# google/ffn

Measured on AMD Instinct MI355X. Metric: FoV-steps/sec (flood-filling inference loop, 250^3 volume), higher is better.
Workload: dtype f32 (fp16 hi + scaled-residual split products on the fp16 MFMA, f32 accumulate)

## Files before the change

### ffn_amd/csrc/ffn_canvas_kernels.h

```cpp
#pragma once

namespace ffn {

struct Box {
  int lo[3];
  int n[3];
  int cy, cx;
};

__device__ __forceinline__ size_t box_index(const Box& b, long e) {
  const int x = e % b.n[2];
  const long t = e / b.n[2];
  const int y = t % b.n[1];
  const int z = t / b.n[1];
  return ((size_t)(b.lo[0] + z) * b.cy + (b.lo[1] + y)) * b.cx + (b.lo[2] + x);
}

template <typename T>
__global__ void box_read_kernel(const T* __restrict__ vol, Box b, long total,
                                T* __restrict__ dst) {
  for (long e = blockIdx.x * (long)blockDim.x + threadIdx.x; e < total;
       e += (long)gridDim.x * blockDim.x)
    dst[e] = vol[box_index(b, e)];
}

template <typename T>
__global__ void box_write_kernel(T* __restrict__ vol, Box b, long total,
                                 const T* __restrict__ src) {
  for (long e = blockIdx.x * (long)blockDim.x + threadIdx.x; e < total;
       e += (long)gridDim.x * blockDim.x)
    vol[box_index(b, e)] = src[e];
}

template <typename T>
__global__ void box_fill_kernel(T* __restrict__ vol, Box b, long total, T value) {
  for (long e = blockIdx.x * (long)blockDim.x + threadIdx.x; e < total;
       e += (long)gridDim.x * blockDim.x)
    vol[box_index(b, e)] = value;
}

__global__ void fill_u32_kernel(uint32_t* __restrict__ p, uint32_t v, size_t n) {
  const size_t n4 = n / 4;
  uint4 vv = make_uint4(v, v, v, v);
  for (size_t e = blockIdx.x * (size_t)blockDim.x + threadIdx.x; e < n4;
       e += (size_t)gridDim.x * blockDim.x)
    reinterpret_cast<uint4*>(p)[e] = vv;
  if (blockIdx.x == 0 && threadIdx.x < (n & 3)) p[n4 * 4 + threadIdx.x] = v;
}

__global__ void points_read_kernel(const float* __restrict__ seed,
                                   const int32_t* __restrict__ seg, int cz,
                                   int cy, int cx, int n,
                                   const int32_t* __restrict__ pos,
                                   float* __restrict__ seed_out,
                                   int32_t* __restrict__ seg_out) {
  const int k = blockIdx.x * blockDim.x + threadIdx.x;
  if (k >= n) return;
  const int z = pos[3 * k], y = pos[3 * k + 1], x = pos[3 * k + 2];
  if (z < 0 || z >= cz || y < 0 || y >= cy || x < 0 || x >= cx) {
    seed_out[k] = __builtin_nanf("");
    seg_out[k] = 0;
    return;
  }
  const size_t ci = ((size_t)z * cy + y) * cx + x;
  seed_out[k] = seed[ci];
  seg_out[k] = seg[ci];
}

__global__ void points_write_seg_kernel(int32_t* __restrict__ seg, int cy, int cx,
                                        int n, const int32_t* __restrict__ pos,
                                        const int32_t* __restrict__ val) {
  const int k = blockIdx.x * blockDim.x + threadIdx.x;
  if (k >= n) return;
  seg[((size_t)pos[3 * k] * cy + pos[3 * k + 1]) * cx + pos[3 * k + 2]] = val[k];
}

__global__ void set_seg_point_kernel(int32_t* __restrict__ seg, size_t ci,
                                     int32_t value) {
  seg[ci] = value;
}

__global__ void set_seed_point_kernel(float* __restrict__ seed, size_t ci,
                                      float value) {
  seed[ci] = value;
}

__global__ void any_segmented_kernel(const int32_t* __restrict__ seg, Box b,
                                     long total, int32_t* __restrict__ out) {
  int hit = 0;
  for (long e = blockIdx.x * (long)blockDim.x + threadIdx.x; e < total;
       e += (long)gridDim.x * blockDim.x)
    hit |= seg[box_index(b, e)] > 0;
  if (__any(hit) && (threadIdx.x & 63) == 0) atomicOr(out, 1);
}

__global__ void commit_count_kernel(const float* __restrict__ seed,
                                    const int32_t* __restrict__ seg, Box b,
                                    long total, float thr, int32_t max_id,
                                    unsigned long long* __restrict__ counts,
                                    unsigned* __restrict__ hist) {
  unsigned raw = 0, act = 0;
  for (long e = blockIdx.x * (long)blockDim.x + threadIdx.x; e < total;
       e += (long)gridDim.x * blockDim.x) {
    const size_t ci = box_index(b, e);
    if (seed[ci] >= thr) {
      ++raw;
      const int32_t s = seg[ci];
      if (s <= 0) {
        ++act;
      } else if (s <= max_id) {
        atomicAdd(&hist[s], 1u);
      }
    }
  }
#pragma unroll
  for (int off = 32; off > 0; off >>= 1) {
    raw += __shfl_xor(raw, off);
    act += __shfl_xor(act, off);
  }
  if ((threadIdx.x & 63) == 0) {
    if (raw) atomicAdd(&counts[0], (unsigned long long)raw);
    if (act) atomicAdd(&counts[1], (unsigned long long)act);
  }
}

__global__ void commit_assign_kernel(const float* __restrict__ seed,
                                     int32_t* __restrict__ seg, Box b, long total,
                                     float thr, int32_t sid) {
  for (long e = blockIdx.x * (long)blockDim.x + threadIdx.x; e < total;
       e += (long)gridDim.x * blockDim.x) {
    const size_t ci = box_index(b, e);
    if (seed[ci] >= thr && seg[ci] <= 0) seg[ci] = sid;
  }
}

struct TurnRecord {
  unsigned long long counts[2];
  int committed;
  int chosen;
  int pad[2];
};
constexpr int kTurnOk = 0, kTurnSegmented = 1, kTurnTooClose = 2, kTurnNotReached = 3,
              kTurnRestricted = 4;

__global__ void turn_commit_kernel(const float* __restrict__ seed,
                                   int32_t* __restrict__ seg, Box b, long total,
                                   float thr, int32_t sid, long long min_size,
                                   TurnRecord* __restrict__ rec, long mark_ci,
                                   int mark_mode) {
  const bool ok = total > 0 && (long long)rec->counts[1] >= min_size;
  if (ok) {
    for (long e = blockIdx.x * (long)blockDim.x + threadIdx.x; e < total;
         e += (long)gridDim.x * blockDim.x) {
      const size_t ci = box_index(b, e);
      if (seed[ci] >= thr && seg[ci] <= 0) seg[ci] = sid;
    }
  }
  if (blockIdx.x == 0 && threadIdx.x == 0) {
    rec->committed = ok ? 1 : 0;
    if ((mark_mode == 1 || (mark_mode == 2 && !ok)) && seg[mark_ci] == 0)
      seg[mark_ci] = -1;
  }
}

__global__ __launch_bounds__(64) void turn_eval_kernel(
    const float* __restrict__ seed, const int32_t* __restrict__ seg, int cz, int cy,
    int cx, const int32_t* __restrict__ cand, int mz, int my, int mx,
    int* __restrict__ flags, float* __restrict__ cand_seed,
    int32_t* __restrict__ cand_seg, const unsigned long long* __restrict__ rplanes,
    size_t plane_words, int row_words) {
  const int j = blockIdx.x;
  const int z = cand[3 * j], y = cand[3 * j + 1], x = cand[3 * j + 2];
  const size_t ci = ((size_t)z * cy + y) * cx + x;
  const int32_t s = seg[ci];
  int flag = kTurnOk;
  bool restricted = false;
  if (rplanes) {
    const size_t wi = ((size_t)z * cy + y) * row_words + (x >> 6);
    restricted = ((rplanes[wi] | rplanes[plane_words + wi]) >> (x & 63)) & 1ull;
  }
  if (s > 0) {
    flag = kTurnSegmented;
  } else if (restricted) {
    flag = kTurnRestricted;
  } else {
    const int z0 = max(z - mz, 0), z1 = min(z + mz + 1, cz);
    const int y0 = max(y - my, 0), y1 = min(y + my + 1, cy);
    const int x0 = max(x - mx, 0), x1 = min(x + mx + 1, cx);
    const int ny = y1 - y0, nx = x1 - x0;
    const int total = (z1 - z0) * ny * nx;
    int hit = 0;
    for (int e = threadIdx.x; e < total; e += 64) {
      const int ex = e % nx, t = e / nx;
      hit |= seg[((size_t)(z0 + t / ny) * cy + (y0 + t % ny)) * cx + (x0 + ex)] > 0;
    }
    if (__any(hit)) flag = kTurnTooClose;
  }
  if (threadIdx.x == 0) {
    flags[j] = flag;
    cand_seed[j] = seed[ci];
    cand_seg[j] = s;
  }
}

__global__ __launch_bounds__(64) void turn_pick_kernel(
    int32_t* __restrict__ seg, int cy, int cx, const int32_t* __restrict__ cand,
    int n, int* __restrict__ flags, TurnRecord* __restrict__ rec) {
  int chosen = -1;
  for (int base = 0; base < n && chosen < 0; base += 64) {
    const int j = base + threadIdx.x;
    const unsigned long long m = __ballot(j < n && flags[j] == kTurnOk);
    if (m) chosen = base + __ffsll((long long)m) - 1;
  }
  const int upto = chosen < 0 ? n : chosen;
  for (int j = threadIdx.x; j < n; j += 64) {
    if (j < upto) {
      if (flags[j] == kTurnTooClose)
        seg[((size_t)cand[3 * j] * cy + cand[3 * j + 1]) * cx + cand[3 * j + 2]] = -1;
    } else if (j > upto) {
      flags[j] = kTurnNotReached;
    }
  }
  if (threadIdx.x == 0) rec->chosen = chosen;
}

__global__ void turn_clear_kernel(uint32_t* __restrict__ seed, Box b, long total,
                                  int linear, size_t nvox,
                                  const TurnRecord* __restrict__ rec) {
  if (rec->chosen < 0) return;
  if (linear) {
    const size_t n4 = nvox / 4;
    const uint4 vv = make_uint4(0x7fc00000u, 0x7fc00000u, 0x7fc00000u, 0x7fc00000u);
    for (size_t e = blockIdx.x * (size_t)blockDim.x + threadIdx.x; e < n4;
         e += (size_t)gridDim.x * blockDim.x)
      reinterpret_cast<uint4*>(seed)[e] = vv;
    if (blockIdx.x == 0 && threadIdx.x < (nvox & 3))
      seed[n4 * 4 + threadIdx.x] = 0x7fc00000u;
    return;
  }
  for (long e = blockIdx.x * (long)blockDim.x + threadIdx.x; e < total;
       e += (long)gridDim.x * blockDim.x)
    seed[box_index(b, e)] = 0x7fc00000u;
}

__global__ void turn_seed_kernel(float* __restrict__ seed, int cy, int cx,
                                 const int32_t* __restrict__ cand, float value,
                                 const TurnRecord* __restrict__ rec) {
  const int j = rec->chosen;
  if (j < 0) return;
  seed[((size_t)cand[3 * j] * cy + cand[3 * j + 1]) * cx + cand[3 * j + 2]] = value;
}

}
```

### ffn_amd/csrc/ffn_hip.hip

```cpp

#include <hip/hip_runtime.h>
#include <hip/hip_ext.h>

#include <algorithm>
#include <cmath>
#include <cstdarg>
#include <cstdio>
#include <cstdlib>
#include <chrono>
#include <cstring>
#include <map>
#include <mutex>
#include <string>
#include <vector>

#include "ffn_internal.h"
#include "ffn_kernels.h"
#include "ffn_restrict_kernels.h"
#include "ffn_host_loop.h"

using namespace ffn;

namespace {

constexpr int kHeadBlocks = 281;

thread_local std::string g_error;

int fail(int code, const char* fmt, ...) {
  char buf[512];
  va_list ap;
  va_start(ap, fmt);
  vsnprintf(buf, sizeof(buf), fmt, ap);
  va_end(ap);
  g_error = buf;
  return code;
}

}

int ffn_set_error(int code, const char* fmt, ...) {
  char buf[512];
  va_list ap;
  va_start(ap, fmt);
  vsnprintf(buf, sizeof(buf), fmt, ap);
  va_end(ap);
  g_error = buf;
  return code;
}

namespace {

#define HIP_TRY(expr)                                                        \
  do {                                                                       \
    hipError_t _e = (expr);                                                  \
    if (_e != hipSuccess)                                                    \
      return fail(FFN_ERR_HIP, "%s failed: %s (%s:%d)", #expr,               \
                  hipGetErrorString(_e), __FILE__, __LINE__);                \
  } while (0)

}

struct ffn_engine {
  std::recursive_mutex mu;
  std::mutex util_mu;
  hipStream_t ustream = nullptr;
  hipEvent_t main_ev = nullptr;
  std::mutex many_mu;
  ffn_host::ManyCarry many_carry;
  uint32_t many_ticket = 0;
  std::vector<ffn_canvas*> many_canvases;
  int device = 0;
  hipStream_t stream = nullptr;
  Geom g{};
  Geom gp{};
  bool permuted = false;
  int depth = 0;
  int max_batch = 0;
  bool weights_set = false;

  float* act_base = nullptr;
  float* bufT = nullptr;
  float* bufX = nullptr;
  uint32_t* validbits = nullptr;
  int32_t* pidx = nullptr;
  int nchunks_c = 0, Rc = 0;
  int fuse_head = 1;
  int count_blocks = kHeadBlocks;
  int store_policy = 1;
  long long* d_dbg = nullptr;
  int dbg_clock = 0;
  int dbg_layer = 3;
  size_t lds_bytes_c = 0;
  int nchunks_k = 0, Rc_k = 0;
  bool k_ok = false;
  float* rawT = nullptr;
  float* rawX = nullptr;
  float* rawS = nullptr;
  bool d_ok = false;
  bool e_ok = false;
  int batch_chunks = 1;
  bool small_now = false;
  bool m_ok = false;
  bool m_now = false;
  bool t_ok = false;
  bool t_now = false;
  int tail_batched = 0;
  int flow = 0;
  unsigned* flow_flags = nullptr;
  unsigned* flow_err = nullptr;
  unsigned flow_epoch = 0;
  int flow_debug = 0;
  bool flow_fits = false;
  int flow_strikes = 0;
  int flow_skip = 0;
  int flow_auto_off = 0;
  long stat_flow_voids = 0;
  bool last_stack_resident = false;
  bool slot_resident[2] = {false, false};
  long long* flow_trace = nullptr;
  int flow_trace_slots = 0;
  int n_main = 0, n_tail = 0, n_tail3 = 0;
  int tsched_aoff[4 * 8] = {};
  int t3sched_aoff[4 * 8] = {};
  int nchunks_m = 0;
  int nchunks_e = 0;
  size_t lds_bytes_e = 0;
  int esched_aoff[4 * 8] = {};
  bool d_weights_ok = true;
  uint16_t* wpackd = nullptr;
  size_t wpackd_layer = 0;
  uint16_t* wpackh = nullptr;
  bool h_ok = false;
  bool h_now = false;
  int n_half = 0;
  int flow_pace = -1;
  int flow_pace_tail = 0;
  int flow_pace_spread = -1;
  int pace_auto = 0;
  float pace_auto_us[2] = {0.f, 0.f};
  int cus = 0;
  size_t lds_bytes_d = 0;
  int dsched_aoff[4 * 8] = {};
  int dsched_btap[4 * 8] = {};
  unsigned* range_flag = nullptr;
  struct Spec {
    bool valid = false;
    const ffn_canvas* canvas = nullptr;
    int n = 0;
    int pos[kSpecMax][3] = {};
    float pad_value = 0.f, move_thr = 0.f;
    int variant = 0;
  } spec;
  int speculate = 1;
  int spec_force_mismatch = 0;
  long stat_spec_mismatch = 0;
  long stat_many_carried = 0;
  int fuse_paste = 1;
  int fuse_conv0a = 1;
  int* d_spec_choice = nullptr;
  long stat_spec_launched = 0, stat_spec_hits = 0;
  long stat_spec_miss_full = 0, stat_spec_miss_short = 0;
  long long stat_segturn_queue_ns = 0, stat_segturn_wait_ns = 0;
  long stat_segturn_calls = 0;
  int stack_ahead = 1;
  int paste_blocks = 0;
  int debug_submit_delay_ns = 0;
  int debug_fused_twice = 0;
  bool trace_now = false;
  bool ahead_valid = false;
  long stat_ahead_used = 0, stat_ahead_wasted = 0;
  unsigned range_tag = 0;
  bool fp16_ok = true;
  int conv_variant = 0;
  int exact_variant = 0;
  float* h_io = nullptr;
  float* up_image = nullptr;
  float* up_seed = nullptr;
  float* seed_raw = nullptr;
  float* seed_raw_alt = nullptr;
  unsigned* range_flag_alt = nullptr;
  int* d_spec_choice_alt = nullptr;
  float* logits = nullptr;
  unsigned* count = nullptr;
  uint8_t* valid = nullptr;
  float* weights = nullptr;
  size_t w0a_off = 0, b0a_off = 0, wl_off = 0;
  size_t w0ap_off = 0;
  std::vector<size_t> wpack_off, bias_off;

  StepItem* d_items = nullptr;
  StepItem* h_items = nullptr;
  unsigned long long* h_pub = nullptr;
  unsigned step_id = 0;
  int next_slot = 0;
  int slot_n[2] = {0, 0};
  bool slot_waited[2] = {false, false};
  unsigned slot_ticket[2] = {0, 0};
  std::vector<ffn_canvas*> slot_canvas[2];
  int sync_mode = 1;
  long stat_calls = 0, stat_items = 0;
  long stat_hist[65] = {};
  long long* d_stamps = nullptr;
  long long t_arrived_ns = 0;
  int fused_trace_in = 0;
  long long stat_turn_host_ns = 0, stat_launch_host_ns = 0;
  long stat_turn_host_count = 0;

  void* d_scratch = nullptr;
  void* h_scratch = nullptr;
  size_t scratch_bytes = 0;

  int prof_mode = 0;
  std::vector<hipEvent_t> events;
  int events_used = 0;
  hipEvent_t ahead_ev[2] = {nullptr, nullptr};
  bool ahead_ev_pending = false;
  double conv_ms = 0.0;
  int64_t conv_launches = 0;
  size_t lds_bytes = 0;
  std::vector<ffn_canvas*> canvases;
  int prof_every = 1;
  long stack_calls = 0;
  bool prof_now = false;
  int ablate = 0;
  std::vector<int> chain_launches_pending;
  std::vector<float> prof_samples;
};

struct ffn_canvas {
  ffn_engine* engine = nullptr;
  float* image = nullptr;
  uint8_t* image_u8 = nullptr;
  float* image_lut = nullptr;
  float* seed = nullptr;
  int32_t* seg = nullptr;
  int cz = 0, cy = 0, cx = 0;
  size_t nvox = 0;
  int dirty_lo[3] = {0, 0, 0};
  int dirty_hi[3] = {0, 0, 0};
  ffn_host::SegmentState loop;
  hipEvent_t ev_util = nullptr;
  bool util_pending = false;
  bool paste_after_flag = false;
  int hint_n = 0;
  int hint_pos[kSpecMax][3] = {};
  bool hint_from_loop = false;
  unsigned long long* restrict_planes = nullptr;
  size_t restrict_plane_words = 0;
  int restrict_row_words = 0;
  std::vector<uint64_t> restrict_host;

  void mark_dirty(const int lo[3], const int hi[3]) {
    const int dims[3] = {cz, cy, cx};
    const bool empty = dirty_lo[0] >= dirty_hi[0];
    for (int k = 0; k < 3; ++k) {
      const int l = std::max(lo[k], 0), h = std::min(hi[k], dims[k]);
      dirty_lo[k] = empty ? l : std::min(dirty_lo[k], l);
      dirty_hi[k] = empty ? h : std::max(dirty_hi[k], h);
    }
  }
};

namespace {
inline long long steady_ns() {
  return std::chrono::duration_cast<std::chrono::nanoseconds>(
             std::chrono::steady_clock::now().time_since_epoch()).count();
}
inline unsigned next_tag(unsigned t) { return t + 1 ? t + 1 : 1; }
inline void drop_spec(ffn_engine* e) {
  if (e->spec.valid && !e->ahead_valid) e->range_tag = next_tag(e->range_tag);
  if (e->ahead_valid) e->stat_ahead_wasted += 1;
  e->spec.valid = false;
  e->ahead_valid = false;
}
struct EngineLock {
  std::unique_lock<std::recursive_mutex> lk;
  explicit EngineLock(ffn_engine* e) {
    if (e) lk = std::unique_lock<std::recursive_mutex>(e->mu);
  }
};
constexpr int kFlowStrikes = 3;

int flow_voided(ffn_engine* e, bool timed_out) {
  if (!timed_out) return 0;
  EngineLock lock_(e);
  e->stat_flow_voids += 1;
  e->flow_strikes += 1;
  e->flow_skip = 1;
  if (e->flow_strikes >= kFlowStrikes && e->flow == 2) {
    e->flow = 0;
    e->flow_auto_off = 1;
    e->flow_skip = 0;
    return fail(FFN_ERR_FLOW,
                "the resident conv launch timed out waiting for one of its own "
                "workgroups %d steps in a row (is the GPU shared or partitioned?): "
                "the step changed nothing; this engine now runs one launch per conv "
                "(option flow = 0; set flow = 2 to try again) -- repeat the step",
                kFlowStrikes);
  }
  return fail(FFN_ERR_FLOW,
              "the resident conv launch timed out waiting for one of its own "
              "workgroups: the step changed nothing; repeat it (the repeat runs one "
              "launch per conv, same arithmetic)");
}

struct UtilLock {
  std::unique_lock<std::mutex> ul;
  std::unique_lock<std::recursive_mutex> lk;
  explicit UtilLock(ffn_engine* e) {
    if (e) {
      ul = std::unique_lock<std::mutex>(e->util_mu);
      lk = std::unique_lock<std::recursive_mutex>(e->mu);
    }
  }
  hipError_t begin(ffn_engine* e, ffn_canvas* c, bool reads_only = false) {
    if (!reads_only) drop_spec(e);
    if (!c->paste_after_flag) return hipSuccess;
    hipError_t err = hipEventRecord(e->main_ev, e->stream);
    if (err == hipSuccess) err = hipStreamWaitEvent(e->ustream, e->main_ev, 0);
    if (err == hipSuccess) c->paste_after_flag = false;
    return err;
  }
  hipError_t end(ffn_engine* e, ffn_canvas* c) {
    c->util_pending = true;
    return hipEventRecord(c->ev_util, e->ustream);
  }
  hipError_t wait(ffn_engine* e, ffn_canvas* c) {
    hipError_t err = end(e, c);
    if (err != hipSuccess) return err;
    lk.unlock();
    err = hipEventSynchronize(c->ev_util);
    lk.lock();
    if (err == hipSuccess) c->util_pending = false;
    return err;
  }
};
hipError_t canvas_quiesce(ffn_engine* e, ffn_canvas* c) {
  drop_spec(e);
  hipError_t err = hipSuccess;
  if (c->paste_after_flag) {
    err = hipStreamSynchronize(e->stream);
    if (err == hipSuccess) c->paste_after_flag = false;
  }
  if (err == hipSuccess && c->util_pending) {
    err = hipEventSynchronize(c->ev_util);
    if (err == hipSuccess) c->util_pending = false;
  }
  return err;
}
}

int ffn_canvas_view(ffn_canvas* c, FfnCanvasView* out) {
  if (!c || !out) return ffn_set_error(FFN_ERR_ARG, "NULL canvas");
  if (!c->engine)
    return ffn_set_error(FFN_ERR_STATE, "canvas outlived its engine");
  {
    EngineLock lock_(c->engine);
    if (canvas_quiesce(c->engine, c) != hipSuccess)
      return ffn_set_error(FFN_ERR_HIP, "canvas_quiesce failed");
  }
  out->device_id = c->engine->device;
  out->engine_stream = c->engine->stream;
  out->image = c->image;
  out->image_u8 = c->image_u8;
  out->image_lut = c->image_lut;
  out->segmentation = c->seg;
  out->shape_zyx[0] = c->cz;
  out->shape_zyx[1] = c->cy;
  out->shape_zyx[2] = c->cx;
  return FFN_OK;
}

namespace {

int ensure_scratch(ffn_engine* e, size_t bytes) {
  if (bytes <= e->scratch_bytes) return FFN_OK;
  HIP_TRY(hipStreamSynchronize(e->ustream));
  if (e->d_scratch) HIP_TRY(hipFree(e->d_scratch));
  if (e->h_scratch) HIP_TRY(hipHostFree(e->h_scratch));
  e->d_scratch = e->h_scratch = nullptr;
  e->scratch_bytes = 0;
  size_t want = std::max<size_t>(bytes, 1 << 20);
  HIP_TRY(hipMalloc(&e->d_scratch, want));
  HIP_TRY(hipHostMalloc(&e->h_scratch, want, hipHostMallocDefault));
  e->scratch_bytes = want;
  return FFN_OK;
}

template <bool RI, bool RO, bool SK>
int set_lds_attr(size_t bytes) {
  HIP_TRY(hipFuncSetAttribute(
      reinterpret_cast<const void*>(&conv32_kernel<RI, RO, SK>),
      hipFuncAttributeMaxDynamicSharedMemorySize, (int)bytes));
  return FFN_OK;
}

inline void split_fp16x2(float x, uint16_t part[2]) {
  const float xh = std::fabs(x) < 6.103515625e-05f ? 0.0f : x;
  const _Float16 hi = (_Float16)xh;
  const _Float16 res = (_Float16)((x - (float)hi) * 2048.0f);
  std::memcpy(&part[0], &hi, 2);
  std::memcpy(&part[1], &res, 2);
}

int set_lds_attr_d(size_t bytes) {
#define FFN_D_ATTR(KIND, SK, KSV, HEADV)                                          \
  HIP_TRY(hipFuncSetAttribute(                                                    \
      reinterpret_cast<const void*>(&conv32d_kernel<KIND, SK, KSV, HEADV>),       \
      hipFuncAttributeMaxDynamicSharedMemorySize, (int)bytes))
#define FFN_D_ATTRS(KSV)            \
  FFN_D_ATTR(0, false, KSV, false); \
  FFN_D_ATTR(1, false, KSV, false); \
  FFN_D_ATTR(1, true, KSV, false);  \
  FFN_D_ATTR(1, false, KSV, true);  \
  FFN_D_ATTR(1, true, KSV, true)
  FFN_D_ATTRS(8);
  FFN_D_ATTRS(9);
  FFN_D_ATTRS(10);
#undef FFN_D_ATTRS
#undef FFN_D_ATTR
  return FFN_OK;
}

constexpr int kERows = 208, kETiles = 3, kEPieces = 7;

// ... 389 lines not shown
  nx.tiles_x = qx;
  nx.so.out_sp = reinterpret_cast<char*>(e->rawT) + (size_t)q.guard * 16;
  nx.so.sp_plane_bytes = (q.act_stride / kFeatures) * 16;
  nx.so.item_bytes = q.act_stride * (long)sizeof(float);
  nx.so.range_flag = next ? e->range_flag_alt : e->range_flag;
  nx.so.range_tag = tag;
  nx.sp = sp;
  if (sp.n > 0) nx.sp.choice = next ? e->d_spec_choice_alt : e->d_spec_choice;
  return qz * qy * qx;
}

void launch_conv0a(ffn_engine* e, int n, const StepItems& si, float pad_value,
                   unsigned tag, const SpecArgs& sp, bool next = false) {
  const Geom& g = e->g;
  const float* W = e->weights;
  const int tz = (g.fz + kC0Z - 1) / kC0Z, ty = (g.fy + kC0Y - 1) / kC0Y,
            tx = (g.fx + kC0X - 1) / kC0X;
  if (e->conv_variant >= 6) {
    Conv0Next nx;
    const int tiles = conv0a_split_args(e, pad_value, tag, sp, next, nx);
    hipLaunchKernelGGL(conv0a_mfma_kernel<true>, dim3(tiles, n),
                       dim3(kC0Threads), 0, e->stream, si, pad_value, nx.w, nx.bias,
                       nx.out, nx.seed_raw, nx.q, nx.tiles_y, nx.tiles_x, nx.so, nx.sp);
  } else {
    SpecArgs sp2 = sp;
    if (sp.n > 0) sp2.choice = next ? e->d_spec_choice_alt : e->d_spec_choice;
    hipLaunchKernelGGL(conv0a_mfma_kernel<false>, dim3(tz * ty * tx, n),
                       dim3(kC0Threads), 0, e->stream, si, pad_value,
                       W + e->w0a_off, W + e->b0a_off, e->bufT,
                       next ? e->seed_raw_alt : e->seed_raw, g, ty, tx,
                       Conv0SplitOut(), sp2);
  }
}

int launch_conv32ps(ffn_engine* e, float pad_value, float move_thr,
                    const int* ahead_choice = nullptr, hipEvent_t ev0 = nullptr,
                    hipEvent_t ev1 = nullptr) {
  HeadFusion hf;
  hf.on = true;
  hf.pad_value = pad_value;
  hf.move_thr = move_thr;
  ConvDArgs a;
  conv32d_args(e, 1, e->rawT, e->rawS, 0, hf, a);
  a.L.dbg = e->dbg_clock ? e->d_dbg : nullptr;
  ConvTailMap mp;
  tail_map(e, 1, mp);
  const Geom& g = e->gp;
  ConvStackTab tb;
  tb.nlayers = 2 * e->depth - 1;
  tb.dbg_layer = e->dbg_layer;
  tb.sp_t = reinterpret_cast<const char*>(e->rawT) + (size_t)g.guard * 16;
  tb.sp_s = reinterpret_cast<char*>(e->rawS) + (size_t)g.guard * 16;
  tb.wpack0 = reinterpret_cast<const char*>(e->wpackd);
  tb.wpack_stride = (long)(e->wpackd_layer * sizeof(uint16_t));
  tb.bias0 = e->weights + e->bias_off[0];
  tb.bias_stride = e->depth > 1 ? (long)(e->bias_off[1] - e->bias_off[0]) : 0;
  tb.epoch0 = e->flow_epoch;
  tb.pace = e->flow_pace < 0 ? e->pace_auto : e->flow_pace;
  tb.pace_tail = e->flow_pace_tail;
  tb.pace_spread = e->flow_pace_spread < 0 ? tb.pace : e->flow_pace_spread;
  e->flow_epoch += (unsigned)tb.nlayers;
  const dim3 grid(8 * (mp.mains_per_xcd + mp.tails_per_xcd)), block(kDThreads);
  tb.l_begin = 0;
  tb.l_end = tb.nlayers;
  tb.stamps = e->d_stamps;
  tb.ahead_choice = ahead_choice;
  tb.trace = e->trace_now ? 1 : (ahead_choice && e->fused_trace_in == 1) ? 2 : 0;
  const long long t_l0 = e->t_arrived_ns ? steady_ns() : 0;
  if (ev0)
    hipExtLaunchKernelGGL(conv32ps_kernel, grid, block, kMLdsBytes, e->stream, ev0, ev1, 0, a,
                          mp, tb);
  else
    hipLaunchKernelGGL(conv32ps_kernel, grid, block, kMLdsBytes, e->stream, a, mp, tb);
  if (e->t_arrived_ns) {
    const long long t_l1 = steady_ns();
    if (t_l1 - e->t_arrived_ns < 100000) {
      e->stat_turn_host_ns += t_l1 - e->t_arrived_ns;
      e->stat_launch_host_ns += t_l1 - t_l0;
      e->stat_turn_host_count += 1;
    }
    e->t_arrived_ns = 0;
  }
  return FFN_OK;
}

void half_map(const ffn_engine* e, ConvHalfMap& mp) {
  mp.n_chunks = e->n_half;
  mp.per_first = std::max(1, e->cus / 8);
  mp.n_first = std::min(e->n_half, 8 * mp.per_first);
  mp.per_second = (e->n_half - mp.n_first + 7) / 8;
}

template <int KIND, bool SK>
int launch_conv32h(ffn_engine* e, const float* raw_in, float* raw_out, int layer,
                   const HeadFusion& head = HeadFusion()) {
  ConvDArgs a;
  conv32d_args(e, 1, raw_in, raw_out, layer, head, a);
  a.L.wpack = reinterpret_cast<const char*>(e->wpackh + (size_t)layer * e->wpackd_layer);
  a.flow_n_main = -1;
  ConvHalfMap mp;
  half_map(e, mp);
  const dim3 grid(8 * (mp.per_first + mp.per_second)), block(kDThreads);
  if (head.on) {
    if constexpr (KIND == 1)
      hipLaunchKernelGGL((conv32h_kernel<KIND, SK, true>), grid, block, kHLdsBytes, e->stream,
                         a, mp);
  } else {
    hipLaunchKernelGGL((conv32h_kernel<KIND, SK, false>), grid, block, kHLdsBytes, e->stream,
                       a, mp);
  }
  return FFN_OK;
}

int launch_conv32hs(ffn_engine* e, float pad_value, float move_thr) {
  HeadFusion hf;
  hf.on = true;
  hf.pad_value = pad_value;
  hf.move_thr = move_thr;
  ConvDArgs a;
  conv32d_args(e, 1, e->rawT, e->rawS, 0, hf, a);
  a.flow_n_main = -1;
  ConvHalfMap mp;
  half_map(e, mp);
  const Geom& g = e->gp;
  ConvStackTab tb;
  tb.nlayers = 2 * e->depth - 1;
  tb.dbg_layer = e->dbg_layer;
  tb.sp_t = reinterpret_cast<const char*>(e->rawT) + (size_t)g.guard * 16;
  tb.sp_s = reinterpret_cast<char*>(e->rawS) + (size_t)g.guard * 16;
  tb.wpack0 = reinterpret_cast<const char*>(e->wpackh);
  tb.wpack_stride = (long)(e->wpackd_layer * sizeof(uint16_t));
  tb.bias0 = e->weights + e->bias_off[0];
  tb.bias_stride = e->depth > 1 ? (long)(e->bias_off[1] - e->bias_off[0]) : 0;
  tb.epoch0 = e->flow_epoch;
  e->flow_epoch += (unsigned)tb.nlayers;
  tb.l_begin = 0;
  tb.l_end = tb.nlayers;
  tb.pace = e->flow_pace < 0 ? 0 : e->flow_pace;
  tb.pace_tail = 0;
  tb.pace_spread = e->flow_pace_spread < 0 ? tb.pace : e->flow_pace_spread;
  tb.stamps = nullptr;
  tb.ahead_choice = nullptr;
  tb.trace = 0;
  const dim3 grid(8 * (mp.per_first + mp.per_second)), block(kDThreads);
  hipLaunchKernelGGL(conv32hs_kernel, grid, block, kHLdsBytes, e->stream, a, mp, tb);
  return FFN_OK;
}

int run_stack(ffn_engine* e, int n, const StepItems& si, float pad_value,
              float move_thr, bool conv0a_done = false, bool ahead = false) {
  const Geom& g = e->g;
  const float* W = e->weights;
  if (!conv0a_done) drop_spec(e);
  if (e->ahead_valid) e->stat_ahead_wasted += 1;
  e->spec.valid = false;
  e->ahead_valid = false;
  e->last_stack_resident = false;
  e->range_tag = next_tag(e->range_tag);
  std::swap(e->seed_raw, e->seed_raw_alt);
  std::swap(e->range_flag, e->range_flag_alt);
  std::swap(e->d_spec_choice, e->d_spec_choice_alt);
  const bool sampled = (e->stack_calls % e->prof_every) == 0;
  e->stack_calls++;
  e->prof_now = e->prof_mode == 1 && sampled;
  const bool prof_chain = e->prof_mode == 2 && sampled;
  if (!conv0a_done) launch_conv0a(e, n, si, pad_value, e->range_tag, SpecArgs());
  int rc;
  const float* head_in;
  bool head_fused = false;
  e->ahead_ev_pending = false;
  const bool one_launch = e->conv_variant == 9 && n == 1 && e->flow == 2 &&
                          e->flow_skip == 0 && e->tail_batched == 0;
  hipEvent_t k_ev0 = nullptr, k_ev1 = nullptr;
  if (prof_chain && ahead) {
    if (one_launch) k_ev0 = e->ahead_ev[0], k_ev1 = e->ahead_ev[1];
    else HIP_TRY(hipEventRecord(e->ahead_ev[0], e->stream));
  } else if (prof_chain) {
    if (e->events_used + 2 > (int)e->events.size()) {
      rc = flush_events(e);
      if (rc) return rc;
    }
    e->chain_launches_pending.push_back(2 * e->depth - 1);
    if (one_launch) {
      k_ev0 = e->events[e->events_used], k_ev1 = e->events[e->events_used + 1];
      e->events_used += 2;
    } else {
      HIP_TRY(hipEventRecord(e->events[e->events_used++], e->stream));
    }
  }
  e->small_now = e->conv_variant == 7 ||
                 (e->conv_variant == 6 && e->batch_chunks == 1 && n >= 2 && e->e_ok);
  e->m_now = e->conv_variant >= 8 ||
             (e->conv_variant == 6 && e->batch_chunks == 2 && n >= 2 && e->m_ok);
  e->t_now = e->conv_variant == 9 && (n == 1 || e->tail_batched != 0);
  e->h_now = e->conv_variant == 10 && n == 1;
  if (e->conv_variant >= 6) {
    if (e->depth == 1)
      return fail(FFN_ERR_ARG, "conv_variant 6 needs depth >= 2 (fused head)");
    auto chain = [&]() -> int {
      if (e->h_now) {
        if (e->flow == 2 && e->flow_skip > 0) {
          e->flow_skip -= 1;
        } else if (e->flow == 2) {
          e->last_stack_resident = true;
          return launch_conv32hs(e, pad_value, move_thr);
        }
        int r = launch_conv32h<1, false>(e, e->rawT, e->rawS, 0);
        for (int i = 1; i < e->depth && !r; ++i) {
          r = launch_conv32h<0, false>(e, e->rawS, e->rawT, 2 * i - 1);
          if (r) break;
          HeadFusion hf;
          hf.on = i == e->depth - 1;
          hf.pad_value = pad_value;
          hf.move_thr = move_thr;
          r = launch_conv32h<1, true>(e, e->rawT, e->rawS, 2 * i, hf);
        }
        return r;
      }
      if (e->t_now && n == 1 && e->flow == 2) {
        if (e->flow_skip > 0) {
          e->flow_skip -= 1;
        } else {
          e->last_stack_resident = true;
          return launch_conv32ps(e, pad_value, move_thr, ahead ? e->d_spec_choice : nullptr,
                                 k_ev0, k_ev1);
        }
      }
      if (ahead) return fail(FFN_ERR_STATE, "stack_ahead without the resident launch");
      int r = launch_conv32d<1, false>(e, n, e->rawT, e->rawS, 0);
      for (int i = 1; i < e->depth && !r; ++i) {
        r = launch_conv32d<0, false>(e, n, e->rawS, e->rawT, 2 * i - 1);
        if (r) break;
        HeadFusion hf;
        hf.on = i == e->depth - 1;
        hf.pad_value = pad_value;
        hf.move_thr = move_thr;
        r = launch_conv32d<1, true>(e, n, e->rawT, e->rawS, 2 * i, hf);
      }
      return r;
    };
    rc = chain();
    if (rc) return rc;
    head_fused = true;
    head_in = e->bufX;
  } else if (e->conv_variant == 0) {
    rc = launch_conv32<false, false, false>(e, n, e->bufT, e->bufX, nullptr, 0);
    if (rc) return rc;
    for (int i = 1; i < e->depth; ++i) {
      rc = launch_conv32<true, true, false>(e, n, e->bufX, e->bufT, nullptr,
                                            2 * i - 1);
      if (rc) return rc;
      rc = launch_conv32<false, false, true>(e, n, e->bufT, e->bufX, e->bufX,
                                             2 * i);
      if (rc) return rc;
    }
    head_in = e->bufX;
  } else {
    rc = launch_conv32c<false, false, false>(e, n, e->bufT, e->bufX, nullptr, 0);
    if (rc) return rc;
    for (int i = 1; i < e->depth; ++i) {
      rc = launch_conv32c<true, true, false>(e, n, e->bufX, e->bufT, nullptr,
                                             2 * i - 1);
      if (rc) return rc;
      HeadFusion hf;
      hf.on = e->fuse_head && i == e->depth - 1 && e->ablate == 0;
      hf.pad_value = pad_value;
      hf.move_thr = move_thr;
      rc = launch_conv32c<false, false, true>(e, n, e->bufT, e->bufX, e->bufX,
                                              2 * i, hf);
      if (rc) return rc;
      head_fused = hf.on;
    }
    head_in = e->bufX;
  }
  if (prof_chain && ahead) {
    if (!k_ev0) HIP_TRY(hipEventRecord(e->ahead_ev[1], e->stream));
    e->ahead_ev_pending = true;
  } else if (prof_chain && !k_ev0) {
    HIP_TRY(hipEventRecord(e->events[e->events_used++], e->stream));
  }
  if (head_fused) {
    e->count_blocks = e->h_now ? e->n_half
                      : e->t_now ? e->n_main + (n == 1 ? e->n_tail : e->n_tail3)
                      : e->m_now ? e->nchunks_m : e->small_now ? e->nchunks_e
                      : e->conv_variant >= 6 ? e->nchunks_k : e->nchunks_c;
  } else {
    e->count_blocks = kHeadBlocks;
    hipLaunchKernelGGL(head_kernel, dim3(kHeadBlocks, n), dim3(256), 0, e->stream,
                       head_in, e->seed_raw, pad_value, W + e->wl_off, move_thr,
                       e->logits, e->count, g);
  }
  HIP_TRY(hipGetLastError());
  return FFN_OK;
}

int dense_items(ffn_engine* e, int n, StepItems* si) {
  const Geom& g = e->g;
  for (int k = 0; k < n; ++k) {
    StepItem& it = e->h_items[k];
    std::memset(&it, 0, sizeof(it));
    it.image = e->up_image + (size_t)k * g.V;
    it.image_u8 = nullptr;
    it.image_lut = nullptr;
    it.seed = e->up_seed + (size_t)k * g.V;
    it.seg = nullptr;
    it.cz = g.fz;
    it.cy = g.fy;
    it.cx = g.fx;
// ... 26 lines not shown
int check_canvas(const ffn_canvas* c) {
  if (!c) return fail(FFN_ERR_ARG, "null canvas");
  if (!c->engine) return fail(FFN_ERR_STATE, "canvas outlived its engine");
  return FFN_OK;
}

int check_box(const ffn_canvas* c, const int32_t lo[3], const int32_t hi[3]) {
  const int dims[3] = {c->cz, c->cy, c->cx};
  for (int k = 0; k < 3; ++k)
    if (lo[k] < 0 || hi[k] > dims[k] || hi[k] < lo[k])
      return fail(FFN_ERR_ARG, "box [%d,%d) out of canvas axis %d (size %d)",
                  lo[k], hi[k], k, dims[k]);
  return FFN_OK;
}

int grid_for(long total, int block = 256) {
  long g = (total + block - 1) / block;
  return (int)std::max<long>(1, std::min<long>(g, 2048));
}

}

extern "C" {

int ffn_abi_version(void) { return 10; }

const char* ffn_last_error(void) { return g_error.c_str(); }

size_t ffn_engine_weight_count(int depth, int features) {
  const size_t F = (size_t)features;
  return 27 * 2 * F + F + (size_t)(2 * depth - 1) * (27 * F * F + F) + F + 1;
}

int ffn_engine_create(int device_id, const int32_t fov_zyx[3],
                      const int32_t deltas_zyx[3], int depth, int features,
                      int max_batch, ffn_engine** out) {
  if (!out || !fov_zyx || !deltas_zyx) return fail(FFN_ERR_ARG, "null argument");
  *out = nullptr;
  if (features != kFeatures)
    return fail(FFN_ERR_ARG, "features must be %d (got %d)", kFeatures, features);
  if (depth < 1 || max_batch < 1)
    return fail(FFN_ERR_ARG, "depth and max_batch must be >= 1");
  for (int k = 0; k < 3; ++k) {
    if (fov_zyx[k] < 3 || fov_zyx[k] % 2 == 0)
      return fail(FFN_ERR_ARG, "fov must be odd and >= 3 per axis");
    if (deltas_zyx[k] < 0 || 2 * deltas_zyx[k] + 1 > fov_zyx[k])
      return fail(FFN_ERR_ARG, "deltas do not fit inside the fov");
  }
  int ndev = 0;
  HIP_TRY(hipGetDeviceCount(&ndev));
  if (device_id < 0 || device_id >= ndev)
    return fail(FFN_ERR_ARG, "device %d not present (%d visible)", device_id, ndev);
  HIP_TRY(hipSetDevice(device_id));

  ffn_engine* e = new ffn_engine();
  e->device = device_id;
  e->depth = depth;
  e->max_batch = max_batch;
  Geom& g = e->g;
  g.fz = fov_zyx[0];
  g.fy = fov_zyx[1];
  g.fx = fov_zyx[2];
  g.dz = deltas_zyx[0];
  g.dy = deltas_zyx[1];
  g.dx = deltas_zyx[2];
  g.XS = g.fx + 1;
  g.plane = (g.fy + 1) * g.XS;
  g.npos = g.fz * g.plane;
  g.guard = g.plane + g.XS + 1;
  g.nchunks = (g.npos + kChunk - 1) / kChunk;
  g.V = g.fz * g.fy * g.fx;
  g.R = kChunk + 2 * (g.XS + 1);
  g.oa[0] = 0, g.oa[1] = 1, g.oa[2] = 2;
  g.dstr[0] = g.fy * g.fx, g.dstr[1] = g.fx, g.dstr[2] = 1;
  g.crop = 0;
  g.c0[0] = g.c0[1] = g.c0[2] = 0;
  g.c1[0] = g.fz, g.c1[1] = g.fy, g.c1[2] = g.fx;
  g.Vp = g.V;
  auto permute = [&](const int oa[3]) {
    const int f[3] = {g.fz, g.fy, g.fx}, d[3] = {g.dz, g.dy, g.dx};
    const int ds[3] = {g.fy * g.fx, g.fx, 1};
    Geom q = g;
    q.fz = f[oa[0]], q.fy = f[oa[1]], q.fx = f[oa[2]];
    q.dz = d[oa[0]], q.dy = d[oa[1]], q.dx = d[oa[2]];
    q.XS = q.fx + 1;
    q.plane = (q.fy + 1) * q.XS;
    q.npos = q.fz * q.plane;
    q.guard = q.plane + q.XS + 1;
    q.nchunks = (q.npos + kChunk - 1) / kChunk;
    q.R = kChunk + 2 * (q.XS + 1);
    for (int a = 0; a < 3; ++a) q.oa[a] = oa[a], q.dstr[a] = ds[oa[a]];
    return q;
  };
  auto chunk_span = [](const Geom& q, int start, int chunk, int count) {
    auto pad = [&](int v) {
      const int x = v % q.fx, y = (v / q.fx) % q.fy, z = v / (q.fx * q.fy);
      return z * q.plane + y * q.XS + x;
    };
    int span = 0;
    for (int c = 0; c < count; ++c) {
      const int lo = start + c * chunk, hi = std::min(q.V, lo + chunk) - 1;
      if (lo <= hi) span = std::max(span, pad(hi) - pad(lo) + 1);
    }
    return span;
  };
  auto m_fits = [&](const Geom& q) {
    return chunk_span(q, 0, kMChunk, (q.V + kMChunk - 1) / kMChunk) +
               2 * (q.XS + 1) <= kMRows;
  };
  e->gp = g;
  if (!m_fits(g)) {
    static const int kPerms[5][3] = {{0, 2, 1}, {1, 0, 2}, {1, 2, 0}, {2, 0, 1},
                                     {2, 1, 0}};
    int best = -1;
    for (int k = 0; k < 5; ++k) {
      const Geom q = permute(kPerms[k]);
      if (m_fits(q) && (best < 0 || q.fx < permute(kPerms[best]).fx)) best = k;
    }
    if (best >= 0) {
      e->gp = permute(kPerms[best]);
      e->permuted = true;
    }
  }
  const long positions = std::max(
      (long)g.guard + (long)g.nchunks * kChunk + g.guard + 320,
      (long)e->gp.guard + (long)e->gp.nchunks * kChunk + e->gp.guard + 320);
  g.act_stride = positions * kFeatures;
  e->gp.act_stride = g.act_stride;
  e->lds_bytes = (size_t)3 * g.R * kFeatures * sizeof(float);
  if (e->lds_bytes > 160 * 1024) {
    delete e;
    return fail(FFN_ERR_ARG, "fov too wide for the LDS-staged conv (%zu B)",
                e->lds_bytes);
  }

#define E_TRY(expr)                                                          \
  do {                                                                       \
    hipError_t _e = (expr);                                                  \
    if (_e != hipSuccess) {                                                  \
      int _rc = fail(FFN_ERR_HIP, "%s failed: %s (%s:%d)", #expr,            \
                     hipGetErrorString(_e), __FILE__, __LINE__);             \
      ffn_engine_destroy(e);                                                 \
      return _rc;                                                            \
    }                                                                        \
  } while (0)

  E_TRY(hipStreamCreateWithFlags(&e->stream, hipStreamNonBlocking));
  {
    int lo = 0, hi = 0;
    E_TRY(hipDeviceGetStreamPriorityRange(&lo, &hi));
    E_TRY(hipStreamCreateWithPriority(&e->ustream, hipStreamNonBlocking, hi));
  }
  E_TRY(hipEventCreateWithFlags(&e->main_ev, hipEventDisableTiming));
  const size_t act_bytes = (size_t)3 * max_batch * g.act_stride * sizeof(float);
  E_TRY(hipMalloc(&e->act_base, act_bytes));
  E_TRY(hipMemset(e->act_base, 0, act_bytes));
  e->rawT = e->act_base;
  e->rawX = e->rawT + (size_t)max_batch * g.act_stride;
  e->rawS = e->rawX + (size_t)max_batch * g.act_stride;
  e->bufT = e->rawT + (size_t)g.guard * kFeatures;
  e->bufX = e->rawX + (size_t)g.guard * kFeatures;
  const size_t vbytes = (size_t)max_batch * g.V * sizeof(float);
  E_TRY(hipMalloc(&e->up_image, vbytes));
  E_TRY(hipMalloc(&e->up_seed, vbytes));
  E_TRY(hipMalloc(&e->seed_raw, vbytes));
  E_TRY(hipMalloc(&e->seed_raw_alt, vbytes));
  E_TRY(hipMalloc(&e->logits, vbytes));
  E_TRY(hipHostMalloc(&e->h_io, 3 * vbytes, hipHostMallocDefault));
  E_TRY(hipMemset(e->up_image, 0, vbytes));
  E_TRY(hipMemset(e->up_seed, 0, vbytes));
  E_TRY(hipMalloc(&e->count, sizeof(unsigned) * max_batch *
                                  std::max<size_t>(kHeadBlocks, (g.V + 31) / 32)));
  E_TRY(hipMalloc(&e->d_items, sizeof(StepItem) * 2 * max_batch));
  E_TRY(hipHostMalloc(&e->h_items, sizeof(StepItem) * 2 * max_batch,
                      hipHostMallocDefault));
  E_TRY(hipHostMalloc(&e->h_pub,
                      sizeof(unsigned long long) * kPubWords * 2 * max_batch,
                      hipHostMallocDefault));
  std::memset(e->h_pub, 0, sizeof(unsigned long long) * kPubWords * 2 * max_batch);

  {
    std::vector<uint8_t> v((size_t)g.nchunks * kChunk, 0);
    for (int p = 0; p < g.npos; ++p) {
      const int rem = p % g.plane;
      v[p] = (rem / g.XS < g.fy && rem % g.XS < g.fx) ? 1 : 0;
    }
    E_TRY(hipMalloc(&e->valid, v.size()));
    E_TRY(hipMemcpy(e->valid, v.data(), v.size(), hipMemcpyHostToDevice));
    std::vector<uint32_t> bits((size_t)g.nchunks * 5, 0u);
    for (size_t p = 0; p < v.size(); ++p)
      if (v[p]) bits[(p / kChunk) * 5 + ((p % kChunk) >> 5)] |= 1u << (p & 31);
    static_assert(kChunk == 160, "validbits layout assumes 5 words per chunk");
    E_TRY(hipMalloc(&e->validbits, bits.size() * sizeof(uint32_t)));
    E_TRY(hipMemcpy(e->validbits, bits.data(), bits.size() * sizeof(uint32_t),
                    hipMemcpyHostToDevice));
  }

  {
    e->nchunks_c = (g.V + kCChunk - 1) / kCChunk;
    e->nchunks_k = (g.V + kDChunk - 1) / kDChunk;
    std::vector<int32_t> pidx(std::max((size_t)e->nchunks_c * kCChunk,
                                       (size_t)e->nchunks_k * kDChunk));
    for (size_t v = 0; v < pidx.size(); ++v) {
      const int vv = (int)std::min<size_t>(v, (size_t)g.V - 1);
      const int x = vv % g.fx, y = (vv / g.fx) % g.fy, z = vv / (g.fx * g.fy);
      pidx[v] = z * g.plane + y * g.XS + x;
    }
    int span = 0;
    for (int c = 0; c < e->nchunks_c; ++c)
      span = std::max(span, pidx[(size_t)c * kCChunk + kCChunk - 1] -
                                pidx[(size_t)c * kCChunk] + 1);
    e->Rc = ((span + 2 * (g.XS + 1)) + 31) / 32 * 32;
    if (e->Rc < 256) e->Rc = 256;
    e->lds_bytes_c = (size_t)2 * e->Rc * kCLdsStride * sizeof(float);
    {
      const Geom& q = e->gp;
      const int span_k = chunk_span(q, 0, kDChunk, e->nchunks_k);
      e->Rc_k = ((span_k + 2 * (q.XS + 1)) + 31) / 32 * 32;
      if (e->Rc_k < 256) e->Rc_k = 256;
      e->k_ok = e->Rc_k <= 320 && e->nchunks_k >= 2;
      static const int kSched[4][7] = {{0, 1, 8, 9, 16, 18, 19},
                                       {2, 3, 10, 11, 17, 20, 21},
                                       {4, 5, 12, 13, 22, 23, 24},
                                       {6, 7, 14, 15, 25, 26, -1}};
      e->lds_bytes_d = std::max((size_t)3 * 128 * e->Rc_k,
                                (size_t)4 * kDChunk * kDRowB + 64);
      for (int w = 0; w < 4; ++w)
        for (int j = 0; j < 7; ++j) {
          int s = kSched[w][j];
          const bool dummy = s < 0;
          if (dummy) s = kSched[w][j - 1];
          const int kz = s / 9, ky = (s / 3) % 3, kx = s % 3;
          e->dsched_aoff[w * 8 + j] =
              kz * 128 * e->Rc_k + ((ky - 1) * q.XS + (kx - 1)) * 16;
          e->dsched_btap[w * 8 + j] = dummy ? 27 : s;
        }
      e->d_ok = e->k_ok && e->lds_bytes_d <= 160 * 1024 && depth >= 2;
      {
        const int ce = 32 * kETiles;
        e->nchunks_e = (q.V + ce - 1) / ce;
        const int span_e = chunk_span(q, 0, ce, e->nchunks_e);
        e->lds_bytes_e = std::max((size_t)3 * 128 * kERows,
                                  (size_t)4 * ce * kDRowB + 64);
        e->e_ok = e->d_ok && span_e + 2 * (q.XS + 1) <= kERows &&
                  e->nchunks_e >= 2 && e->lds_bytes_e <= 80 * 1024;
        e->nchunks_m = (q.V + kMChunk - 1) / kMChunk;
        const int span_m = chunk_span(q, 0, kMChunk, e->nchunks_m);
        e->m_ok = e->d_ok && span_m + 2 * (q.XS + 1) <= kMRows && e->nchunks_m >= 2;
        if (e->m_ok && e->nchunks_m > 256) {
          e->n_main = 256;
          e->n_tail = (q.V - 256 * kMChunk + 31) / 32;
          e->n_tail3 = (q.V - 256 * kMChunk + 95) / 96;
          const int span_t = chunk_span(q, 256 * kMChunk, 32, e->n_tail);
          const int span_t3 = chunk_span(q, 256 * kMChunk, 96, e->n_tail3);
          static_assert((size_t)3 * 128 * kTRows <= kMLdsBytes &&
                            (size_t)4 * 32 * kDRowB + 64 <= kMLdsBytes &&
                            (size_t)3 * 128 * kT3Rows <= kMLdsBytes &&
                            (size_t)4 * 96 * kDRowB + 64 <= kMLdsBytes,
                        "a tail workgroup fits conv32m's LDS");
          e->t_ok = span_t + 2 * (q.XS + 1) <= kTRows &&
                    span_t3 + 2 * (q.XS + 1) <= kT3Rows && e->n_tail <= 256;
          for (int w = 0; w < 4; ++w)
            for (int j = 0; j < 7; ++j) {
              int s = kSched[w][j];
              if (s < 0) s = kSched[w][j - 1];
              const int kz = s / 9, ky = (s / 3) % 3, kx = s % 3;
              e->tsched_aoff[w * 8 + j] =
                  kz * 128 * kTRows + ((ky - 1) * q.XS + (kx - 1)) * 16;
              e->t3sched_aoff[w * 8 + j] =
                  kz * 128 * kT3Rows + ((ky - 1) * q.XS + (kx - 1)) * 16;
            }
        }
        for (int w = 0; w < 4; ++w)
          for (int j = 0; j < 7; ++j) {
            int s = kSched[w][j];
            if (s < 0) s = kSched[w][j - 1];
            const int kz = s / 9, ky = (s / 3) % 3, kx = s % 3;
            e->esched_aoff[w * 8 + j] =
                kz * 128 * kERows + ((ky - 1) * q.XS + (kx - 1)) * 16;
          }
      }
    }
    E_TRY(hipMalloc(&e->d_dbg, (24 + 4 * kDbgMaxWgs) * sizeof(long long)));
    E_TRY(hipMemset(e->d_dbg, 0, (24 + 4 * kDbgMaxWgs) * sizeof(long long)));
    E_TRY(hipMalloc(&e->pidx, pidx.size() * sizeof(int32_t)));
    E_TRY(hipMemcpy(e->pidx, pidx.data(), pidx.size() * sizeof(int32_t),
                    hipMemcpyHostToDevice));
    const bool c_ok = e->Rc == 256 || e->Rc == 288;
    e->exact_variant = c_ok ? 2 : 0;
    e->conv_variant = e->t_ok ? 9 : e->m_ok ? 8 : e->d_ok ? 6 : e->exact_variant;
    if (e->t_ok && depth >= 2) {
      int cus = 0, per_cu = 0;
      E_TRY(hipDeviceGetAttribute(&cus, hipDeviceAttributeMultiprocessorCount, device_id));
      E_TRY(hipFuncSetAttribute(reinterpret_cast<const void*>(conv32ps_kernel),
                                hipFuncAttributeMaxDynamicSharedMemorySize, kMLdsBytes));
      E_TRY(hipOccupancyMaxActiveBlocksPerMultiprocessor(&per_cu, conv32ps_kernel,
                                                         kDThreads, kMLdsBytes));
      ConvTailMap mp;
      tail_map(e, 1, mp);
      const int grid = 8 * (mp.mains_per_xcd + mp.tails_per_xcd);
      e->flow_fits = cus >= e->n_main && (long)cus * per_cu >= grid;
    }
    e->flow = e->flow_fits ? 2 : 0;
    if (e->t_ok && depth >= 2) {
      const Geom& q = e->gp;
      e->n_half = FFN_H_VCLIP ? FFN_H_VCLIP / kHChunk : (q.V + kHChunk - 1) / kHChunk;
      const int span_h = chunk_span(q, 0, kHChunk, e->n_half);
      int cus = 0, per_cu = 0;
      E_TRY(hipDeviceGetAttribute(&cus, hipDeviceAttributeMultiprocessorCount, device_id));
      e->cus = cus;
      E_TRY(hipFuncSetAttribute(reinterpret_cast<const void*>(conv32hs_kernel),
                                hipFuncAttributeMaxDynamicSharedMemorySize, kHLdsBytes));
      E_TRY(hipOccupancyMaxActiveBlocksPerMultiprocessor(&per_cu, conv32hs_kernel, kDThreads,
                                                         kHLdsBytes));
      ConvHalfMap mp;
      half_map(e, mp);
      e->h_ok = e->n_half >= 2 && span_h + 2 * (q.XS + 1) <= kHRows &&
                (long)cus * per_cu >= 8 * (mp.per_first + mp.per_second);
    }
  }

  {
    size_t off = 0;
    e->w0a_off = off;
    off += 27 * 2 * kFeatures;
    e->b0a_off = off;
    off += kFeatures;
    e->w0ap_off = off;
    off += 27 * 2 * kFeatures;
    for (int l = 0; l < 2 * depth - 1; ++l) {
      e->wpack_off.push_back(off);
      off += 27 * kFeatures * kFeatures;
      e->bias_off.push_back(off);
      off += kFeatures;
    }
    e->wl_off = off;
    off += kFeatures + 1;
    off = (off + 3) & ~(size_t)3;
    E_TRY(hipMalloc(&e->weights, off * sizeof(float)));
    e->wpackd_layer = (size_t)kDTaps * 2 * 2 * 64 * 8;
    E_TRY(hipMalloc(&e->wpackd, e->wpackd_layer * (2 * depth - 1) *
                                    sizeof(uint16_t)));
    E_TRY(hipMalloc(&e->wpackh, e->wpackd_layer * (2 * depth - 1) * sizeof(uint16_t)));
    E_TRY(hipMalloc(&e->range_flag, 2 * sizeof(unsigned)));
    E_TRY(hipMemset(e->range_flag, 0, 2 * sizeof(unsigned)));
    E_TRY(hipMalloc(&e->range_flag_alt, 2 * sizeof(unsigned)));
    E_TRY(hipMemset(e->range_flag_alt, 0, 2 * sizeof(unsigned)));
    {
      const size_t words = ((size_t)(e->gp.V + 31) / 32 + 64) * kFlowStride;
      E_TRY(hipMalloc(&e->flow_flags, words * sizeof(unsigned)));
      E_TRY(hipMemset(e->flow_flags, 0, words * sizeof(unsigned)));
      E_TRY(hipMalloc(&e->flow_err, sizeof(unsigned)));
      E_TRY(hipMemset(e->flow_err, 0, sizeof(unsigned)));
      if (e->t_ok) {
        e->flow_trace_slots = std::max(e->n_main + e->n_tail, (e->gp.V + kHChunk - 1) / kHChunk);
        const size_t bytes = (size_t)e->flow_trace_slots * kFlowTraceLayers * 8 * sizeof(long long);
        E_TRY(hipMalloc(&e->flow_trace, bytes));
        E_TRY(hipMemset(e->flow_trace, 0, bytes));
      }
    }
    E_TRY(hipMalloc(&e->d_stamps, (32 + 1024) * sizeof(long long)));
    E_TRY(hipMemset(e->d_stamps, 0, (32 + 1024) * sizeof(long long)));
    E_TRY(hipMalloc(&e->d_spec_choice, sizeof(int)));
    E_TRY(hipMemset(e->d_spec_choice, 0xff, sizeof(int)));
    E_TRY(hipMalloc(&e->d_spec_choice_alt, sizeof(int)));
    E_TRY(hipMemset(e->d_spec_choice_alt, 0xff, sizeof(int)));
  }

  e->events.resize(2 * 64);
  for (auto& ev : e->events) E_TRY(hipEventCreate(&ev));
  for (auto& ev : e->ahead_ev) E_TRY(hipEventCreate(&ev));

  {
    int rc = set_lds_attr<false, false, false>(e->lds_bytes);
    if (!rc) rc = set_lds_attr<true, true, false>(e->lds_bytes);
    if (!rc) rc = set_lds_attr<false, false, true>(e->lds_bytes);
    if (!rc) rc = set_lds_attr_c<false, false, false>(e->lds_bytes_c);
    if (!rc) rc = set_lds_attr_c<true, true, false>(e->lds_bytes_c);
    if (!rc) rc = set_lds_attr_c<false, false, true>(e->lds_bytes_c);
    if (!rc) rc = set_lds_attr_c<false, false, true, 8>(e->lds_bytes_c);
    if (!rc) rc = set_lds_attr_c<false, false, true, 16>(e->lds_bytes_c);
    if (!rc) rc = set_lds_attr_c<false, false, true, 24>(e->lds_bytes_c);
    if (!rc && e->d_ok) rc = set_lds_attr_d(e->lds_bytes_d);
    if (!rc && e->e_ok) rc = set_lds_attr_e(e->lds_bytes_e);
    if (!rc && e->m_ok) rc = set_lds_attr_m();
    if (rc) {
      ffn_engine_destroy(e);
      return rc;
    }
  }
#undef E_TRY
  *out = e;
  return FFN_OK;
}

void ffn_engine_destroy(ffn_engine* e) {
  if (!e) return;
  (void)hipSetDevice(e->device);
  if (e->stream) (void)hipStreamSynchronize(e->stream);
  for (ffn_canvas* c : e->canvases) {
    (void)hipFree(c->image);
    (void)hipFree(c->image_u8);
    (void)hipFree(c->image_lut);
    (void)hipFree(c->seed);
    (void)hipFree(c->seg);
    (void)hipFree(c->restrict_planes);
    c->restrict_planes = nullptr;
    if (c->ev_util) (void)hipEventDestroy(c->ev_util);
    c->ev_util = nullptr;
    c->image = c->seed = nullptr;
    c->image_u8 = nullptr;
    c->image_lut = nullptr;
    c->seg = nullptr;
    c->engine = nullptr;
  }
  e->canvases.clear();
  if (e->ustream) (void)hipStreamSynchronize(e->ustream);
  if (e->main_ev) (void)hipEventDestroy(e->main_ev);
  if (e->ustream) (void)hipStreamDestroy(e->ustream);
  for (auto& ev : e->events)
    if (ev) (void)hipEventDestroy(ev);
  for (auto& ev : e->ahead_ev)
    if (ev) (void)hipEventDestroy(ev);
  (void)hipFree(e->act_base);
  (void)hipFree(e->up_image);
  (void)hipFree(e->up_seed);
  (void)hipFree(e->seed_raw);
  (void)hipFree(e->seed_raw_alt);
  (void)hipFree(e->range_flag_alt);
  (void)hipFree(e->d_spec_choice_alt);
  (void)hipFree(e->logits);
  (void)hipFree(e->count);
  (void)hipFree(e->wpackd);
  (void)hipFree(e->wpackh);
  (void)hipFree(e->range_flag);
  (void)hipFree(e->flow_flags);
  (void)hipFree(e->flow_err);
  (void)hipFree(e->flow_trace);
  (void)hipFree(e->d_spec_choice);
  (void)hipFree(e->d_stamps);
  (void)hipFree(e->valid);
  (void)hipFree(e->validbits);
  (void)hipFree(e->pidx);
  (void)hipFree(e->d_dbg);
  (void)hipFree(e->weights);
  (void)hipFree(e->d_items);
  (void)hipFree(e->d_scratch);
  if (e->h_io) (void)hipHostFree(e->h_io);
  if (e->h_items) (void)hipHostFree(e->h_items);
  if (e->h_pub) (void)hipHostFree(e->h_pub);
  if (e->h_scratch) (void)hipHostFree(e->h_scratch);
  if (e->stream) (void)hipStreamDestroy(e->stream);
  delete e;
}

struct PaceKey {
  int device, depth, V;
  bool operator<(const PaceKey& o) const {
    return device != o.device ? device < o.device : depth != o.depth ? depth < o.depth : V < o.V;
  }
};
struct PaceVal { int beat; float free_us, best_us; };
std::mutex g_pace_mu;
std::map<PaceKey, PaceVal> g_pace_cache;

int tune_pace(ffn_engine* e) {
  e->pace_auto = 0;
  e->pace_auto_us[0] = e->pace_auto_us[1] = 0.f;
  if (!(e->t_ok && e->flow_fits && e->flow == 2 && e->conv_variant == 9 && e->depth >= 2))
    return FFN_OK;
  const PaceKey key{e->device, e->depth, e->g.V};
  {
    std::lock_guard<std::mutex> lk(g_pace_mu);
    auto it = g_pace_cache.find(key);
    if (it != g_pace_cache.end()) {
      e->pace_auto = it->second.beat;
      e->pace_auto_us[0] = it->second.free_us;
      e->pace_auto_us[1] = it->second.best_us;
      return FFN_OK;
    }
  }
  const size_t V = (size_t)e->g.V;
  {
    std::vector<float> noise(2 * V);
    unsigned x = 12345u;
    for (auto& v : noise) {
      x = x * 1664525u + 1013904223u;
      v = ((int)(x >> 8) % 2001 - 1000) * 1e-3f;
    }
    HIP_TRY(hipMemcpy(e->up_image, noise.data(), V * sizeof(float), hipMemcpyHostToDevice));
    HIP_TRY(hipMemcpy(e->up_seed, noise.data() + V, V * sizeof(float), hipMemcpyHostToDevice));
  }
  unsigned errs0 = 0;
  HIP_TRY(hipMemcpy(&errs0, e->flow_err, sizeof(errs0), hipMemcpyDeviceToHost));
  StepItems si;
  int rc = dense_items(e, 1, &si);
  if (rc) return rc;
  hipEvent_t ev0, ev1;
  HIP_TRY(hipEventCreate(&ev0));
  HIP_TRY(hipEventCreate(&ev1));
  const int user_pace = e->flow_pace;
  auto stacks_us = [&](int pace, int reps, float* us) -> int {
    e->flow_pace = pace;
    int r = FFN_OK;
    for (int k = 0; k < 6 && !r; ++k) r = run_stack(e, 1, si, std::nanf(""), INFINITY);
    if (!r && hipEventRecord(ev0, e->stream) != hipSuccess) r = FFN_ERR_HIP;
    for (int k = 0; k < reps && !r; ++k) r = run_stack(e, 1, si, std::nanf(""), INFINITY);
    if (!r && (hipEventRecord(ev1, e->stream) != hipSuccess ||
               hipEventSynchronize(ev1) != hipSuccess))
      r = FFN_ERR_HIP;
    float ms = 0.f;
    if (!r && hipEventElapsedTime(&ms, ev0, ev1) != hipSuccess) r = FFN_ERR_HIP;
    *us = ms * 1e3f / (float)reps;
    return r;
  };
  float us = 0.f, free_us = 0.f, best_us = 0.f;
  int best = 0;
  {
    const long long t_end = steady_ns() + 150000000LL;
    while (!rc && steady_ns() < t_end) rc = stacks_us(0, 60, &us);
  }
  if (!rc) rc = stacks_us(0, 40, &free_us);
  best_us = 1e30f;
  for (int pace = 560; pace <= 800 && !rc; pace += 20) {
    rc = stacks_us(pace, 24, &us);
    if (!rc && us < best_us) {
      best_us = us;
      best = pace;
    }
  }
  if (!rc) {
    rc = stacks_us(0, 40, &us);
    free_us = std::min(free_us, us);
  }
  bool keep = !rc && best > 0 && best_us < 0.985f * free_us;
  float conf_free = free_us, conf_paced = best_us;
  for (int round = 0; round < 2 && keep && !rc; ++round) {
    float f = 0.f, p = 0.f;
    rc = stacks_us(0, 40, &f);
    if (!rc) rc = stacks_us(best + 10, 40, &p);
    keep = !rc && p < 0.985f * f;
    conf_free = f;
    conf_paced = p;
  }
  e->flow_pace = user_pace;
  (void)hipEventDestroy(ev0);
  (void)hipEventDestroy(ev1);
  if (rc) return rc;
  unsigned errs = 0;
  HIP_TRY(hipMemcpy(&errs, e->flow_err, sizeof(errs), hipMemcpyDeviceToHost));
  const bool timed_out = errs != errs0;
  e->pace_auto_us[0] = conf_free;
  e->pace_auto_us[1] = keep ? conf_paced : best_us;
  if (!timed_out && keep) e->pace_auto = best + 10;
  if (!timed_out) {
    std::lock_guard<std::mutex> lk(g_pace_mu);
    g_pace_cache[key] = PaceVal{e->pace_auto, e->pace_auto_us[0], e->pace_auto_us[1]};
  }
  return FFN_OK;
}

int ffn_engine_set_weights(ffn_engine* e, const float* blob, size_t count) {
  EngineLock lock_(e);
  if (!e || !blob) return fail(FFN_ERR_ARG, "null argument");
  const size_t want = ffn_engine_weight_count(e->depth, kFeatures);
  if (count != want)
    return fail(FFN_ERR_ARG, "weight blob has %zu floats, expected %zu", count,
                want);
  drop_spec(e);
  HIP_TRY(hipSetDevice(e->device));
  const int F = kFeatures;
  std::vector<float> host(e->wl_off + F + 1 + 3, 0.0f);
  const float* src = blob;
  std::vector<uint16_t> hostd(e->wpackd_layer * (2 * e->depth - 1));
  std::vector<uint16_t> hosth(hostd.size());
  bool d_weights_ok = true;
  bool weights_in_fp16_range = true;
  int tap_of[27];
  for (int t = 0; t < 27; ++t) {
    const int kp[3] = {t / 9, (t / 3) % 3, t % 3};
    int ko[3];
    for (int a = 0; a < 3; ++a) ko[e->gp.oa[a]] = kp[a];
    tap_of[t] = ko[0] * 9 + ko[1] * 3 + ko[2];
  }
  std::memcpy(&host[e->w0a_off], src, sizeof(float) * 27 * 2 * F);
  for (int t = 0; t < 27; ++t)
    std::memcpy(&host[e->w0ap_off + (size_t)t * 2 * F], src + (size_t)tap_of[t] * 2 * F,
                sizeof(float) * 2 * F);
  src += 27 * 2 * F;
  std::memcpy(&host[e->b0a_off], src, sizeof(float) * F);
  src += F;
  for (int l = 0; l < 2 * e->depth - 1; ++l) {
    float* wp = &host[e->wpack_off[l]];
    for (int tap = 0; tap < 27; ++tap)
      for (int nh = 0; nh < 2; ++nh)
        for (int h = 0; h < 2; ++h)
          for (int lane = 0; lane < 64; ++lane)
            for (int s = 0; s < 4; ++s) {
              const int gq = lane >> 4, j = lane & 15;
              const int ci = 16 * h + 4 * gq + s, co = 16 * nh + j;
// ... 89 lines not shown
    if (!is_void) {
      if (e->last_stack_resident) e->flow_strikes = 0;
      break;
    }
    if (attempt == 2) return fail(FFN_ERR_HIP, "ffn_predict: the step stayed void");
    if (flow_voided(e, flag[1] == e->range_tag) == 0) {
      rc = switch_variant(e, e->exact_variant);
      if (rc) return rc;
    }
    rc = run_stack(e, n, si, std::nanf(""), INFINITY);
    if (rc) return rc;
    HIP_TRY(hipMemcpyAsync(h_logits, e->logits, bytes, hipMemcpyDeviceToHost, e->stream));
  }
  std::memcpy(logits_out, h_logits, bytes);
  return FFN_OK;
}

int ffn_forward_resident(ffn_engine* e, int n, int repeats) {
  EngineLock lock_(e);
  if (!e) return fail(FFN_ERR_ARG, "null argument");
  if (n < 1 || n > e->max_batch)
    return fail(FFN_ERR_ARG, "batch %d outside [1, %d]", n, e->max_batch);
  if (!e->weights_set) return fail(FFN_ERR_STATE, "weights not set");
  HIP_TRY(hipSetDevice(e->device));
  StepItems si;
  int rc = dense_items(e, n, &si);
  if (rc) return rc;
  for (int r = 0; r < repeats; ++r) {
    rc = run_stack(e, n, si, std::nanf(""), INFINITY);
    if (rc) return rc;
  }
  return FFN_OK;
}

int ffn_engine_set_option(ffn_engine* e, const char* name, int value) {
  EngineLock lock_(e);
  if (!e || !name) return fail(FFN_ERR_ARG, "null argument");

  if (std::strcmp(name, "conv_variant") == 0) {
    if (value == -1) value = e->exact_variant;
    if (value != 0 && value != 2 && !(value >= 6 && value <= 10))
      return fail(FFN_ERR_ARG, "conv_variant must be 0, 2, 6, 7, 8, 9 or 10 (1, 3, 4, 5 "
                               "were removed in ABI 7)");
    if (value == 10 && !e->h_ok)
      return fail(FFN_ERR_ARG, "conv_variant 10 unsupported for this fov / depth / device "
                               "(80-voxel workgroups, two per CU, all resident)");
    if (value >= 6 && e->weights_set && !e->fp16_ok)
      return fail(FFN_ERR_ARG, "conv_variant %d: a weight is outside the fp16 range",
                  value);
    if (value == 6 && !e->d_ok)
      return fail(FFN_ERR_ARG, "conv_variant 6 unsupported for this fov / depth");
    if (value == 7 && !e->e_ok)
      return fail(FFN_ERR_ARG, "conv_variant 7 unsupported for this fov / depth");
    if (value == 8 && !e->m_ok)
      return fail(FFN_ERR_ARG, "conv_variant 8 unsupported for this fov / depth");
    if (value == 9 && !e->t_ok)
      return fail(FFN_ERR_ARG, "conv_variant 9 unsupported for this fov / depth "
                               "(257 .. 512 chunks of 128 voxels)");
    if (value >= 6 && e->weights_set && !e->d_weights_ok)
      return fail(FFN_ERR_ARG, "conv_variant 6: a weight x 2^11 is outside the fp16 range");
    if (value == 2 && !(e->Rc == 256 || e->Rc == 288))
      return fail(FFN_ERR_ARG, "conv_variant %d unsupported for this fov", value);
    return switch_variant(e, value);
  }
  if (std::strcmp(name, "profile_every") == 0) {
    if (value < 1) return fail(FFN_ERR_ARG, "profile_every must be >= 1");
    e->prof_every = value;
    return FFN_OK;
  }
  if (std::strcmp(name, "sync_mode") == 0) {
    if (value != 0 && value != 1) return fail(FFN_ERR_ARG, "sync_mode must be 0 or 1");
    e->sync_mode = value;
    return FFN_OK;
  }
  if (std::strcmp(name, "debug_clock") == 0) {
    e->dbg_clock = value;
    return FFN_OK;
  }
  if (std::strcmp(name, "batch_chunks") == 0) {
    if (value < 0 || value > 2) return fail(FFN_ERR_ARG, "batch_chunks 0..2");
    e->batch_chunks = value;
    return FFN_OK;
  }
  if (std::strcmp(name, "tail_batched") == 0) {
    e->tail_batched = value != 0;
    return FFN_OK;
  }
  if (std::strcmp(name, "flow_debug") == 0) {
    e->flow_debug = value;
    return FFN_OK;
  }
  if (std::strcmp(name, "flow_pace") == 0) {
    if (value < -1 || value > 5000)
      return fail(FFN_ERR_ARG, "flow_pace: -1 (measured), 0 (off) .. 5000 (10-ns ticks)");
    e->flow_pace = value;
    return FFN_OK;
  }
  if (std::strcmp(name, "flow_pace_spread") == 0) {
    if (value < -1 || value > 5000) return fail(FFN_ERR_ARG, "flow_pace_spread: -1 .. 5000");
    e->flow_pace_spread = value;
    return FFN_OK;
  }
  if (std::strcmp(name, "flow_pace_tail") == 0) {
    if (value < 0 || value > 5000) return fail(FFN_ERR_ARG, "flow_pace_tail: 0 .. 5000");
    e->flow_pace_tail = value;
    return FFN_OK;
  }
  if (std::strcmp(name, "flow") == 0) {
    if (value < 0 || value > 2) return fail(FFN_ERR_ARG, "flow: 0, 1 or 2");
    if (value && !e->t_ok)
      return fail(FFN_ERR_ARG, "flow needs conv32mt's geometry (conv_variant 9)");
    if (value && e->depth < 2) return fail(FFN_ERR_ARG, "flow needs depth >= 2");
    if (value == 2 && !e->flow_fits)
      return fail(FFN_ERR_ARG, "flow 2: this device cannot hold the resident launch's "
                  "workgroups all at once (compute units x occupancy)");
    drop_spec(e);
    e->flow = value;
    e->flow_auto_off = 0;
    e->flow_strikes = 0;
    e->flow_skip = 0;
    return FFN_OK;
  }
  if (std::strcmp(name, "spec_force_mismatch") == 0) {
    e->spec_force_mismatch = value;
    return FFN_OK;
  }
  if (std::strcmp(name, "fuse_paste") == 0) {
    e->fuse_paste = value != 0;
    return FFN_OK;
  }
  if (std::strcmp(name, "fuse_conv0a") == 0) {
    drop_spec(e);
    e->fuse_conv0a = value != 0;
    return FFN_OK;
  }
  if (std::strcmp(name, "paste_blocks") == 0) {
    if (value < 0 || value > 1024) return fail(FFN_ERR_ARG, "paste_blocks out of range");
    e->paste_blocks = value;
    return FFN_OK;
  }
  if (std::strcmp(name, "debug_fused_twice") == 0) {
    e->debug_fused_twice = value;
    return FFN_OK;
  }
  if (std::strcmp(name, "debug_submit_delay_ns") == 0) {
    e->debug_submit_delay_ns = value;
    return FFN_OK;
  }
  if (std::strcmp(name, "stack_ahead") == 0) {
    drop_spec(e);
    e->stack_ahead = value != 0;
    return FFN_OK;
  }
  if (std::strcmp(name, "speculate") == 0) {
    drop_spec(e);
    e->speculate = value != 0;
    return FFN_OK;
  }
  if (std::strcmp(name, "stat_reset") == 0) {
    e->stat_spec_launched = e->stat_spec_hits = e->stat_spec_mismatch = 0;
    e->stat_ahead_used = e->stat_ahead_wasted = 0;
    e->stat_spec_miss_full = e->stat_spec_miss_short = 0;
    e->stat_segturn_queue_ns = e->stat_segturn_wait_ns = 0;
    e->stat_segturn_calls = 0;
    e->stat_calls = e->stat_items = 0;
    std::memset(e->stat_hist, 0, sizeof(e->stat_hist));
    e->stat_turn_host_ns = e->stat_launch_host_ns = 0;
    e->stat_turn_host_count = 0;
    e->t_arrived_ns = 0;
    HIP_TRY(hipSetDevice(e->device));
    HIP_TRY(hipStreamSynchronize(e->stream));
    HIP_TRY(hipMemset(e->d_stamps, 0, 32 * sizeof(long long)));
    return FFN_OK;
  }
  if (std::strcmp(name, "debug_fused_trace") == 0) {
    HIP_TRY(hipSetDevice(e->device));
    HIP_TRY(hipStreamSynchronize(e->stream));
    HIP_TRY(hipMemset(e->d_stamps + 4, 0x7f, 4 * sizeof(long long)));
    HIP_TRY(hipMemset(e->d_stamps + 8, 0, 4 * sizeof(long long)));
    HIP_TRY(hipMemset(e->d_stamps + 12, 0, 20 * sizeof(long long)));
    HIP_TRY(hipMemset(e->d_stamps + 32, 0, 1024 * sizeof(long long)));
    e->fused_trace_in = value;
    return FFN_OK;
  }
  if (std::strcmp(name, "debug_layer") == 0) {
    e->dbg_layer = value;
    return FFN_OK;
  }
  if (std::strcmp(name, "ablate") == 0) {
    e->ablate = value;
    return FFN_OK;
  }
  if (std::strcmp(name, "fuse_head") == 0) {
    e->fuse_head = value != 0;
    return FFN_OK;
  }
  if (std::strcmp(name, "store_policy") == 0) {
    if (value < 0 || value > 2) return fail(FFN_ERR_ARG, "store_policy 0..2");
    e->store_policy = value;
    return FFN_OK;
  }
  return fail(FFN_ERR_ARG, "unknown option '%s'", name);
}

int ffn_engine_get_option(ffn_engine* e, const char* name, int* value) {
  EngineLock lock_(e);
  if (!e || !name || !value) return fail(FFN_ERR_ARG, "null argument");
  if (std::strcmp(name, "conv_variant") == 0) *value = e->conv_variant;
  else if (std::strcmp(name, "fuse_head") == 0) *value = e->fuse_head;
  else if (std::strcmp(name, "exact_variant") == 0) *value = e->exact_variant;
  else if (std::strcmp(name, "stat_step_calls") == 0) *value = (int)e->stat_calls;
  else if (std::strcmp(name, "stat_step_items") == 0) *value = (int)e->stat_items;
  else if (std::strcmp(name, "speculate") == 0) *value = e->speculate;
  else if (std::strcmp(name, "stack_ahead") == 0) *value = e->stack_ahead;
  else if (std::strcmp(name, "paste_blocks") == 0) *value = e->paste_blocks;
  else if (std::strcmp(name, "stat_segturn_queue_ns") == 0)
    *value = e->stat_segturn_calls ? (int)(e->stat_segturn_queue_ns / e->stat_segturn_calls) : 0;
  else if (std::strcmp(name, "stat_segturn_wait_ns") == 0)
    *value = e->stat_segturn_calls ? (int)(e->stat_segturn_wait_ns / e->stat_segturn_calls) : 0;
  else if (std::strcmp(name, "stat_segturn_calls") == 0) *value = (int)e->stat_segturn_calls;
  else if (std::strcmp(name, "stat_spec_miss_full") == 0) *value = (int)e->stat_spec_miss_full;
  else if (std::strcmp(name, "stat_spec_miss_short") == 0) *value = (int)e->stat_spec_miss_short;
  else if (std::strcmp(name, "stat_ahead_used") == 0) *value = (int)e->stat_ahead_used;
  else if (std::strcmp(name, "stat_ahead_wasted") == 0) *value = (int)e->stat_ahead_wasted;
  else if (std::strcmp(name, "fuse_paste") == 0) *value = e->fuse_paste;
  else if (std::strcmp(name, "fuse_conv0a") == 0) *value = e->fuse_conv0a;
  else if (std::strcmp(name, "stat_spec_launched") == 0)
    *value = (int)e->stat_spec_launched;
  else if (std::strcmp(name, "stat_spec_hits") == 0) *value = (int)e->stat_spec_hits;
  else if (std::strcmp(name, "stat_spec_mismatch") == 0)
    *value = (int)e->stat_spec_mismatch;
  else if (std::strcmp(name, "stat_many_carried") == 0)
    *value = (int)e->stat_many_carried;
  else if (std::strcmp(name, "flow") == 0) *value = e->flow;
  else if (std::strcmp(name, "flow_auto_off") == 0) *value = e->flow_auto_off;
  else if (std::strcmp(name, "stat_flow_voids") == 0) *value = (int)e->stat_flow_voids;
  else if (std::strcmp(name, "stat_turn_host_ns") == 0)
    *value = e->stat_turn_host_count
                 ? (int)(e->stat_turn_host_ns / e->stat_turn_host_count) : 0;
  else if (std::strcmp(name, "stat_launch_host_ns") == 0)
    *value = e->stat_turn_host_count
                 ? (int)(e->stat_launch_host_ns / e->stat_turn_host_count) : 0;
  else if (std::strcmp(name, "stat_turn_count") == 0) *value = (int)e->stat_turn_host_count;
  else if (std::strcmp(name, "stat_ahead_aborted") == 0) {
    long long st[4] = {0, 0, 0, 0};
    HIP_TRY(hipSetDevice(e->device));
    HIP_TRY(hipStreamSynchronize(e->stream));
    HIP_TRY(hipMemcpy(st, e->d_stamps, sizeof(st), hipMemcpyDeviceToHost));
    *value = (int)st[3];
  }
  else if (std::strcmp(name, "stat_turn_gpu_ns") == 0) {
    long long st[4] = {0, 0, 0, 0};
    HIP_TRY(hipSetDevice(e->device));
    HIP_TRY(hipStreamSynchronize(e->stream));
    HIP_TRY(hipMemcpy(st, e->d_stamps, sizeof(st), hipMemcpyDeviceToHost));
    *value = st[2] ? (int)(st[1] * 10 / st[2]) : 0;
  }
  else if (std::strncmp(name, "debug_fused_stamp_", 18) == 0) {
    const int k = std::atoi(name + 18);
    long long st[32 + 1024];
    HIP_TRY(hipSetDevice(e->device));
    HIP_TRY(hipStreamSynchronize(e->stream));
    HIP_TRY(hipMemcpy(st, e->d_stamps, sizeof(st), hipMemcpyDeviceToHost));
    for (int w = 0; w < 512; ++w) st[25] = std::max(st[25], st[32 + w]);
    {
      std::map<unsigned, int> per_cu;
      for (int w = 0; w < 512; ++w) {
        const unsigned v = (unsigned)st[32 + 512 + w];
        if (st[32 + 512 + w] != 0 && ((v - 1) >> 31)) per_cu[(v - 1) & 0x7fffffffu] += 1;
      }
      long long shared = 0;
      for (const auto& kv : per_cu) if (kv.second > 1) shared += kv.second;
      st[27] = st[4] + shared;
      if (!e->stack_ahead) st[27] = st[7] + shared;
    }
    if (k < 4 || k > 27 || k == 15) return fail(FFN_ERR_ARG, "debug_fused_stamp_4 .. 27");
    *value = (int)(st[k] - (e->stack_ahead ? st[4] : st[7]));
  }
  else if (std::strcmp(name, "flow_pace") == 0) *value = e->flow_pace;
  else if (std::strcmp(name, "flow_pace_now") == 0)
    *value = e->flow_pace < 0 ? e->pace_auto : e->flow_pace;
  else if (std::strcmp(name, "flow_pace_free_ns") == 0) *value = (int)(e->pace_auto_us[0] * 1e3f);
  else if (std::strcmp(name, "flow_pace_best_ns") == 0) *value = (int)(e->pace_auto_us[1] * 1e3f);
  else if (std::strcmp(name, "stat_flow_timeouts") == 0) {
    unsigned v = 0;
    HIP_TRY(hipSetDevice(e->device));
    HIP_TRY(hipStreamSynchronize(e->stream));
    HIP_TRY(hipMemcpy(&v, e->flow_err, sizeof(v), hipMemcpyDeviceToHost));
    *value = (int)v;
  }
  else if (std::strncmp(name, "stat_hist_", 10) == 0) {
    const int k = std::atoi(name + 10);
    if (k < 0 || k > 64) return fail(FFN_ERR_ARG, "stat_hist_<0..64>");
    *value = (int)e->stat_hist[k];
  }
  else if (std::strcmp(name, "store_policy") == 0) *value = e->store_policy;
  else if (std::strcmp(name, "sync_mode") == 0) *value = e->sync_mode;
  else if (std::strcmp(name, "profile_every") == 0) *value = e->prof_every;
  else return fail(FFN_ERR_ARG, "unknown option '%s'", name);
  return FFN_OK;
}

int ffn_engine_set_pred_size(ffn_engine* e, const int32_t pred_zyx[3]) {
  EngineLock lock_(e);
  if (!e || !pred_zyx) return fail(FFN_ERR_ARG, "null argument");
  Geom& g = e->g;
  const int f[3] = {g.fz, g.fy, g.fx}, d[3] = {g.dz, g.dy, g.dx};
  for (int a = 0; a < 3; ++a) {
    if (pred_zyx[a] < 1 || pred_zyx[a] > f[a])
      return fail(FFN_ERR_ARG, "pred size %d outside 1..%d (axis %d)", pred_zyx[a],
                  f[a], a);
    if (d[a] > pred_zyx[a] / 2)
      return fail(FFN_ERR_ARG, "delta %d beyond the prediction's half size %d (axis %d)",
                  d[a], pred_zyx[a] / 2, a);
    if ((f[a] - pred_zyx[a]) % 2 != 0)
      return fail(FFN_ERR_ARG, "seed size %d - pred size %d is odd (axis %d): the "
                  "prediction cannot be centred in the seed FoV", f[a], pred_zyx[a], a);
  }
  HIP_TRY(hipSetDevice(e->device));
  HIP_TRY(hipStreamSynchronize(e->stream));
  drop_spec(e);
  g.Vp = 1;
  g.crop = 0;
  for (int a = 0; a < 3; ++a) {
    g.c0[a] = (f[a] - pred_zyx[a]) / 2;
    g.c1[a] = g.c0[a] + pred_zyx[a];
    g.Vp *= pred_zyx[a];
    g.crop |= pred_zyx[a] != f[a];
  }
  return FFN_OK;
}

int ffn_engine_debug_flow_trace(ffn_engine* e, long long* out, int max_slots) {
  EngineLock lock_(e);
  if (!e || !out) return fail(FFN_ERR_ARG, "null argument");
  if (!e->flow_trace) return fail(FFN_ERR_ARG, "no flow trace on this engine (conv_variant 9)");
  if (max_slots < 0 || max_slots > e->flow_trace_slots)
    return fail(FFN_ERR_ARG, "max_slots must be 0..%d", e->flow_trace_slots);
  HIP_TRY(hipSetDevice(e->device));
  HIP_TRY(hipStreamSynchronize(e->stream));
  const size_t row = (size_t)kFlowTraceLayers * 8 * sizeof(long long);
  HIP_TRY(hipMemcpy(out, e->flow_trace, row * max_slots, hipMemcpyDeviceToHost));
  HIP_TRY(hipMemset(e->flow_trace, 0, row * e->flow_trace_slots));
  return FFN_OK;
}

int ffn_engine_debug_workgroups(ffn_engine* e, long long* out, int max_wgs) {
  EngineLock lock_(e);
  if (!e || !out) return fail(FFN_ERR_ARG, "null argument");
  if (max_wgs < 0 || max_wgs > kDbgMaxWgs)
    return fail(FFN_ERR_ARG, "max_wgs must be 0..%d", kDbgMaxWgs);
  HIP_TRY(hipSetDevice(e->device));
  HIP_TRY(hipStreamSynchronize(e->stream));
  HIP_TRY(hipMemcpy(out, e->d_dbg + 24, (size_t)4 * max_wgs * sizeof(long long),
                    hipMemcpyDeviceToHost));
  HIP_TRY(hipMemset(e->d_dbg + 24, 0, (size_t)4 * kDbgMaxWgs * sizeof(long long)));
  return FFN_OK;
}

int ffn_engine_debug_clocks(ffn_engine* e, long long* out24) {
  EngineLock lock_(e);
  if (!e || !out24) return fail(FFN_ERR_ARG, "null argument");
  HIP_TRY(hipSetDevice(e->device));
  HIP_TRY(hipStreamSynchronize(e->stream));
  HIP_TRY(hipMemcpy(out24, e->d_dbg, 24 * sizeof(long long), hipMemcpyDeviceToHost));
  return FFN_OK;
}

// ... 131 lines not shown
namespace {
int resolve_many_carry(ffn_engine* e, const ffn_canvas* only = nullptr);
}

void ffn_canvas_destroy(ffn_canvas* c) {
  if (c && c->engine) (void)resolve_many_carry(c->engine, c);
  EngineLock lock_(c ? c->engine : nullptr);
  if (!c) return;
  if (c->engine) {
    ffn_engine* e = c->engine;
    drop_spec(e);
    (void)hipSetDevice(e->device);
    (void)hipStreamSynchronize(e->stream);
    (void)hipStreamSynchronize(e->ustream);
    if (c->ev_util) (void)hipEventDestroy(c->ev_util);
    e->canvases.erase(std::remove(e->canvases.begin(), e->canvases.end(), c),
                      e->canvases.end());
    (void)hipFree(c->image);
    (void)hipFree(c->image_u8);
    (void)hipFree(c->image_lut);
    (void)hipFree(c->seed);
    (void)hipFree(c->seg);
    (void)hipFree(c->restrict_planes);
  }
  delete c;
}

int ffn_canvas_init_seed(ffn_canvas* c, const int32_t pos[3], float value) {
  UtilLock lock_(c ? c->engine : nullptr);
  if (!c || !pos) return fail(FFN_ERR_ARG, "null argument");
  if (pos[0] < 0 || pos[0] >= c->cz || pos[1] < 0 || pos[1] >= c->cy ||
      pos[2] < 0 || pos[2] >= c->cx)
    return fail(FFN_ERR_ARG, "seed position outside the canvas");
  ffn_engine* e = c->engine;
  if (!e) return fail(FFN_ERR_STATE, "canvas outlived its engine");
  HIP_TRY(hipSetDevice(e->device));
  HIP_TRY(lock_.begin(e, c));
  if (c->dirty_lo[0] < c->dirty_hi[0]) {
    long total = 0;
    Box b = make_box(c, c->dirty_lo, c->dirty_hi, &total);
    if ((size_t)total * 2 >= c->nvox) {
      hipLaunchKernelGGL(fill_u32_kernel, dim3(2048), dim3(256), 0, e->ustream,
                         reinterpret_cast<uint32_t*>(c->seed), 0x7fc00000u,
                         c->nvox);
    } else if (total > 0) {
      hipLaunchKernelGGL((box_fill_kernel<uint32_t>), dim3(grid_for(total)),
                         dim3(256), 0, e->ustream,
                         reinterpret_cast<uint32_t*>(c->seed), b, total,
                         0x7fc00000u);
    }
  }
  {
    const int lo[3] = {pos[0], pos[1], pos[2]};
    const int hi[3] = {pos[0] + 1, pos[1] + 1, pos[2] + 1};
    c->dirty_lo[0] = c->dirty_hi[0] = 0;
    c->mark_dirty(lo, hi);
  }
  const size_t ci = ((size_t)pos[0] * c->cy + pos[1]) * c->cx + pos[2];
  hipLaunchKernelGGL(set_seed_point_kernel, dim3(1), dim3(1), 0, e->ustream,
                     c->seed, ci, value);
  HIP_TRY(hipGetLastError());
  HIP_TRY(lock_.end(e, c));
  return FFN_OK;
}

int ffn_canvas_step_submit(ffn_engine* e, int n, ffn_canvas* const* canvases,
                           const ffn_step_request* requests,
                           const ffn_step_params* params, uint32_t* ticket) {
  EngineLock lock_(e);
  if (!e || !canvases || !requests || !params || !ticket)
    return fail(FFN_ERR_ARG, "null argument");
  if (n < 1 || n > e->max_batch)
    return fail(FFN_ERR_ARG, "batch %d outside [1, %d]", n, e->max_batch);
  if (!e->weights_set) return fail(FFN_ERR_STATE, "weights not set");
  const int slot = e->slot_n[e->next_slot] == 0 ? e->next_slot : e->next_slot ^ 1;
  if (e->slot_n[slot] != 0)
    return fail(FFN_ERR_STATE,
                "two steps already in flight: call ffn_canvas_step_wait first");
  HIP_TRY(hipSetDevice(e->device));
  const Geom& g = e->g;
  int hint_n = 0;
  int hint_pos[kSpecMax][3];
  bool from_loop = false;
  for (int k = 0; k < n; ++k)
    if (canvases[k]) {
      if (n == 1) {
        hint_n = canvases[k]->hint_n;
        std::memcpy(hint_pos, canvases[k]->hint_pos, sizeof(hint_pos));
        from_loop = canvases[k]->hint_from_loop;
      }
      canvases[k]->hint_n = 0;
      canvases[k]->hint_from_loop = false;
    }
  StepItem* h_items = e->h_items + (size_t)slot * e->max_batch;
  StepItem* d_items = e->d_items + (size_t)slot * e->max_batch;
  unsigned long long* h_pub = e->h_pub + (size_t)slot * e->max_batch * kPubWords;
  const int other = slot ^ 1;
  for (int k = 0; k < n; ++k) {
    const ffn_canvas* c = canvases[k];
    if (!c || c->engine != e) return fail(FFN_ERR_ARG, "canvas %d not of this engine", k);
    const ffn_step_request& r = requests[k];
    const int half[3] = {g.fz / 2, g.fy / 2, g.fx / 2};
    const int dims[3] = {c->cz, c->cy, c->cx};
    for (int a = 0; a < 3; ++a)
      if (r.pos[a] - half[a] < 0 || r.pos[a] + half[a] >= dims[a])
        return fail(FFN_ERR_ARG, "FoV at (%d,%d,%d) leaves the canvas", r.pos[0],
                    r.pos[1], r.pos[2]);
    if (r.num_candidates < 0 || r.num_candidates > FFN_MAX_CANDIDATES)
      return fail(FFN_ERR_ARG, "num_candidates out of range");
    for (int k2 = 0; k2 < k; ++k2)
      if (canvases[k2] == c)
        return fail(FFN_ERR_ARG, "canvas appears twice in one batch");
    for (int k2 = 0; k2 < e->slot_n[other]; ++k2)
      if (e->slot_canvas[other][k2] == c)
        return fail(FFN_ERR_STATE, "canvas %d already has a step in flight", k);
    {
      const int lo[3] = {r.pos[0] - half[0], r.pos[1] - half[1], r.pos[2] - half[2]};
      const int hi[3] = {r.pos[0] + half[0] + 1, r.pos[1] + half[1] + 1,
                         r.pos[2] + half[2] + 1};
      const_cast<ffn_canvas*>(c)->mark_dirty(lo, hi);
    }
    if (c->util_pending) {
      HIP_TRY(hipStreamWaitEvent(e->stream, c->ev_util, 0));
      const_cast<ffn_canvas*>(c)->util_pending = false;
    }
    const_cast<ffn_canvas*>(c)->paste_after_flag = n == 1;
    StepItem& it = h_items[k];
    it.image = c->image;
    it.image_u8 = c->image_u8;
    it.image_lut = c->image_lut;
    it.seed = c->seed;
    it.seg = c->seg;
    it.cz = c->cz;
    it.cy = c->cy;
    it.cx = c->cx;
    it.req = r;
  }
  HIP_TRY(hipSetDevice(e->device));
  StepItems si;
  si.items = d_items;
  si.use_inline = n == 1;
  si.inline_item = h_items[0];
  if (n > 1)
    HIP_TRY(hipMemcpyAsync(d_items, h_items, sizeof(StepItem) * n,
                           hipMemcpyHostToDevice, e->stream));
  int spec_expected = -1;
  if (e->spec.valid && n == 1 && from_loop && e->spec.canvas == canvases[0] &&
      e->spec.variant == e->conv_variant &&
      std::memcmp(&e->spec.pad_value, &params->pad_value, sizeof(float)) == 0 &&
      std::memcmp(&e->spec.move_thr, &params->move_threshold, sizeof(float)) == 0)
    for (int j = 0; j < e->spec.n && spec_expected < 0; ++j)
      if (std::memcmp(e->spec.pos[j], requests[0].pos, sizeof(int) * 3) == 0)
        spec_expected = j;
  if (spec_expected >= 0) e->stat_spec_hits += 1;
  else if (e->spec.valid && n == 1 && from_loop && e->spec.canvas == canvases[0]) {
    if (e->spec.n >= kSpecMax) e->stat_spec_miss_full += 1;
    else e->stat_spec_miss_short += 1;
  }
  if (spec_expected >= 0 && e->spec_force_mismatch > 0) {
    e->spec_force_mismatch -= 1;
    spec_expected = kSpecMax;
  }
  const bool traced = n == 1 && e->fused_trace_in > 0 && --e->fused_trace_in == 0;
  e->trace_now = traced;
  if (e->debug_submit_delay_ns > 0) {
    const long long t_d = steady_ns();
    while (steady_ns() - t_d < e->debug_submit_delay_ns) {}
  }
  int rc = FFN_OK;
  if (e->ahead_valid && spec_expected >= 0) {
    e->ahead_valid = false;
    e->spec.valid = false;
    e->stat_ahead_used += 1;
    if (e->ahead_ev_pending) {
      e->ahead_ev_pending = false;
      if (e->events_used + 2 > (int)e->events.size()) {
        rc = flush_events(e);
        if (rc) return rc;
      }
      e->chain_launches_pending.push_back(2 * e->depth - 1);
      std::swap(e->events[e->events_used++], e->ahead_ev[0]);
      std::swap(e->events[e->events_used++], e->ahead_ev[1]);
    }
  } else {
    rc = run_stack(e, n, si, params->pad_value, params->move_threshold,
                   spec_expected >= 0);
  }
  if (rc) return rc;
  const bool this_stack_resident = e->last_stack_resident;
  const unsigned step_id = ++e->step_id ? e->step_id : ++e->step_id;
  auto paste = [&]() {
    hipLaunchKernelGGL(paste_kernel, dim3(71, n), dim3(512), 0, e->stream, si, g,
                       e->logits, e->seed_raw, e->count, e->count_blocks,
                       params->move_threshold, params->disco_seed_threshold,
                       e->range_flag, e->range_tag,
                       e->d_spec_choice, spec_expected);
  };
  SpecArgs sp;
  sp.n = 0;
  sp.move_thr = params->move_threshold;
  sp.choice = nullptr;
  if (n == 1) {
    const ffn_canvas* c = canvases[0];
    const int half[3] = {g.fz / 2, g.fy / 2, g.fx / 2};
    const int dims[3] = {c->cz, c->cy, c->cx};
    for (int j = 0; j < hint_n && e->speculate; ++j) {
      bool inside = true;
      for (int a = 0; a < 3; ++a)
        if (hint_pos[j][a] - half[a] < 0 || hint_pos[j][a] + half[a] >= dims[a])
          inside = false;
      if (!inside) continue;
      for (int a = 0; a < 3; ++a) sp.pos[sp.n][a] = hint_pos[j][a];
      ++sp.n;
    }
    for (int j = sp.n; j < kSpecMax && sp.n > 0; ++j)
      for (int a = 0; a < 3; ++a) sp.pos[j][a] = sp.pos[0][a];
  }
  const bool fused_next = n == 1 && sp.n > 0 && e->fuse_paste && e->fuse_conv0a &&
                          e->conv_variant >= 6;
  if (n > 1) paste();
  if (fused_next) {
    Conv0Next nx;
    const int tiles = conv0a_split_args(e, params->pad_value, next_tag(e->range_tag), sp,
                                        true, nx);
    const int paste_blocks = e->paste_blocks > 0
        ? e->paste_blocks
        : std::max(kPasteBlocksMin, std::min(kPasteBlocks, e->cus - 1 - tiles));
    if (e->debug_fused_twice)
      hipLaunchKernelGGL(faces_paste_conv0a_kernel, dim3(1 + paste_blocks + tiles),
                         dim3(512), 0, e->stream, si, g, e->logits, e->seed_raw, e->count,
                         e->count_blocks, params->move_threshold,
                         params->disco_seed_threshold, params->deleted_threshold,
                         e->range_flag, e->range_tag, h_pub, step_id, e->d_spec_choice,
                         spec_expected, nx, e->d_stamps, 0, paste_blocks);
    hipLaunchKernelGGL(faces_paste_conv0a_kernel, dim3(1 + paste_blocks + tiles),
                       dim3(512), 0, e->stream, si, g, e->logits, e->seed_raw, e->count,
                       e->count_blocks, params->move_threshold,
                       params->disco_seed_threshold, params->deleted_threshold,
                       e->range_flag, e->range_tag, h_pub, step_id, e->d_spec_choice,
                       spec_expected, nx, e->d_stamps, e->trace_now ? 1 : 0, paste_blocks);
  } else if (n == 1 && e->fuse_paste) {
    hipLaunchKernelGGL(faces_paste_kernel, dim3(1 + 71), dim3(512), 0, e->stream, si,
                       g, e->logits, e->seed_raw, e->count, e->count_blocks,
                       params->move_threshold, params->disco_seed_threshold,
                       params->deleted_threshold, e->range_flag, e->range_tag,
                       h_pub, step_id, e->d_spec_choice, spec_expected);
  } else {
    hipLaunchKernelGGL(faces_kernel, dim3(n), dim3(512), 0, e->stream, si, g,
                       e->logits, e->seed_raw, e->count, e->count_blocks,
                       params->move_threshold, params->disco_seed_threshold,
                       params->deleted_threshold, e->range_flag, e->range_tag,
                       h_pub, step_id, e->d_spec_choice, spec_expected);
    if (n == 1) paste();
  }
  if (n == 1) {
    ffn_canvas* c = canvases[0];
    if (sp.n > 0) {
      if (!fused_next)
        launch_conv0a(e, 1, si, params->pad_value, next_tag(e->range_tag), sp, true);
      bool ahead = false;
      if (fused_next && e->stack_ahead && from_loop && this_stack_resident &&
          e->flow == 2 && e->flow_skip == 0 && e->conv_variant == 9) {
        rc = run_stack(e, 1, si, params->pad_value, params->move_threshold, true, true);
        if (rc) return rc;
        ahead = true;
      }
      e->ahead_valid = ahead;
      e->spec.valid = true;
      e->spec.canvas = c;
      e->spec.n = sp.n;
      std::memcpy(e->spec.pos, sp.pos, sizeof(sp.pos));
      e->spec.pad_value = params->pad_value;
      e->spec.move_thr = params->move_threshold;
      e->spec.variant = e->conv_variant;
      e->stat_spec_launched += 1;
    }
  }
  e->trace_now = false;
  HIP_TRY(hipGetLastError());
  e->stat_calls += 1;
  e->stat_items += n;
  e->stat_hist[n < 64 ? n : 64] += 1;
  e->slot_n[slot] = n;
  e->slot_resident[slot] = this_stack_resident;
  e->slot_ticket[slot] = step_id;
  e->slot_canvas[slot].assign(canvases, canvases + n);
  e->next_slot = other;
  *ticket = step_id;
  return FFN_OK;
}

namespace {
int step_wait_impl(ffn_engine* e, uint32_t ticket, ffn_step_result* results,
                   bool* spec_mismatch);
}

int ffn_canvas_step_wait(ffn_engine* e, uint32_t ticket,
                         ffn_step_result* results) {
  return step_wait_impl(e, ticket, results, nullptr);
}

namespace {
int step_wait_impl(ffn_engine* e, uint32_t ticket, ffn_step_result* results,
                   bool* spec_mismatch) {
  if (spec_mismatch) *spec_mismatch = false;
  if (!e || !results) return fail(FFN_ERR_ARG, "null argument");
  int slot = -1;
  int n = 0;
  {
    EngineLock lock_(e);
    for (int s = 0; s < 2; ++s)
      if (e->slot_n[s] != 0 && e->slot_ticket[s] == ticket && !e->slot_waited[s])
        slot = s;
    if (slot < 0)
      return fail(FFN_ERR_STATE, "no step with ticket %u in flight", ticket);
    n = e->slot_n[slot];
    e->slot_waited[slot] = true;
  }
  const unsigned step_id = ticket;
  unsigned long long* h_pub = e->h_pub + (size_t)slot * e->max_batch * kPubWords;
  struct SlotRelease {
    ffn_engine* e;
    int slot;
    ~SlotRelease() {
      EngineLock lock_(e);
      e->slot_n[slot] = 0;
      e->slot_waited[slot] = false;
      e->slot_canvas[slot].clear();
    }
  } release_{e, slot};
  HIP_TRY(hipSetDevice(e->device));
  auto arrived = [&]() {
    for (int k = 0; k < n * kPubWords; ++k)
      if ((unsigned)(__atomic_load_n(&h_pub[k], __ATOMIC_ACQUIRE) >> 32) != step_id)
        return false;
    return true;
  };
  if (e->sync_mode == 1) {
    bool done = false;
    long long t_first = 0, t_query = 0;
    for (long spin = 0; !done; ++spin) {
      done = arrived();
      if (!done && (spin & 0xfff) == 0xfff) {
        const long long now = steady_ns();
        if (t_first == 0) t_first = t_query = now;
        if (now - t_first > 10000000000LL) break;
        if (now - t_query > 2000000) {
          t_query = now;
          if (hipStreamQuery(e->stream) == hipSuccess)
            done = true;
        }
      }
    }
    if (!done) HIP_TRY(hipStreamSynchronize(e->stream));
  } else {
    HIP_TRY(hipStreamSynchronize(e->stream));
  }
  if (!arrived()) {
    HIP_TRY(hipStreamSynchronize(e->stream));
    if (!arrived()) return fail(FFN_ERR_HIP, "step %u did not complete", step_id);
  }
  if (n == 1) e->t_arrived_ns = steady_ns();
  {
    uint32_t* out = reinterpret_cast<uint32_t*>(results);
    for (int k = 0; k < n * kPubWords; ++k)
      out[k] = (uint32_t)__atomic_load_n(&h_pub[k], __ATOMIC_RELAXED);
  }
  for (int k = 0; k < n; ++k)
    if (results[k].range_error == 2) {
      if (spec_mismatch) {
        *spec_mismatch = true;
        return FFN_OK;
      }
      return fail(FFN_ERR_STATE,
                  "the speculative conv0_a launch of step %u chose another position "
                  "than the segment loop; the step changed nothing (speculate 0 "
                  "turns the launches off)", step_id);
    }
  bool any_void = false;
  for (int k = 0; k < n; ++k) any_void = any_void || results[k].range_error != 0;
  if (any_void) {
    bool timed_out = false;
    for (int k = 0; k < n; ++k) timed_out = timed_out || results[k].range_error == 3;
    const int frc = flow_voided(e, timed_out);
    if (frc) return frc;
  } else {
    EngineLock lock_(e);
    if (e->slot_resident[slot]) e->flow_strikes = 0;
  }
  for (int k = 0; k < n; ++k)
    if (results[k].range_error)
      return fail(FFN_ERR_RANGE,
                  "an activation left the fp16 range (conv_variant >= 6): the "
                  "step changed nothing; set conv_variant -1 and repeat it");
  return FFN_OK;
}
}

int ffn_canvas_step(ffn_engine* e, int n, ffn_canvas* const* canvases,
                    const ffn_step_request* requests,
                    const ffn_step_params* params, ffn_step_result* results) {
  if (!results) return fail(FFN_ERR_ARG, "null argument");
  uint32_t ticket = 0;
  int rc = ffn_canvas_step_submit(e, n, canvases, requests, params, &ticket);
  if (rc) return rc;
  bool mismatch = false;
  rc = step_wait_impl(e, ticket, results, &mismatch);
  if (rc || !mismatch) return rc;
  {
    EngineLock lock_(e);
    e->stat_spec_mismatch += 1;
    drop_spec(e);
  }
  rc = ffn_canvas_step_submit(e, n, canvases, requests, params, &ticket);
  if (rc) return rc;
  return step_wait_impl(e, ticket, results, nullptr);
}

namespace {
struct HipLoopDevice {
  ffn_canvas* c;
  int step(const ffn_step_request& req, const ffn_step_params& params,
           ffn_step_result* res) {
    ffn_canvas* one = c;
    return ffn_canvas_step(c->engine, 1, &one, &req, &params, res);
  }
  int read_point(const int32_t pos[3], float* seed, int32_t* seg) {
    return ffn_canvas_read_points(c, 1, pos, seed, seg);
  }
  void hint_next(int n, const int32_t (*pos)[3]) {
    EngineLock lock_(c->engine);
    c->hint_from_loop = true;
    c->hint_n = n < kSpecMax ? n : kSpecMax;
    for (int j = 0; j < c->hint_n; ++j)
      for (int a = 0; a < 3; ++a) c->hint_pos[j][a] = pos[j][a];
  }
};
}

namespace {
int resolve_many_carry_locked(ffn_engine* e) {
  if (!e->many_carry.active) return FFN_OK;
  HipLoopDevice dev{e->many_canvases.empty() ? nullptr : e->many_canvases[0]};
  auto wait = [&](ffn_step_result* res) {
    return step_wait_impl(e, e->many_ticket, res, nullptr);
  };
  const int rc = ffn_host::resolve_carry(&e->many_carry, dev, wait);
  e->many_canvases.clear();
  return rc;
}
int resolve_many_carry(ffn_engine* e, const ffn_canvas* only) {
  std::lock_guard<std::mutex> guard(e->many_mu);
  if (only && std::find(e->many_canvases.begin(), e->many_canvases.end(), only) ==
                  e->many_canvases.end())
    return FFN_OK;
  return resolve_many_carry_locked(e);
}
}

int ffn_canvas_segment_at(ffn_canvas* c, const int32_t start[3],
                          const ffn_segment_params* p, int resume,
                          ffn_segment_result* out) {
  if (!c || !start || !p || !out) return fail(FFN_ERR_ARG, "null argument");
  if (!c->engine) return fail(FFN_ERR_STATE, "canvas outlived its engine");
  if (int rc = resolve_many_carry(c->engine, c)) return rc;
  if (p->prefetch < 0 || p->prefetch > FFN_MAX_CANDIDATES)
    return fail(FFN_ERR_ARG, "prefetch must be 0..%d", FFN_MAX_CANDIDATES);
  if (p->shape_zyx[0] != c->cz || p->shape_zyx[1] != c->cy ||
      p->shape_zyx[2] != c->cx)
    return fail(FFN_ERR_ARG, "shape_zyx does not match the canvas");
  for (int a = 0; a < 3; ++a)
    if (p->deltas_zyx[a] < 0 || p->margin_zyx[a] < 0)
      return fail(FFN_ERR_ARG, "negative deltas / margin");
  if (resume && !c->loop.active)
    return fail(FFN_ERR_STATE, "no segment to resume");
  HipLoopDevice dev{c};
  ffn_host::SegmentLoop<HipLoopDevice> loop(dev, c->loop, *p);
  return loop.run(start, resume, out);
}

int ffn_canvas_segment_many(ffn_engine* e, int n, ffn_canvas* const* canvases,
                            const int32_t (*starts)[3],
                            const ffn_segment_params* params, const int32_t* resume,
                            ffn_segment_result* results, int32_t* finished) {
  return ffn_canvas_segment_many_carry(e, n, canvases, starts, params, resume, results,
                                       finished, 0);
}

int ffn_canvas_segment_many_carry(ffn_engine* e, int n, ffn_canvas* const* canvases,
                                  const int32_t (*starts)[3],
                                  const ffn_segment_params* params,
                                  const int32_t* resume, ffn_segment_result* results,
                                  int32_t* finished, int32_t carry) {
  if (!e || !canvases || !starts || !params || !resume || !results || !finished)
    return fail(FFN_ERR_ARG, "null argument");
  if (n < 1 || n > e->max_batch)
    return fail(FFN_ERR_ARG, "batch %d outside [1, %d]", n, e->max_batch);
  std::vector<HipLoopDevice> devs(n);
  std::vector<ffn_host::SegmentState*> states(n);
  for (int k = 0; k < n; ++k) {
    ffn_canvas* c = canvases[k];
    if (!c) return fail(FFN_ERR_ARG, "null canvas");
    if (c->engine != e) return fail(FFN_ERR_ARG, "canvas %d is not of this engine", k);
    for (int k2 = 0; k2 < k; ++k2)
      if (canvases[k2] == c) return fail(FFN_ERR_ARG, "canvas appears twice");
    const ffn_segment_params& p = params[k];
    if (p.prefetch < 0 || p.prefetch > FFN_MAX_CANDIDATES)
      return fail(FFN_ERR_ARG, "prefetch must be 0..%d", FFN_MAX_CANDIDATES);
    if (p.shape_zyx[0] != c->cz || p.shape_zyx[1] != c->cy || p.shape_zyx[2] != c->cx)
      return fail(FFN_ERR_ARG, "shape_zyx does not match canvas %d", k);
    for (int a = 0; a < 3; ++a)
      if (p.deltas_zyx[a] < 0 || p.margin_zyx[a] < 0)
        return fail(FFN_ERR_ARG, "negative deltas / margin");
    if (resume[k] && !c->loop.active)
      return fail(FFN_ERR_STATE, "canvas %d: no segment to resume", k);
    if (std::memcmp(&p.step, &params[0].step, sizeof(ffn_step_params)) != 0)
      return fail(FFN_ERR_ARG, "canvas %d: step parameters differ from canvas 0's", k);
    devs[k].c = c;
    states[k] = &c->loop;
  }
  std::vector<ffn_canvas*> batch(n);
  auto batch_step = [&](int nb, const int* idx, const ffn_step_request* reqs,
                        const ffn_step_params& sp, ffn_step_result* res) {
    for (int b = 0; b < nb; ++b) batch[b] = canvases[idx[b]];
    return ffn_canvas_step(e, nb, batch.data(), reqs, &sp, res);
  };
  std::unique_lock<std::mutex> many_guard(e->many_mu);
  if (!carry) {
    const int rc = resolve_many_carry_locked(e);
    many_guard.unlock();
    if (rc) return rc;
    return ffn_host::segment_many(n, devs.data(), states.data(), starts, params,
                                  resume, results, finished, batch_step);
  }
  auto submit = [&](int nb, const int* idx, const ffn_step_request* reqs,
                    const ffn_step_params& sp) {
    for (int b = 0; b < nb; ++b) batch[b] = canvases[idx[b]];
    const int rc = ffn_canvas_step_submit(e, nb, batch.data(), reqs, &sp,
                                          &e->many_ticket);
    if (rc == FFN_OK) {
      e->many_canvases.assign(batch.begin(), batch.begin() + nb);
      e->stat_many_carried += 1;
    }
    return rc;
  };
  auto wait = [&](ffn_step_result* res) {
    const int rc = step_wait_impl(e, e->many_ticket, res, nullptr);
    e->many_canvases.clear();
    return rc;
  };
  return ffn_host::segment_many(n, devs.data(), states.data(), starts, params, resume,
                                results, finished, batch_step, &e->many_carry, submit,
                                wait);
}

int ffn_canvas_segment_history(ffn_canvas* c, size_t first, size_t n,
                               int32_t* pos, uint32_t* deleted, size_t* total) {
  if (!c) return fail(FFN_ERR_ARG, "null canvas");
  if (c->engine)
    if (int rc = resolve_many_carry(c->engine, c)) return rc;
  const size_t have = c->loop.history_deleted.size();
  if (total) *total = have;
  if (n == 0) return FFN_OK;
  if (first > have || n > have - first)
    return fail(FFN_ERR_ARG, "history range [%zu, +%zu) of %zu", first, n, have);
  if (pos) std::memcpy(pos, c->loop.history.data() + 3 * first, 12 * n);
  if (deleted) std::memcpy(deleted, c->loop.history_deleted.data() + first, 4 * n);
  return FFN_OK;
}

int ffn_canvas_set_restrictor(ffn_canvas* c, const uint8_t* mask,
                              const uint8_t* seed_mask, const uint8_t* shift_mask,
                              const int32_t shift_shape[3], const int32_t pre[3],
                              const int32_t post[3], int32_t scale) {
  if (!c) return fail(FFN_ERR_ARG, "null canvas");
  ffn_engine* e = c->engine;
  if (!e) return fail(FFN_ERR_STATE, "canvas outlived its engine");
  if (shift_mask) {
    if (!shift_shape || !pre || !post)
      return fail(FFN_ERR_ARG, "shift mask without its shape / FoV offsets");
    for (int k = 0; k < 3; ++k) {
      if (shift_shape[k] < 1) return fail(FFN_ERR_ARG, "bad shift mask shape");
      if (post[k] < -1) return fail(FFN_ERR_ARG, "shift mask FoV ends before 0");
    }
    if (scale < 1) return fail(FFN_ERR_ARG, "shift mask scale must be >= 1");
  }
// ... 151 lines not shown
                     e->ustream, c->seed, c->seg, c->cz, c->cy, c->cx, n,
                     reinterpret_cast<const int32_t*>(ds), d_seed, d_seg);
  HIP_TRY(hipMemcpyAsync(hs + pbr, ds + pbr, 8 * (size_t)n, hipMemcpyDeviceToHost,
                         e->ustream));
  HIP_TRY(lock_.wait(e, c));
  std::memcpy(seed_out, hs + pbr, 4 * (size_t)n);
  std::memcpy(seg_out, hs + pbr + 4 * (size_t)n, 4 * (size_t)n);
  return FFN_OK;
}

int ffn_canvas_write_seg_points(ffn_canvas* c, int n, const int32_t* pos,
                                const int32_t* values) {
  UtilLock lock_(c ? c->engine : nullptr);
  if (!c || !pos || !values) return fail(FFN_ERR_ARG, "null argument");
  if (n < 1) return FFN_OK;
  for (int k = 0; k < n; ++k)
    if (pos[3 * k] < 0 || pos[3 * k] >= c->cz || pos[3 * k + 1] < 0 ||
        pos[3 * k + 1] >= c->cy || pos[3 * k + 2] < 0 || pos[3 * k + 2] >= c->cx)
      return fail(FFN_ERR_ARG, "point %d outside the canvas", k);
  ffn_engine* e = c->engine;
  if (!e) return fail(FFN_ERR_STATE, "canvas outlived its engine");
  HIP_TRY(hipSetDevice(e->device));
  HIP_TRY(lock_.begin(e, c));
  if (n == 1) {
    const size_t ci = ((size_t)pos[0] * c->cy + pos[1]) * c->cx + pos[2];
    hipLaunchKernelGGL(set_seg_point_kernel, dim3(1), dim3(1), 0, e->ustream, c->seg,
                       ci, values[0]);
    HIP_TRY(hipGetLastError());
    HIP_TRY(lock_.end(e, c));
    return FFN_OK;
  }
  const size_t pb = sizeof(int32_t) * 3 * n;
  const size_t pbr = (pb + 15) & ~(size_t)15;
  int rc = ensure_scratch(e, pbr + 4 * (size_t)n);
  if (rc) return rc;
  char* hs = static_cast<char*>(e->h_scratch);
  char* ds = static_cast<char*>(e->d_scratch);
  std::memcpy(hs, pos, pb);
  std::memcpy(hs + pbr, values, 4 * (size_t)n);
  HIP_TRY(hipMemcpyAsync(ds, hs, pbr + 4 * (size_t)n, hipMemcpyHostToDevice,
                         e->ustream));
  hipLaunchKernelGGL(points_write_seg_kernel, dim3((n + 63) / 64), dim3(64), 0,
                     e->ustream, c->seg, c->cy, c->cx, n,
                     reinterpret_cast<const int32_t*>(ds),
                     reinterpret_cast<const int32_t*>(ds + pbr));
  HIP_TRY(lock_.wait(e, c));
  return FFN_OK;
}

int ffn_canvas_any_segmented(ffn_canvas* c, const int32_t lo[3],
                             const int32_t hi[3], int32_t* out) {
  UtilLock lock_(c ? c->engine : nullptr);
  if (!c || !lo || !hi || !out) return fail(FFN_ERR_ARG, "null argument");
  int32_t l[3], h[3];
  const int dims[3] = {c->cz, c->cy, c->cx};
  for (int k = 0; k < 3; ++k) {
    l[k] = std::max(lo[k], 0);
    h[k] = std::min(hi[k], dims[k]);
    if (h[k] <= l[k]) {
      *out = 0;
      return FFN_OK;
    }
  }
  ffn_engine* e = c->engine;
  if (!e) return fail(FFN_ERR_STATE, "canvas outlived its engine");
  HIP_TRY(hipSetDevice(e->device));
  HIP_TRY(lock_.begin(e, c));
  int rc = ensure_scratch(e, 16);
  if (rc) return rc;
  long total;
  Box b = make_box(c, l, h, &total);
  HIP_TRY(hipMemsetAsync(e->d_scratch, 0, 4, e->ustream));
  hipLaunchKernelGGL(any_segmented_kernel, dim3(grid_for(total)), dim3(256), 0,
                     e->ustream, c->seg, b, total,
                     static_cast<int32_t*>(e->d_scratch));
  HIP_TRY(hipMemcpyAsync(e->h_scratch, e->d_scratch, 4, hipMemcpyDeviceToHost,
                         e->ustream));
  HIP_TRY(lock_.wait(e, c));
  *out = *static_cast<int32_t*>(e->h_scratch);
  return FFN_OK;
}

int ffn_canvas_commit_count(ffn_canvas* c, const int32_t lo[3],
                            const int32_t hi[3], float segment_threshold,
                            int32_t max_existing_id, ffn_commit_counts* counts,
                            int32_t max_overlaps, int32_t* overlap_ids,
                            int64_t* overlap_counts) {
  UtilLock lock_(c ? c->engine : nullptr);
  if (!c || !lo || !hi || !counts) return fail(FFN_ERR_ARG, "null argument");
  int rc = check_box(c, lo, hi);
  if (rc) return rc;
  if (max_existing_id < 0) max_existing_id = 0;
  ffn_engine* e = c->engine;
  if (!e) return fail(FFN_ERR_STATE, "canvas outlived its engine");
  HIP_TRY(hipSetDevice(e->device));
  HIP_TRY(lock_.begin(e, c));
  const size_t hist_n = (size_t)max_existing_id + 1;
  const size_t bytes = 16 + hist_n * sizeof(unsigned);
  rc = ensure_scratch(e, bytes);
  if (rc) return rc;
  long total;
  Box b = make_box(c, lo, hi, &total);
  HIP_TRY(hipMemsetAsync(e->d_scratch, 0, bytes, e->ustream));
  auto* d_counts = static_cast<unsigned long long*>(e->d_scratch);
  auto* d_hist = reinterpret_cast<unsigned*>(static_cast<char*>(e->d_scratch) + 16);
  if (total > 0)
    hipLaunchKernelGGL(commit_count_kernel, dim3(grid_for(total)), dim3(256), 0,
                       e->ustream, c->seed, c->seg, b, total, segment_threshold,
                       max_existing_id, d_counts, d_hist);
  HIP_TRY(hipMemcpyAsync(e->h_scratch, e->d_scratch, bytes, hipMemcpyDeviceToHost,
                         e->ustream));
  HIP_TRY(lock_.wait(e, c));
  const auto* hc = static_cast<const unsigned long long*>(e->h_scratch);
  const auto* hh = reinterpret_cast<const unsigned*>(
      static_cast<const char*>(e->h_scratch) + 16);
  counts->raw_segmented_voxels = (int64_t)hc[0];
  counts->actual_segmented_voxels = (int64_t)hc[1];
  int nover = 0;
  for (size_t id = 1; id < hist_n; ++id) {
    if (hh[id]) {
      if (nover < max_overlaps && overlap_ids && overlap_counts) {
        overlap_ids[nover] = (int32_t)id;
        overlap_counts[nover] = (int64_t)hh[id];
      }
      ++nover;
    }
  }
  counts->num_overlapped_ids = nover;
  return FFN_OK;
}

int ffn_canvas_commit_assign(ffn_canvas* c, const int32_t lo[3],
                             const int32_t hi[3], float segment_threshold,
                             int32_t segment_id) {
  UtilLock lock_(c ? c->engine : nullptr);
  if (!c || !lo || !hi) return fail(FFN_ERR_ARG, "null argument");
  int rc = check_box(c, lo, hi);
  if (rc) return rc;
  ffn_engine* e = c->engine;
  if (!e) return fail(FFN_ERR_STATE, "canvas outlived its engine");
  HIP_TRY(hipSetDevice(e->device));
  HIP_TRY(lock_.begin(e, c));
  long total;
  Box b = make_box(c, lo, hi, &total);
  if (total > 0)
    hipLaunchKernelGGL(commit_assign_kernel, dim3(grid_for(total)), dim3(256), 0,
                       e->ustream, c->seed, c->seg, b, total, segment_threshold,
                       segment_id);
  HIP_TRY(hipGetLastError());
  HIP_TRY(lock_.end(e, c));
  return FFN_OK;
}

int ffn_canvas_segment_turn(ffn_canvas* c, const ffn_turn_request* rq,
                            const int32_t* cand, ffn_turn_result* out,
                            int32_t max_overlaps, int32_t* overlap_ids,
                            int64_t* overlap_counts, int32_t* cand_flags,
                            float* cand_seed, int32_t* cand_seg) {
  UtilLock lock_(c ? c->engine : nullptr);
  if (!c || !rq || !out) return fail(FFN_ERR_ARG, "null argument");
  const int n = rq->num_candidates;
  if (n < 0 || (n > 0 && (!cand || !cand_flags || !cand_seed || !cand_seg)))
    return fail(FFN_ERR_ARG, "candidate arrays");
  int rc = FFN_OK;
  if (rq->do_commit && (rc = check_box(c, rq->lo, rq->hi))) return rc;
  auto inside = [&](const int32_t* p) {
    return p[0] >= 0 && p[0] < c->cz && p[1] >= 0 && p[1] < c->cy && p[2] >= 0 &&
           p[2] < c->cx;
  };
  if (rq->mark_mode && !inside(rq->mark_pos))
    return fail(FFN_ERR_ARG, "marker outside the canvas");
  for (int k = 0; k < n; ++k)
    if (!inside(cand + 3 * k)) return fail(FFN_ERR_ARG, "candidate %d outside the canvas", k);
  for (int a = 0; a < 3; ++a)
    if (rq->min_boundary_dist[a] < 0) return fail(FFN_ERR_ARG, "min_boundary_dist");
  ffn_engine* e = c->engine;
  if (!e) return fail(FFN_ERR_STATE, "canvas outlived its engine");
  HIP_TRY(hipSetDevice(e->device));
  const long long t_turn0 = steady_ns();
  HIP_TRY(lock_.begin(e, c));
  const int32_t max_id = rq->do_commit ? std::max(rq->max_existing_id, 0) : 0;
  const size_t hist_n = rq->do_commit ? (size_t)max_id + 1 : 0;
  const size_t o_hist = sizeof(TurnRecord);
  const size_t o_flag = (o_hist + hist_n * 4 + 15) & ~(size_t)15;
  const size_t o_cand = o_flag + 12 * (size_t)n;
  const size_t bytes = o_cand + 12 * (size_t)n;
  rc = ensure_scratch(e, bytes);
  if (rc) return rc;
  char* ds = static_cast<char*>(e->d_scratch);
  char* hs = static_cast<char*>(e->h_scratch);
  auto* d_rec = reinterpret_cast<TurnRecord*>(ds);
  auto* d_hist = reinterpret_cast<unsigned*>(ds + o_hist);
  auto* d_flag = reinterpret_cast<int*>(ds + o_flag);
  auto* d_cseed = reinterpret_cast<float*>(ds + o_flag + 4 * (size_t)n);
  auto* d_cseg = reinterpret_cast<int32_t*>(ds + o_flag + 8 * (size_t)n);
  auto* d_cand = reinterpret_cast<int32_t*>(ds + o_cand);
  HIP_TRY(hipMemsetAsync(ds, 0, o_flag, e->ustream));
  HIP_TRY(hipMemsetAsync(&d_rec->chosen, 0xff, 4, e->ustream));
  if (n > 0) {
    std::memcpy(hs + o_cand, cand, 12 * (size_t)n);
    HIP_TRY(hipMemcpyAsync(d_cand, hs + o_cand, 12 * (size_t)n, hipMemcpyHostToDevice,
                           e->ustream));
  }
  long total = 0;
  Box b{};
  if (rq->do_commit) {
    b = make_box(c, rq->lo, rq->hi, &total);
    if (total > 0)
      hipLaunchKernelGGL(commit_count_kernel, dim3(grid_for(total)), dim3(256), 0,
                         e->ustream, c->seed, c->seg, b, total, rq->segment_threshold,
                         max_id, d_rec->counts, d_hist);
  }
  if (rq->do_commit || rq->mark_mode) {
    const long mark_ci =
        rq->mark_mode ? ((long)rq->mark_pos[0] * c->cy + rq->mark_pos[1]) * c->cx +
                            rq->mark_pos[2]
                      : 0;
    hipLaunchKernelGGL(turn_commit_kernel, dim3(total > 0 ? grid_for(total) : 1),
                       dim3(256), 0, e->ustream, c->seed, c->seg, b, total,
                       rq->segment_threshold, rq->segment_id,
                       (long long)rq->min_segment_size, d_rec, mark_ci, rq->mark_mode);
  }
  long dirty_total = 0;
  if (n > 0) {
    hipLaunchKernelGGL(turn_eval_kernel, dim3(n), dim3(64), 0, e->ustream, c->seed,
                       c->seg, c->cz, c->cy, c->cx, d_cand, rq->min_boundary_dist[0],
                       rq->min_boundary_dist[1], rq->min_boundary_dist[2], d_flag,
                       d_cseed, d_cseg, c->restrict_planes, c->restrict_plane_words,
                       c->restrict_row_words);
    hipLaunchKernelGGL(turn_pick_kernel, dim3(1), dim3(64), 0, e->ustream, c->seg,
                       c->cy, c->cx, d_cand, n, d_flag, d_rec);
    if (rq->do_init) {
      if (c->dirty_lo[0] < c->dirty_hi[0]) {
        Box db = make_box(c, c->dirty_lo, c->dirty_hi, &dirty_total);
        const int linear = (size_t)dirty_total * 2 >= c->nvox;
        if (dirty_total > 0)
          hipLaunchKernelGGL(turn_clear_kernel,
                             dim3(linear ? 2048 : grid_for(dirty_total)), dim3(256), 0,
                             e->ustream, reinterpret_cast<uint32_t*>(c->seed), db,
                             dirty_total, linear, c->nvox, d_rec);
      }
      hipLaunchKernelGGL(turn_seed_kernel, dim3(1), dim3(1), 0, e->ustream, c->seed,
                         c->cy, c->cx, d_cand, rq->init_value, d_rec);
    }
  }
  HIP_TRY(hipGetLastError());
  HIP_TRY(hipMemcpyAsync(hs, ds, o_cand, hipMemcpyDeviceToHost, e->ustream));
  const long long t_turn1 = steady_ns();
  HIP_TRY(lock_.wait(e, c));
  e->stat_segturn_queue_ns += t_turn1 - t_turn0;
  e->stat_segturn_wait_ns += steady_ns() - t_turn1;
  e->stat_segturn_calls += 1;
  const auto* hr = reinterpret_cast<const TurnRecord*>(hs);
  std::memset(out, 0, sizeof(*out));
  out->counts.raw_segmented_voxels = (int64_t)hr->counts[0];
  out->counts.actual_segmented_voxels = (int64_t)hr->counts[1];
  out->committed = hr->committed;
  out->chosen = n > 0 ? hr->chosen : -1;
  const auto* hh = reinterpret_cast<const unsigned*>(hs + o_hist);
  int nover = 0;
  for (size_t id = 1; id < hist_n; ++id) {
    if (hh[id]) {
      if (nover < max_overlaps && overlap_ids && overlap_counts) {
        overlap_ids[nover] = (int32_t)id;
        overlap_counts[nover] = (int64_t)hh[id];
      }
      ++nover;
    }
  }
  out->counts.num_overlapped_ids = nover;
  if (n > 0) {
    std::memcpy(cand_flags, hs + o_flag, 4 * (size_t)n);
    std::memcpy(cand_seed, hs + o_flag + 4 * (size_t)n, 4 * (size_t)n);
    std::memcpy(cand_seg, hs + o_flag + 8 * (size_t)n, 4 * (size_t)n);
    if (rq->do_init && out->chosen >= 0) {
      const int32_t* p = cand + 3 * out->chosen;
      const int lo[3] = {p[0], p[1], p[2]};
      const int hi[3] = {p[0] + 1, p[1] + 1, p[2] + 1};
      c->dirty_lo[0] = c->dirty_hi[0] = 0;
      c->mark_dirty(lo, hi);
    }
  }
  return FFN_OK;
}

}

namespace {

template <typename T>
int box_read(ffn_canvas* c, const T* vol, const int32_t lo[3], const int32_t hi[3],
             T* dst) {
  UtilLock lock_(c ? c->engine : nullptr);
  if (!c || !lo || !hi || !dst) return fail(FFN_ERR_ARG, "null argument");
  int rc = check_box(c, lo, hi);
  if (rc) return rc;
  ffn_engine* e = c->engine;
  if (!e) return fail(FFN_ERR_STATE, "canvas outlived its engine");
  HIP_TRY(hipSetDevice(e->device));
  long total;
  Box b = make_box(c, lo, hi, &total);
  if (total == 0) return FFN_OK;
  if (total == (long)c->nvox) {
    HIP_TRY(canvas_quiesce(e, c));
    HIP_TRY(hipMemcpy(dst, vol, sizeof(T) * total, hipMemcpyDeviceToHost));
    return FFN_OK;
  }
  HIP_TRY(lock_.begin(e, c));
  rc = ensure_scratch(e, sizeof(T) * total);
  if (rc) return rc;
  hipLaunchKernelGGL((box_read_kernel<T>), dim3(grid_for(total)), dim3(256), 0,
                     e->ustream, vol, b, total, static_cast<T*>(e->d_scratch));
  HIP_TRY(hipMemcpyAsync(e->h_scratch, e->d_scratch, sizeof(T) * total,
                         hipMemcpyDeviceToHost, e->ustream));
  HIP_TRY(lock_.wait(e, c));
  std::memcpy(dst, e->h_scratch, sizeof(T) * total);
  return FFN_OK;
}

template <typename T>
int box_write(ffn_canvas* c, T* vol, const int32_t lo[3], const int32_t hi[3],
              const T* src) {
  UtilLock lock_(c ? c->engine : nullptr);
  if (!c || !lo || !hi || !src) return fail(FFN_ERR_ARG, "null argument");
  int rc = check_box(c, lo, hi);
  if (rc) return rc;
  ffn_engine* e = c->engine;
  if (!e) return fail(FFN_ERR_STATE, "canvas outlived its engine");
  HIP_TRY(hipSetDevice(e->device));
  long total;
  Box b = make_box(c, lo, hi, &total);
  if (total == 0) return FFN_OK;
  if (total == (long)c->nvox) {
    HIP_TRY(canvas_quiesce(e, c));
    HIP_TRY(hipMemcpy(vol, src, sizeof(T) * total, hipMemcpyHostToDevice));
    return FFN_OK;
  }
  HIP_TRY(lock_.begin(e, c));
  rc = ensure_scratch(e, sizeof(T) * total);
  if (rc) return rc;
  std::memcpy(e->h_scratch, src, sizeof(T) * total);
  HIP_TRY(hipMemcpyAsync(e->d_scratch, e->h_scratch, sizeof(T) * total,
                         hipMemcpyHostToDevice, e->ustream));
  hipLaunchKernelGGL((box_write_kernel<T>), dim3(grid_for(total)), dim3(256), 0,
                     e->ustream, vol, b, total,
                     static_cast<const T*>(e->d_scratch));
  HIP_TRY(lock_.wait(e, c));
  return FFN_OK;
}

}

extern "C" {

int ffn_canvas_read_seed(ffn_canvas* c, const int32_t lo[3], const int32_t hi[3],
                         float* dst) {
  return box_read<float>(c, c ? c->seed : nullptr, lo, hi, dst);
}

int ffn_canvas_read_segmentation(ffn_canvas* c, const int32_t lo[3],
                                 const int32_t hi[3], int32_t* dst) {
  return box_read<int32_t>(c, c ? c->seg : nullptr, lo, hi, dst);
}

int ffn_canvas_write_seed(ffn_canvas* c, const int32_t lo[3], const int32_t hi[3],
                          const float* src) {
  if (c && lo && hi) c->mark_dirty(lo, hi);
  return box_write<float>(c, c ? c->seed : nullptr, lo, hi, src);
}

int ffn_canvas_write_segmentation(ffn_canvas* c, const int32_t lo[3],
                                  const int32_t hi[3], const int32_t* src) {
  return box_write<int32_t>(c, c ? c->seg : nullptr, lo, hi, src);
}

}
```

### ffn_amd/csrc/ffn_host_loop.h

```cpp
#pragma once

#include <cstdlib>
#include <algorithm>
#include <cstdint>
#include <cstring>
#include <deque>
#include <unordered_map>
#include <unordered_set>
#include <vector>

#include "../../include/ffn_hip.h"

namespace ffn_host {

struct Coord {
  int32_t z, y, x;
  bool operator==(const Coord& o) const { return z == o.z && y == o.y && x == o.x; }
};

struct CoordHash {
  size_t operator()(const Coord& c) const {
    uint64_t h = (uint64_t)(uint32_t)c.z * 0x9E3779B97F4A7C15ull;
    h ^= (uint64_t)(uint32_t)c.y * 0xC2B2AE3D27D4EB4Full + (h << 6) + (h >> 2);
    h ^= (uint64_t)(uint32_t)c.x * 0x165667B19E3779F9ull + (h << 6) + (h >> 2);
    return (size_t)h;
  }
};

inline int32_t floordiv(int32_t a, int32_t b) {
  int32_t q = a / b;
  if ((a % b != 0) && (a < 0)) --q;
  return q;
}

struct SegmentState {
  struct Entry {
    float score;
    Coord pos;
    Coord q;
  };
  std::deque<Entry> queue;
  std::unordered_set<Coord, CoordHash> done;
  std::unordered_map<Coord, std::pair<float, int32_t>, CoordHash> cache;
  Coord start{0, 0, 0};
  float start_logit = 0.f;
  bool start_logit_known = false;
  bool active = false;
  bool has_pending = false;
  Coord pending{0, 0, 0};
  int32_t min_pos[3] = {0, 0, 0}, max_pos[3] = {0, 0, 0};
  std::vector<int32_t> history;
  std::vector<uint32_t> history_deleted;
  int64_t many_steps = 0, many_skip_threshold = 0, many_skip_invalid_pos = 0,
          many_gate_rejects = 0;
  const uint64_t* restrict_bits = nullptr;
  int32_t restrict_dims[3] = {0, 0, 0};
  int64_t restrict_row_words = 0;
  int64_t skip_restricted = 0;

  bool pos_blocked(const Coord& c) const {
    if (!restrict_bits) return false;
    if (c.z < 0 || c.y < 0 || c.x < 0 || c.z >= restrict_dims[0] ||
        c.y >= restrict_dims[1] || c.x >= restrict_dims[2])
      return false;
    const uint64_t w =
        restrict_bits[((int64_t)c.z * restrict_dims[1] + c.y) * restrict_row_words +
                      (c.x >> 6)];
    return (w >> (c.x & 63)) & 1u;
  }
};

constexpr int kHintMax = 3;

struct StepPending {
  Coord pos;
  Coord cands[FFN_MAX_CANDIDATES];
  int nc = 0;
  ffn_step_request req;
};

struct ManyCarry {
  struct Item {
    SegmentState* st;
    ffn_segment_params params;
    StepPending pd;
  };
  bool active = false;
  std::vector<Item> items;
};

template <class Dev>
class SegmentLoop {
 public:
  SegmentLoop(Dev& dev, SegmentState& st, const ffn_segment_params& p)
      : dev_(dev), st_(st), p_(p) {
    for (int a = 0; a < 3; ++a) {
      d_[a] = p.deltas_zyx[a];
      dh_[a] = d_[a] / 2;
      dm_[a] = d_[a] > 1 ? d_[a] : 1;
    }
  }

  int run(const int32_t start[3], int resume, ffn_segment_result* out) {
    int rc = begin(start, resume, out);
    if (rc) return rc;
    for (;;) {
      Pending pd;
      bool ended = false;
      rc = prepare(&pd, out, &ended);
      if (rc || ended) break;
      int32_t hint[kHintMax][3];
      const int nh = guess_next(pd.pos, hint);
      dev_.hint_next(nh, hint);
      ffn_step_result res;
      rc = dev_.step(pd.req, p_.step, &res);
      if (rc) {
        step_failed(pd);
        break;
      }
      consume(pd, res);
    }
    finish(out);
    return rc;
  }

  typedef StepPending Pending;

  int begin(const int32_t start[3], int resume, ffn_segment_result* out) {
    std::memset(out, 0, sizeof(*out));
    steps_ = 0;
    if (!resume) {
      st_.queue.clear();
      st_.done.clear();
      st_.cache.clear();
      st_.history.clear();
      st_.history_deleted.clear();
      st_.start = Coord{start[0], start[1], start[2]};
      st_.has_pending = false;
      st_.active = true;
      for (int a = 0; a < 3; ++a) {
        st_.min_pos[a] = p_.init_min_pos[a];
        st_.max_pos[a] = p_.init_max_pos[a];
      }
      st_.start_logit_known = p_.initial_start_logit == p_.initial_start_logit;
      st_.start_logit = p_.initial_start_logit;
      push((float)(p_.score_threshold * 2.0), st_.start);
    } else if (!st_.active) {
      return FFN_ERR_STATE;
    }
    return FFN_OK;
  }

  int prepare(Pending* pd, ffn_segment_result* out, bool* ended) {
    *ended = false;
    if (p_.max_steps > 0 && steps_ >= p_.max_steps) {
      out->budget_exhausted = 1;
      *ended = true;
      return FFN_OK;
    }
    Coord pos;
    for (;;) {
      if (st_.has_pending) {
        pos = st_.pending;
      } else {
        bool found = false;
        const int rc = next(&pos, &found, out);
        if (rc) return rc;
        if (!found) {
          st_.active = false;
          *ended = true;
          return FFN_OK;
        }
      }
      if (!st_.start_logit_known) {
        int32_t seg;
        const int32_t sp[3] = {st_.start.z, st_.start.y, st_.start.x};
        const int rc = dev_.read_point(sp, &st_.start_logit, &seg);
        if (rc) {
          st_.pending = pos;
          st_.has_pending = true;
          return rc;
        }
        st_.start_logit_known = true;
      }
      if (st_.start_logit < p_.step.move_threshold) {
        out->seed_got_too_weak = 1;
        st_.has_pending = false;
        st_.active = false;
        *ended = true;
        return FFN_OK;
      }
      if (!st_.pos_blocked(pos)) break;
      ++st_.skip_restricted;
      st_.has_pending = false;
    }
    pd->pos = pos;
    ffn_step_request& req = pd->req;
    req.pos[0] = pos.z, req.pos[1] = pos.y, req.pos[2] = pos.x;
    req.start_pos[0] = st_.start.z, req.start_pos[1] = st_.start.y,
    req.start_pos[2] = st_.start.x;
    pd->nc = peek(pd->cands, p_.prefetch < FFN_MAX_CANDIDATES
                                 ? p_.prefetch : FFN_MAX_CANDIDATES);
    req.num_candidates = pd->nc;
    for (int k = 0; k < pd->nc; ++k) {
      req.candidates[k][0] = pd->cands[k].z;
      req.candidates[k][1] = pd->cands[k].y;
      req.candidates[k][2] = pd->cands[k].x;
    }
    st_.pending = pos;
    st_.has_pending = true;
    return FFN_OK;
  }

  void step_failed(const Pending& pd) {
    st_.pending = pd.pos;
    st_.has_pending = true;
  }

  void consume(const Pending& pd, const ffn_step_result& res) {
    const Coord& pos = pd.pos;
    st_.has_pending = false;
    ++steps_;
    st_.cache.clear();
    for (int k = 0; k < pd.nc; ++k)
      st_.cache.emplace(pd.cands[k],
// ... 305 lines not shown
```

### ffn_amd/csrc/ffn_step_kernels.h

```cpp
#pragma once

namespace ffn {

struct StepItems {
  const StepItem* items;
  StepItem inline_item;
  int use_inline;
};

#define FFN_GLOBAL __attribute__((address_space(1)))
struct ItemView {
  const FFN_GLOBAL float* image;
  const FFN_GLOBAL uint8_t* image_u8;
  const FFN_GLOBAL float* image_lut;
  FFN_GLOBAL float* seed;
  const FFN_GLOBAL int32_t* seg;
  int cz, cy, cx;
  int pos[3];
  const ffn_step_request* req;
};
template <bool INLINE_ONLY = false>
__device__ __forceinline__ ItemView item_view(const StepItems& si, int item) {
  ItemView v;
#define FFN_VIEW_FROM(S)                                                        \
  v.image = (const FFN_GLOBAL float*)(S).image;                                  \
  v.image_u8 = (const FFN_GLOBAL uint8_t*)(S).image_u8;                          \
  v.image_lut = (const FFN_GLOBAL float*)(S).image_lut;                          \
  v.seed = (FFN_GLOBAL float*)(S).seed;                                          \
  v.seg = (const FFN_GLOBAL int32_t*)(S).seg;                                    \
  v.cz = (S).cz, v.cy = (S).cy, v.cx = (S).cx;                                   \
  v.pos[0] = (S).req.pos[0], v.pos[1] = (S).req.pos[1], v.pos[2] = (S).req.pos[2]; \
  v.req = &(S).req;
  if (INLINE_ONLY || si.use_inline) {
    FFN_VIEW_FROM(si.inline_item)
    asm volatile("" : "+s"(v.pos[0]), "+s"(v.pos[1]), "+s"(v.pos[2]));
  } else {
    FFN_VIEW_FROM(si.items[item])
    asm volatile("" : "+v"(v.pos[0]), "+v"(v.pos[1]), "+v"(v.pos[2]));
  }
#undef FFN_VIEW_FROM
  return v;
}

constexpr int kC0Z = 4, kC0Y = 8, kC0X = 8;
constexpr int kC0Threads = 512;

struct Conv0SplitOut {
  char* out_sp;
  long sp_plane_bytes;
  long item_bytes;
  unsigned* range_flag;
  unsigned range_tag;
};
typedef _Float16 f16x8_c0 __attribute__((ext_vector_type(8)));
typedef _Float16 f16x4_c0 __attribute__((ext_vector_type(4)));

constexpr int kSpecMax = 3;
struct SpecArgs {
  int n;
  int pos[kSpecMax][3];
  float move_thr;
  int* choice;
};

struct SeedOverlay {
  int on;
  int disco;
  const float* lg;
  const float* old;
  int z0, y0, x0;
  int fy, fx;
  int c0[3], c1[3];
};

__device__ __forceinline__ float post_disco(float lg, float old, bool disco);

__device__ __forceinline__ int overlay_index(const SeedOverlay& ov, int Z, int Y, int X) {
  const int lz = Z - ov.z0, ly = Y - ov.y0, lx = X - ov.x0;
  const bool in = ov.on && lz >= ov.c0[0] && lz < ov.c1[0] && ly >= ov.c0[1] &&
                  ly < ov.c1[1] && lx >= ov.c0[2] && lx < ov.c1[2];
  return in ? (lz * ov.fy + ly) * ov.fx + lx : -1;
}

struct Conv0NoResolve {
  __device__ void operator()(SeedOverlay&) const {}
};
template <bool SPLIT, class Resolve = Conv0NoResolve>
__device__ __forceinline__ void conv0a_body(
    const int tile_block, const int item, const StepItems& si, float pad_value,
    const float* __restrict__ w ,
    const float* __restrict__ bias, float* __restrict__ out,
    float* __restrict__ seed_raw, const Geom& g, int tiles_y, int tiles_x,
    const Conv0SplitOut& so, const SpecArgs& sp, const SeedOverlay& ov_in,
    long long* tr = nullptr, Resolve resolve = Resolve()) {
  SeedOverlay ov = ov_in;
  auto stamp = [&](int k) {
    if (tr && threadIdx.x == 0 && (tile_block & 7) == 0)
      atomicMax(reinterpret_cast<unsigned long long*>(tr + k), (unsigned long long)wall_clock64());
  };
  constexpr int HZ = kC0Z + 2, HY = kC0Y + 2, HX = kC0X + 2;
  __shared__ float tile[HZ * HY * HX * 2];
  __shared__ float s_lut[256];
  __shared__ __attribute__((aligned(16))) float otile[SPLIT ? 256 * 36 : 4];
  const ItemView it = item_view(si, item);
  int b = tile_block;
  const int tx = b % tiles_x;
  b /= tiles_x;
  const int ty = b % tiles_y;
  const int tz = b / tiles_y;
  const int oz = tz * kC0Z, oy = ty * kC0Y, ox = tx * kC0X;
  const long cstr[3] = {(long)it.cy * it.cx, (long)it.cx, 1};
  const long sz = cstr[g.oa[0]], sy = cstr[g.oa[1]], sx = cstr[g.oa[2]];
  int pos[3] = {it.pos[0], it.pos[1], it.pos[2]};

  const int lane = threadIdx.x & 63;
  const int wave = __builtin_amdgcn_readfirstlane(threadIdx.x >> 6);
  const int i = lane & 15;
  const int grp = lane >> 4;

  constexpr int kC0Per = (HZ * HY * HX + kC0Threads - 1) / kC0Threads;
  const bool u8 = it.image == nullptr;
  float g_img[kC0Per] = {}, g_seed[kC0Per];
  unsigned g_raw[kC0Per] = {};
  float o_l[kC0Per] = {}, o_o[kC0Per] = {};
  int g_ov[kC0Per];
  long g_out[kC0Per];
  bool g_in[kC0Per];
  int g_zz[kC0Per], g_yy[kC0Per], g_xx[kC0Per];
#pragma unroll
  for (int k = 0; k < kC0Per; ++k) {
    const int e = threadIdx.x + k * kC0Threads;
    const int ec = e < HZ * HY * HX ? e : 0;
    const int hx = ec % HX;
    const int t = ec / HX;
    const int hy = t % HY;
    const int hz = t / HY;
    const int zz = oz + hz - 1, yy = oy + hy - 1, xx = ox + hx - 1;
    g_zz[k] = zz, g_yy[k] = yy, g_xx[k] = xx;
    g_in[k] = e < HZ * HY * HX && zz >= 0 && zz < g.fz && yy >= 0 && yy < g.fy &&
              xx >= 0 && xx < g.fx;
    g_out[k] = (g_in[k] && hz >= 1 && hz <= kC0Z && hy >= 1 && hy <= kC0Y &&
                hx >= 1 && hx <= kC0X)
                   ? (long)((size_t)item * g.V + (size_t)zz * g.dstr[0] +
                            yy * g.dstr[1] + xx * g.dstr[2])
                   : -1;
  }
  auto issue_gather = [&](const int* p3) {
    const int pz = g.oa[0] == 0 ? p3[0] : g.oa[0] == 1 ? p3[1] : p3[2];
    const int py = g.oa[1] == 0 ? p3[0] : g.oa[1] == 1 ? p3[1] : p3[2];
    const int px = g.oa[2] == 0 ? p3[0] : g.oa[2] == 1 ? p3[1] : p3[2];
    const int z0 = pz - g.fz / 2;
    const int y0 = py - g.fy / 2;
    const int x0 = px - g.fx / 2;
    size_t g_ci[kC0Per];
#pragma unroll
    for (int k = 0; k < kC0Per; ++k) {
      g_ci[k] = g_in[k] ? (size_t)((z0 + g_zz[k]) * sz + (y0 + g_yy[k]) * sy +
                                   (x0 + g_xx[k]) * sx)
                        : 0;
      g_ov[k] = -1;
      if (ov.on && g_in[k]) {
        int cc[3];
        cc[g.oa[0]] = z0 + g_zz[k];
        cc[g.oa[1]] = y0 + g_yy[k];
        cc[g.oa[2]] = x0 + g_xx[k];
        g_ov[k] = overlay_index(ov, cc[0], cc[1], cc[2]);
      }
    }
    if (u8) {
#pragma unroll
      for (int k = 0; k < kC0Per; ++k) g_raw[k] = it.image_u8[g_ci[k]];
    } else {
#pragma unroll
      for (int k = 0; k < kC0Per; ++k) g_img[k] = it.image[g_ci[k]];
    }
#pragma unroll
    for (int k = 0; k < kC0Per; ++k) g_seed[k] = it.seed[g_ci[k]];
    if (ov.on) {
#pragma unroll
      for (int k = 0; k < kC0Per; ++k) {
        o_l[k] = ov.lg[g_ov[k] < 0 ? 0 : g_ov[k]];
        o_o[k] = ov.old[g_ov[k] < 0 ? 0 : g_ov[k]];
      }
    }
  };

  float bw[2][14];
#pragma unroll
  for (int s = 0; s < 14; ++s) {
    const int kk = 4 * s + grp;
#pragma unroll
    for (int h = 0; h < 2; ++h)
      bw[h][s] = kk < 54 ? w[kk * kFeatures + 16 * h + i] : 0.0f;
  }
  const float bias0 = bias[i], bias1 = bias[16 + i];
  float lut_v = 0.0f;
  if (u8 && threadIdx.x < 256) lut_v = it.image_lut[threadIdx.x];

  if (sp.n > 0) {
    float sv[kSpecMax];
    int gv[kSpecMax];
    int ovi[kSpecMax];
    float ol[kSpecMax], oo[kSpecMax];
#pragma unroll
    for (int k = 0; k < kSpecMax; ++k) {
      const size_t ci =
          ((size_t)sp.pos[k][0] * it.cy + sp.pos[k][1]) * it.cx + sp.pos[k][2];
      sv[k] = it.seed[ci];
      gv[k] = it.seg[ci];
      ovi[k] = overlay_index(ov, sp.pos[k][0], sp.pos[k][1], sp.pos[k][2]);
// ... 6 lines not shown
    if (tr && threadIdx.x == 0 && tile_block == 0) tr[21] = wall_clock64();
#pragma unroll
    for (int k = 0; k < kSpecMax; ++k)
      if (ov.on && ovi[k] >= 0) sv[k] = post_disco(ol[k], oo[k], ov.disco != 0);
#pragma unroll
    for (int k = 0; k < kSpecMax; ++k)
      asm volatile("" : "+v"(sv[k]), "+v"(gv[k]));
    int ch = -1;
#pragma unroll
    for (int k = kSpecMax - 1; k >= 0; --k)
      if (k < sp.n && !(sv[k] < sp.move_thr) && gv[k] <= 0) ch = k;
    if (tile_block == 0 && threadIdx.x == 0) *sp.choice = ch;
    if (ch < 0) return;
    stamp(16);
    if (tr && threadIdx.x == 0 && tile_block == 0) tr[22] = wall_clock64();
#pragma unroll
    for (int k = 0; k < kSpecMax; ++k)
      if (k == ch) {
        pos[0] = sp.pos[k][0];
        pos[1] = sp.pos[k][1];
        pos[2] = sp.pos[k][2];
      }
    if (ch != 0) issue_gather(pos);
  } else {
    issue_gather(pos);
    resolve(ov);
  }

  if (ov.on) {
#pragma unroll
    for (int k = 0; k < kC0Per; ++k)
      if (g_ov[k] >= 0) g_seed[k] = post_disco(o_l[k], o_o[k], ov.disco != 0);
  }
  if (u8 && threadIdx.x < 256) s_lut[threadIdx.x] = lut_v;
  __syncthreads();
#pragma unroll
  for (int k = 0; k < kC0Per; ++k) {
    const int e = threadIdx.x + k * kC0Threads;
    if (e >= HZ * HY * HX) continue;
    float vi = 0.0f, vs = 0.0f;
    if (g_in[k]) {
      vi = u8 ? s_lut[g_raw[k]] : g_img[k];
      vs = g_seed[k];
      if (g_out[k] >= 0) seed_raw[g_out[k]] = vs;
      if (vs != vs) vs = pad_value;
    }
    tile[2 * e] = vi;
    tile[2 * e + 1] = vs;
  }
  __syncthreads();
  stamp(17);

  const int ch = grp & 1;
#pragma unroll
  for (int m = 0; m < 2; ++m) {
    const int lp = (wave * 2 + m) * kTile + i;
    const int lx = lp % kC0X;
    const int ly = (lp / kC0X) % kC0Y;
    const int lz = lp / (kC0X * kC0Y);
    const int abase = ((lz * HY + ly) * HX + lx) * 2 + ch;
    f32x4 acc0 = {bias0, bias0, bias0, bias0};
    f32x4 acc1 = {bias1, bias1, bias1, bias1};
#pragma unroll
    for (int s = 0; s < 14; ++s) {
      int tap = 2 * s + (grp >> 1);
      tap = tap > 26 ? 26 : tap;
      const int kz = tap / 9, ky = (tap / 3) % 3, kx = tap % 3;
      const float av = tile[abase + ((kz * HY + ky) * HX + kx) * 2];
      acc0 = __builtin_amdgcn_mfma_f32_16x16x4f32(av, bw[0][s], acc0, 0, 0, 0);
      acc1 = __builtin_amdgcn_mfma_f32_16x16x4f32(av, bw[1][s], acc1, 0, 0, 0);
    }
#pragma unroll
    for (int r = 0; r < 4; ++r) {
      const int op = (wave * 2 + m) * kTile + grp * 4 + r;
      if constexpr (SPLIT) {
        otile[op * 36 + i] = fmaxf(acc0[r], 0.0f);
        otile[op * 36 + 16 + i] = fmaxf(acc1[r], 0.0f);
        continue;
      }
      const int ox_ = op % kC0X;
      const int oy_ = (op / kC0X) % kC0Y;
      const int oz_ = op / (kC0X * kC0Y);
      const int z = oz + oz_, y = oy + oy_, x = ox + ox_;
      if (z >= g.fz || y >= g.fy || x >= g.fx) continue;
      const size_t p = (size_t)z * g.plane + (size_t)y * g.XS + x;
      float* o = out + (size_t)item * g.act_stride + p * kFeatures;
      o[i] = fmaxf(acc0[r], 0.0f);
      o[16 + i] = fmaxf(acc1[r], 0.0f);
    }
  }
  stamp(18);
  if constexpr (SPLIT) {
    __syncthreads();
    unsigned range_max = 0;
    char* ob = so.out_sp + (long)item * so.item_bytes;
    const __amdgpu_buffer_rsrc_t rs_out =
        __builtin_amdgcn_make_buffer_rsrc(ob, 0, 0x7fffffff, 0x00020000);
#pragma unroll
    for (int k = 0; k < 2; ++k) {
      const int e = threadIdx.x + kC0Threads * k;
      const int c = e >> 8, op = e & 255;
      const int ox_ = op % kC0X;
      const int oy_ = (op / kC0X) % kC0Y;
      const int oz_ = op / (kC0X * kC0Y);
      const int z = oz + oz_, y = oy + oy_, x = ox + ox_;
      if (z >= g.fz || y >= g.fy || x >= g.fx) continue;
      const long p = (long)z * g.plane + (long)y * g.XS + x;
      const f32x4 va = *reinterpret_cast<const f32x4*>(otile + op * 36 + c * 8);
      const f32x4 vb = *reinterpret_cast<const f32x4*>(otile + op * 36 + c * 8 + 4);
      f16x8_c0 hi, res;
#pragma unroll
      for (int h = 0; h < 2; ++h) {
        const f32x4 v = h ? vb : va;
        f32x4 vh = v;
#pragma unroll
        for (int cc = 0; cc < 4; ++cc) {
          const unsigned mbits = __float_as_uint(v[cc]) & 0x7fffffffu;
          range_max = mbits > range_max ? mbits : range_max;
          vh[cc] = mbits < 0x38800000u ? 0.0f : v[cc];
        }
        const f16x4_c0 h4 = __builtin_convertvector(vh, f16x4_c0);
        const f32x4 r1 = (v - __builtin_convertvector(h4, f32x4)) * 2048.0f;
        const f16x4_c0 r4 = __builtin_convertvector(r1, f16x4_c0);
#pragma unroll
        for (int cc = 0; cc < 4; ++cc) {
          hi[4 * h + cc] = h4[cc];
          res[4 * h + cc] = r4[cc];
        }
      }
      typedef unsigned u32x4_c0 __attribute__((ext_vector_type(4)));
      __builtin_amdgcn_raw_buffer_store_b128(
          __builtin_bit_cast(u32x4_c0, hi), rs_out,
          (unsigned)((long)c * so.sp_plane_bytes + p * 16), 0, 16);
      __builtin_amdgcn_raw_buffer_store_b128(
          __builtin_bit_cast(u32x4_c0, res), rs_out,
          (unsigned)((long)(4 + c) * so.sp_plane_bytes + p * 16), 0, 16);
    }
    if (__ballot(range_max > 0x477fe000u) && lane == 0)
      *so.range_flag = so.range_tag;
  }
}

template <bool SPLIT>
__global__ __launch_bounds__(kC0Threads) void conv0a_mfma_kernel(
    StepItems si, float pad_value, const float* __restrict__ w ,
    const float* __restrict__ bias, float* __restrict__ out,
    float* __restrict__ seed_raw, Geom g, int tiles_y, int tiles_x,
    Conv0SplitOut so, SpecArgs sp) {
  SeedOverlay ov;
  ov.on = 0;
  conv0a_body<SPLIT>(blockIdx.x, blockIdx.y, si, pad_value, w, bias, out, seed_raw, g,
                     tiles_y, tiles_x, so, sp, ov);
}


__global__ __launch_bounds__(256) void head_kernel(
    const float* __restrict__ X, const float* __restrict__ in_seed,
    float pad_value, const float* __restrict__ wl ,
    float move_thr, float* __restrict__ logits,
    unsigned* __restrict__ block_count , Geom g) {
  __shared__ unsigned wave_cnt[4];
  const int item = blockIdx.y;
  const int sub = threadIdx.x & 7;
  const f32x4 w4 = *reinterpret_cast<const f32x4*>(wl + sub * 4);
  const float bias = wl[kFeatures];
  unsigned mine = 0;
  for (int v0 = blockIdx.x * 32; v0 < g.V; v0 += gridDim.x * 32) {
    const int v = v0 + (threadIdx.x >> 3);
    float partial = 0.0f;
    const bool live = v < g.V;
    if (live) {
      const int x = v % g.fx;
      const int t = v / g.fx;
      const int y = t % g.fy;
      const int z = t / g.fy;
      const size_t p = (size_t)z * g.plane + y * g.XS + x;
      const f32x4 a = *reinterpret_cast<const f32x4*>(
          X + (size_t)item * g.act_stride + p * kFeatures + sub * 4);
      partial = fmaxf(a[0], 0.f) * w4[0];
      partial = __builtin_fmaf(fmaxf(a[1], 0.f), w4[1], partial);
      partial = __builtin_fmaf(fmaxf(a[2], 0.f), w4[2], partial);
      partial = __builtin_fmaf(fmaxf(a[3], 0.f), w4[3], partial);
    }
    partial += __shfl_xor(partial, 1);
    partial += __shfl_xor(partial, 2);
    partial += __shfl_xor(partial, 4);
    bool above = false;
    if (live && sub == 0) {
      float s = in_seed[(size_t)item * g.V + v];
      if (s != s) s = pad_value;
      const float lg = s + (partial + bias);
      logits[(size_t)item * g.V + v] = lg;
      above = lg >= move_thr;
    }
    mine += (unsigned)__popcll(__ballot(above));
  }
  if ((threadIdx.x & 63) == 0) wave_cnt[threadIdx.x >> 6] = mine;
  __syncthreads();
  if (threadIdx.x == 0)
    block_count[item * gridDim.x + blockIdx.x] =
        wave_cnt[0] + wave_cnt[1] + wave_cnt[2] + wave_cnt[3];
}

__device__ __forceinline__ float post_disco(float lg, float old, bool disco) {
  return (disco && old < 0.0f && lg > old) ? old : lg;
}

__device__ __forceinline__ bool disco_on(unsigned cnt, int V, float thr) {
  return thr >= 0.0f && ((double)cnt / (double)V) > (double)thr;
}

__device__ __forceinline__ unsigned sum_block_counts(
    const unsigned* __restrict__ block_count, int head_blocks, int item,
    unsigned* s_cnt ) {
  unsigned part = 0;
  for (int e = threadIdx.x; e < head_blocks; e += blockDim.x)
    part += block_count[item * head_blocks + e];
#pragma unroll
  for (int off = 32; off > 0; off >>= 1) part += __shfl_xor(part, off);
  if ((threadIdx.x & 63) == 0) s_cnt[threadIdx.x >> 6] = part;
  __syncthreads();
  unsigned cnt = 0;
  for (int wv = 0; wv < (int)(blockDim.x >> 6); ++wv) cnt += s_cnt[wv];
  return cnt;
}

__device__ __forceinline__ unsigned step_count(
    const Geom& g, const float* __restrict__ lg, float move_thr,
    const unsigned* __restrict__ block_count, int head_blocks, int item,
    unsigned* s_cnt) {
  if (!g.crop) return sum_block_counts(block_count, head_blocks, item, s_cnt);
  unsigned part = 0;
  for (int v = threadIdx.x; v < g.V; v += blockDim.x) {
    const int x = v % g.fx, t = v / g.fx;
    part += (in_pred_box(g, t / g.fy, t % g.fy, x) && lg[v] >= move_thr) ? 1u : 0u;
  }
#pragma unroll
  for (int off = 32; off > 0; off >>= 1) part += __shfl_xor(part, off);
  if ((threadIdx.x & 63) == 0) s_cnt[threadIdx.x >> 6] = part;
  __syncthreads();
  unsigned cnt = 0;
  for (int wv = 0; wv < (int)(blockDim.x >> 6); ++wv) cnt += s_cnt[wv];
  return cnt;
}

constexpr int kPubWords = (int)(sizeof(ffn_step_result) / 4);

__device__ __forceinline__ void faces_body(
    const int item, const StepItems& si, const Geom& g,
    const float* __restrict__ logits, const float* __restrict__ in_seed,
    const unsigned* __restrict__ block_count, int head_blocks, float move_thr,
    float disco_thr, float deleted_thr, const unsigned* __restrict__ range_flag,
    unsigned range_tag, unsigned long long* __restrict__ pub, unsigned step_id,
    const int* __restrict__ spec_choice, int spec_expected, long long* tr = nullptr) {
  __shared__ unsigned s_cnt[8];
  __shared__ ffn_step_result s_res;
  const ItemView it = item_view(si, item);
  const float* lg = logits + (size_t)item * g.V;
  const float* old = in_seed + (size_t)item * g.V;
  const int z0 = it.pos[0] - g.fz / 2;
  const int y0 = it.pos[1] - g.fy / 2;
  const int x0 = it.pos[2] - g.fx / 2;
  const int wave = threadIdx.x >> 6;
  const int lane = threadIdx.x & 63;
  unsigned cnt_part = 0;
  if (!g.crop)
    for (int e = threadIdx.x; e < head_blocks; e += blockDim.x)
      cnt_part += block_count[item * head_blocks + e];
  const int f_axis = wave >> 1;
  const int f_sign = (wave & 1) ? 1 : -1;
  const int f_cz = g.c0[0] + (g.c1[0] - g.c0[0]) / 2;
  const int f_cy = g.c0[1] + (g.c1[1] - g.c0[1]) / 2;
  const int f_cx = g.c0[2] + (g.c1[2] - g.c0[2]) / 2;
  const int f_nr = f_axis == 0 ? 2 * g.dy + 1 : 2 * g.dz + 1;
  const int f_nc = f_axis == 2 ? 2 * g.dy + 1 : 2 * g.dx + 1;
  const int f_total = f_nr * f_nc;
  auto face_zyx = [&](int e, int& z, int& y, int& x) {
    const int fi = e / f_nc, fj = e - fi * f_nc;
    z = f_axis == 0 ? f_cz + f_sign * g.dz : f_cz - g.dz + fi;
    y = f_axis == 1 ? f_cy + f_sign * g.dy
                    : (f_axis == 0 ? f_cy - g.dy + fi : f_cy - g.dy + fj);
    x = f_axis == 2 ? f_cx + f_sign * g.dx : f_cx - g.dx + fj;
  };
  constexpr int kFaceSweep = 8;
  const bool one_sweep = f_total <= kFaceSweep * 64;
  float fa[kFaceSweep], fb[kFaceSweep];
  int fs[kFaceSweep];
  if (wave < 6 && one_sweep) {
#pragma unroll
    for (int k = 0; k < kFaceSweep; ++k) {
      const int e = k * 64 + lane;
      int z, y, x;
      face_zyx(e < f_total ? e : 0, z, y, x);
      const int v = (z * g.fy + y) * g.fx + x;
      fa[k] = lg[v];
      fb[k] = old[v];
      fs[k] = it.seg[((size_t)(z0 + z) * it.cy + (y0 + y)) * it.cx + (x0 + x)];
    }
  }
  float c_lg = 0.f, c_old = 0.f, c_seed = 0.f;
  int c_seg = 0, c_kind = 0;
  if (wave == 6) {
    const int n = it.req->num_candidates;
    if (lane <= n && lane <= FFN_MAX_CANDIDATES) {
      const int32_t* q = lane == 0 ? it.req->start_pos : it.req->candidates[lane - 1];
      const int z = q[0], y = q[1], x = q[2];
// ... 87 lines not shown
        best = ob;
        besti = oi;
      }
    }
    if (tr && threadIdx.x == 0) tr[13] = wall_clock64();
    if (lane == 0) {
      s_res.face_score[wave] = best;
      s_res.face_index[wave] = besti;
      int sg = 0;
      if (besti != 0x7fffffff && !one_sweep) {
        const int fi = besti / nc, fj = besti - fi * nc;
        const int z = axis == 0 ? cz + sign * g.dz : cz - g.dz + fi;
        const int y = axis == 1 ? cy + sign * g.dy
                                : (axis == 0 ? cy - g.dy + fi : cy - g.dy + fj);
        const int x = axis == 2 ? cx + sign * g.dx : cx - g.dx + fj;
        sg = it.seg[((size_t)(z0 + z) * it.cy + (y0 + y)) * it.cx + (x0 + x)];
      }
      s_res.face_seg[wave] = sg;
    }
    if (one_sweep) {
      int mine = 0;
#pragma unroll
      for (int k = 0; k < kFaceSweep; ++k) mine = (besti >> 6) == k ? fs[k] : mine;
      const int sgv = __shfl(mine, besti == 0x7fffffff ? 0 : (besti & 63));
      if (lane == 0) s_res.face_seg[wave] = besti == 0x7fffffff ? 0 : sgv;
    }
  } else if (wave == 6) {
    const int n = it.req->num_candidates;
    if (lane <= n && lane <= FFN_MAX_CANDIDATES) {
      const float sv = c_kind == 1   ? post_disco(c_lg, c_old, disco)
                       : c_kind == 2 ? c_seed
                                     : __builtin_nanf("");
      const int gv = c_seg;
      if (lane == 0) {
        s_res.start_logit = sv;
        s_res.num_above_move = cnt;
        s_res.disco_applied = disco ? 1 : 0;
      } else {
        s_res.cand_seed[lane - 1] = sv;
        s_res.cand_seg[lane - 1] = gv;
      }
    }
  } else {
    unsigned deleted = 0;
    if (deleted_thr == deleted_thr) {
      for (int v = lane; v < g.V; v += 64) {
        const int x = v % g.fx, t = v / g.fx;
        deleted += ((!g.crop || in_pred_box(g, t / g.fy, t % g.fy, x)) &&
                    old[v] >= deleted_thr && lg[v] < 0.0f) ? 1u : 0u;
      }
#pragma unroll
      for (int off = 32; off > 0; off >>= 1) deleted += __shfl_xor(deleted, off);
    }
    if (lane == 0) {
      s_res.num_deleted = deleted;
      s_res.range_error = (*range_flag == range_tag) ? (range_flag[1] == range_tag ? 3 : 1)
                          : (spec_expected >= 0 && *spec_choice != spec_expected) ? 2
                                                                                  : 0;
    }
  }
  __syncthreads();
  if (tr && threadIdx.x == 0) tr[14] = wall_clock64();
  if (wave == 0) {
    const uint32_t* src = reinterpret_cast<const uint32_t*>(&s_res);
    unsigned long long* dst = pub + (size_t)item * kPubWords;
    for (int k = lane; k < kPubWords; k += 64)
      __hip_atomic_store(&dst[k], ((unsigned long long)step_id << 32) | src[k],
                         __ATOMIC_RELAXED, __HIP_MEMORY_SCOPE_SYSTEM);
  }
}

__global__ __launch_bounds__(512) void faces_kernel(
    StepItems si, Geom g, const float* __restrict__ logits,
    const float* __restrict__ in_seed,
    const unsigned* __restrict__ block_count, int head_blocks, float move_thr,
    float disco_thr, float deleted_thr, const unsigned* __restrict__ range_flag,
    unsigned range_tag, unsigned long long* __restrict__ pub, unsigned step_id,
    const int* __restrict__ spec_choice, int spec_expected) {
  faces_body(blockIdx.x, si, g, logits, in_seed, block_count, head_blocks, move_thr,
             disco_thr, deleted_thr, range_flag, range_tag, pub, step_id,
             spec_choice, spec_expected);
}

__device__ __forceinline__ void paste_body(
    const int item, const int bx, const int nbx, const StepItems& si, const Geom& g,
    const float* __restrict__ logits, const float* __restrict__ in_seed,
    const unsigned* __restrict__ block_count, int head_blocks, float move_thr,
    float disco_thr, const unsigned* __restrict__ range_flag, unsigned range_tag,
    const int* __restrict__ spec_choice, int spec_expected) {
  __shared__ unsigned s_cnt[8];
  if (*range_flag == range_tag) return;
  if (spec_expected >= 0 && *spec_choice != spec_expected) return;
  const ItemView it = item_view(si, item);
  const float* lg = logits + (size_t)item * g.V;
  const float* old = in_seed + (size_t)item * g.V;
  const unsigned cnt = step_count(g, lg, move_thr, block_count, head_blocks, item, s_cnt);
  const bool disco = disco_on(cnt, g.Vp, disco_thr);
  const int z0 = it.pos[0] - g.fz / 2;
  const int y0 = it.pos[1] - g.fy / 2;
  const int x0 = it.pos[2] - g.fx / 2;
  for (int v = bx * blockDim.x + threadIdx.x; v < g.V; v += nbx * blockDim.x) {
    const int x = v % g.fx;
    const int t = v / g.fx;
    const int y = t % g.fy;
    const int z = t / g.fy;
    if (g.crop && !in_pred_box(g, z, y, x)) continue;
    const size_t ci = ((size_t)(z0 + z) * it.cy + (y0 + y)) * it.cx + (x0 + x);
    it.seed[ci] = post_disco(lg[v], old[v], disco);
  }
}

__global__ __launch_bounds__(512) void paste_kernel(
    StepItems si, Geom g, const float* __restrict__ logits,
    const float* __restrict__ in_seed,
    const unsigned* __restrict__ block_count, int head_blocks, float move_thr,
    float disco_thr, const unsigned* __restrict__ range_flag,
    unsigned range_tag, const int* __restrict__ spec_choice, int spec_expected) {
  paste_body(blockIdx.y, blockIdx.x, gridDim.x, si, g, logits, in_seed, block_count,
             head_blocks, move_thr, disco_thr, range_flag, range_tag, spec_choice,
             spec_expected);
}

__global__ __launch_bounds__(512) void faces_paste_kernel(
    StepItems si, Geom g, const float* __restrict__ logits,
    const float* __restrict__ in_seed,
    const unsigned* __restrict__ block_count, int head_blocks, float move_thr,
    float disco_thr, float deleted_thr, const unsigned* __restrict__ range_flag,
    unsigned range_tag, unsigned long long* __restrict__ pub, unsigned step_id,
    const int* __restrict__ spec_choice, int spec_expected) {
  if (blockIdx.x == 0)
    faces_body(0, si, g, logits, in_seed, block_count, head_blocks, move_thr,
               disco_thr, deleted_thr, range_flag, range_tag, pub, step_id,
               spec_choice, spec_expected);
  else
    paste_body(0, blockIdx.x - 1, gridDim.x - 1, si, g, logits, in_seed, block_count,
               head_blocks, move_thr, disco_thr, range_flag, range_tag, spec_choice,
               spec_expected);
}

constexpr int kPasteBlocks = 71;
constexpr int kPasteBlocksMin = 16;
struct Conv0Next {
  float pad_value;
  const float* w;
  const float* bias;
  float* out;
  float* seed_raw;
  Geom q;
  int tiles_y, tiles_x;
  Conv0SplitOut so;
  SpecArgs sp;
};

__global__ __launch_bounds__(512) void faces_paste_conv0a_kernel(
    StepItems si, Geom g, const float* __restrict__ logits,
    const float* __restrict__ in_seed,
    const unsigned* __restrict__ block_count, int head_blocks, float move_thr,
    float disco_thr, float deleted_thr, const unsigned* __restrict__ range_flag,
    unsigned range_tag, unsigned long long* __restrict__ pub, unsigned step_id,
    const int* __restrict__ spec_choice, int spec_expected, Conv0Next nx,
    long long* __restrict__ stamps, int trace, int paste_blocks) {
  static_assert(kC0Threads == 512, "one block size for the three roles");
  const long long t_in = wall_clock64();
  warm_kernargs<832>();
  const long long t_warm = wall_clock64();
  const bool tr_on = stamps && trace != 0;
  struct RoleStamp {
    long long* lo;
    long long* hi;
    bool on;
    __device__ RoleStamp(long long* l, long long* h, bool o)
        : lo(l), hi(h), on(o && (blockIdx.x <= 1 || (blockIdx.x & 7) == 0)) {
      if (on && threadIdx.x == 0)
        atomicMin(reinterpret_cast<unsigned long long*>(lo), (unsigned long long)wall_clock64());
    }
    __device__ ~RoleStamp() {
      if (on && threadIdx.x == 0)
        atomicMax(reinterpret_cast<unsigned long long*>(hi), (unsigned long long)wall_clock64());
    }
  };
  if (blockIdx.x == 0) {
    RoleStamp rs(stamps + 4, stamps + 8, tr_on);
    faces_body(0, si, g, logits, in_seed, block_count, head_blocks, move_thr,
               disco_thr, deleted_thr, range_flag, range_tag, pub, step_id,
               spec_choice, spec_expected, tr_on ? stamps : nullptr);
    if (stamps && threadIdx.x == 0) stamps[0] = wall_clock64();
    return;
  }
  if ((int)blockIdx.x <= paste_blocks) {
    RoleStamp rs(stamps + 5, stamps + 9, tr_on);
    paste_body(0, blockIdx.x - 1, paste_blocks, si, g, logits, in_seed, block_count,
               head_blocks, move_thr, disco_thr, range_flag, range_tag, spec_choice,
               spec_expected);
    return;
  }
  RoleStamp rs(stamps + 6, stamps + 10, tr_on);
  if (tr_on && threadIdx.x == 0) {
    if (((blockIdx.x - 1 - paste_blocks) & 7) == 0)
      atomicMax(reinterpret_cast<unsigned long long*>(stamps + 23), (unsigned long long)t_in);
    if ((int)blockIdx.x == 1 + paste_blocks) stamps[24] = t_warm;
  }
  __shared__ unsigned s_cnt[8];
  const ItemView it = item_view<true>(si, 0);
  int z = 0;
  asm volatile("" : "+v"(z));
  unsigned rf = range_flag[z];
  int sc = spec_choice[z];
  const int e0 = (int)threadIdx.x < head_blocks ? (int)threadIdx.x : 0;
  unsigned part = block_count[e0];
  SeedOverlay ov;
  ov.on = 1;
  ov.disco = 0;
  ov.lg = logits;
  ov.old = in_seed;
  ov.z0 = it.pos[0] - g.fz / 2;
  ov.y0 = it.pos[1] - g.fy / 2;
  ov.x0 = it.pos[2] - g.fx / 2;
  ov.fy = g.fy;
  ov.fx = g.fx;
#pragma unroll
  for (int a = 0; a < 3; ++a) {
    ov.c0[a] = g.c0[a];
    ov.c1[a] = g.c1[a];
  }
  auto resolve = [&](SeedOverlay& o) {
    asm volatile("" : "+v"(rf), "+v"(sc), "+v"(part) : : "memory");
    unsigned cnt;
    if (g.crop) {
      cnt = step_count(g, logits, move_thr, block_count, head_blocks, 0, s_cnt);
    } else {
      unsigned p2 = (int)threadIdx.x < head_blocks ? part : 0u;
      for (int e = kC0Threads + (int)threadIdx.x; e < head_blocks; e += kC0Threads)
        p2 += block_count[e];
#pragma unroll
      for (int off = 32; off > 0; off >>= 1) p2 += __shfl_xor(p2, off);
      if ((threadIdx.x & 63) == 0) s_cnt[threadIdx.x >> 6] = p2;
      __syncthreads();
      cnt = 0;
#pragma unroll
      for (int wv = 0; wv < kC0Threads / 64; ++wv) cnt += s_cnt[wv];
    }
    o.on = !(rf == range_tag || (spec_expected >= 0 && sc != spec_expected));
    o.disco = disco_on(cnt, g.Vp, disco_thr) ? 1 : 0;
  };
  conv0a_body<true>(blockIdx.x - 1 - paste_blocks, 0, si, nx.pad_value, nx.w, nx.bias,
                    nx.out, nx.seed_raw, nx.q, nx.tiles_y, nx.tiles_x, nx.so, nx.sp, ov,
                    tr_on ? stamps : nullptr, resolve);
}

}
```

Baseline: 5143.

## Fuse segment-turn kernels, publish results via host-mapped memory, and speculate next step

Merges the turn eval and pick kernels into one launch using a last-block-done counter, and merges seed clearing with seed placement. Results are published with tagged stores into pinned host memory that the host spin-polls, replacing the device-to-host memcpy and stream sync. When enabled by default, it also launches conv0a and the network stack ahead for the newly chosen seed position, so the next inference step can start before the host returns. It also raises the speculation hint limit from 3 to 8. The cost is extra complexity, host CPU spinning, and wasted GPU work whenever the speculative step goes unused.

Result: no change. 5128 (-0.3%).

```diff
diff --git a/ffn_amd/csrc/ffn_canvas_kernels.h b/ffn_amd/csrc/ffn_canvas_kernels.h
--- a/ffn_amd/csrc/ffn_canvas_kernels.h
+++ b/ffn_amd/csrc/ffn_canvas_kernels.h
@@ -140,14 +140,72 @@
   int chosen;
   int pad[2];
 };
+constexpr int kTurnRecWords = (int)(sizeof(TurnRecord) / 4);
+struct TurnCtl {
+  unsigned done[3];
+  int ahead[4];
+  int pad;
+};
 constexpr int kTurnOk = 0, kTurnSegmented = 1, kTurnTooClose = 2, kTurnNotReached = 3,
               kTurnRestricted = 4;
+
+struct TurnPub {
+  int on;
+  unsigned turn_id;
+  unsigned long long* dst;
+  TurnRecord* rec;
+  TurnCtl* ctl;
+  unsigned* hist;
+  int hist_n;
+  const int* cand_out;
+  int n;
+};
+
+__device__ __forceinline__ bool turn_last_block(unsigned* done) {
+  __shared__ int s_last;
+  asm volatile("s_waitcnt vmcnt(0)" ::: "memory");
+  __syncthreads();
+  if (threadIdx.x == 0) {
+    __builtin_amdgcn_fence(__ATOMIC_RELEASE, "agent");
+    asm volatile("s_waitcnt vmcnt(0)" ::: "memory");
+    const unsigned t =
+        __hip_atomic_fetch_add(done, 1u, __ATOMIC_RELAXED, __HIP_MEMORY_SCOPE_AGENT);
+    s_last = t == gridDim.x - 1;
+    if (s_last) {
+      __hip_atomic_store(done, 0u, __ATOMIC_RELAXED, __HIP_MEMORY_SCOPE_AGENT);
+      __builtin_amdgcn_fence(__ATOMIC_ACQUIRE, "agent");
+      asm volatile("s_waitcnt vmcnt(0)" ::: "memory");
+    }
+  }
+  __syncthreads();
+  return s_last != 0;
+}
+
+__device__ __forceinline__ void turn_publish(const TurnPub& p, int committed, int chosen) {
+  const unsigned long long tag = (unsigned long long)p.turn_id << 32;
+  unsigned* rw = reinterpret_cast<unsigned*>(p.rec);
+  const int total = kTurnRecWords + p.hist_n + 3 * p.n;
+  for (int w = threadIdx.x; w < total; w += blockDim.x) {
+    unsigned v;
+    if (w < kTurnRecWords) {
+      v = w == 4 ? (unsigned)committed : w == 5 ? (unsigned)chosen : w < 4 ? rw[w] : 0u;
+      if (w <= 4) rw[w] = 0u;
+    } else if (w < kTurnRecWords + p.hist_n) {
+      v = p.hist[w - kTurnRecWords];
+      if (v) p.hist[w - kTurnRecWords] = 0u;
+    } else {
+      v = (unsigned)__hip_atomic_load(&p.cand_out[w - kTurnRecWords - p.hist_n],
+                                      __ATOMIC_RELAXED, __HIP_MEMORY_SCOPE_AGENT);
+    }
+    __hip_atomic_store(&p.dst[w], tag | v, __ATOMIC_RELAXED, __HIP_MEMORY_SCOPE_SYSTEM);
+  }
+}
 
 __global__ void turn_commit_kernel(const float* __restrict__ seed,
                                    int32_t* __restrict__ seg, Box b, long total,
                                    float thr, int32_t sid, long long min_size,
                                    TurnRecord* __restrict__ rec, long mark_ci,
-                                   int mark_mode) {
+                                   int mark_mode, TurnPub pub) {
   const bool ok = total > 0 && (long long)rec->counts[1] >= min_size;
   if (ok) {
     for (long e = blockIdx.x * (long)blockDim.x + threadIdx.x; e < total;
@@ -157,98 +215,122 @@
     }
   }
   if (blockIdx.x == 0 && threadIdx.x == 0) {
-    rec->committed = ok ? 1 : 0;
     if ((mark_mode == 1 || (mark_mode == 2 && !ok)) && seg[mark_ci] == 0)
       seg[mark_ci] = -1;
   }
-}
-
-__global__ __launch_bounds__(64) void turn_eval_kernel(
-    const float* __restrict__ seed, const int32_t* __restrict__ seg, int cz, int cy,
-    int cx, const int32_t* __restrict__ cand, int mz, int my, int mx,
+  if (pub.on) {
+    if (turn_last_block(&pub.ctl->done[0])) turn_publish(pub, ok ? 1 : 0, -1);
+  } else if (blockIdx.x == 0 && threadIdx.x == 0) {
+    rec->committed = ok ? 1 : 0;
+  }
+}
+
+__global__ __launch_bounds__(64) void turn_eval_pick_kernel(
+    const float* __restrict__ seed, int32_t* __restrict__ seg, int cz, int cy,
+    int cx, const int32_t* __restrict__ cand, int n, int mz, int my, int mx,
     int* __restrict__ flags, float* __restrict__ cand_seed,
     int32_t* __restrict__ cand_seg, const unsigned long long* __restrict__ rplanes,
-    size_t plane_words, int row_words) {
-  const int j = blockIdx.x;
-  const int z = cand[3 * j], y = cand[3 * j + 1], x = cand[3 * j + 2];
-  const size_t ci = ((size_t)z * cy + y) * cx + x;
-  const int32_t s = seg[ci];
-  int flag = kTurnOk;
-  bool restricted = false;
-  if (rplanes) {
-    const size_t wi = ((size_t)z * cy + y) * row_words + (x >> 6);
-    restricted = ((rplanes[wi] | rplanes[plane_words + wi]) >> (x & 63)) & 1ull;
-  }
-  if (s > 0) {
-    flag = kTurnSegmented;
-  } else if (restricted) {
-    flag = kTurnRestricted;
-  } else {
-    const int z0 = max(z - mz, 0), z1 = min(z + mz + 1, cz);
-    const int y0 = max(y - my, 0), y1 = min(y + my + 1, cy);
-    const int x0 = max(x - mx, 0), x1 = min(x + mx + 1, cx);
-    const int ny = y1 - y0, nx = x1 - x0;
-    const int total = (z1 - z0) * ny * nx;
-    int hit = 0;
-    for (int e = threadIdx.x; e < total; e += 64) {
-      const int ex = e % nx, t = e / nx;
-      hit |= seg[((size_t)(z0 + t / ny) * cy + (y0 + t % ny)) * cx + (x0 + ex)] > 0;
-    }
-    if (__any(hit)) flag = kTurnTooClose;
-  }
-  if (threadIdx.x == 0) {
-    flags[j] = flag;
-    cand_seed[j] = seed[ci];
-    cand_seg[j] = s;
-  }
-}
-
-__global__ __launch_bounds__(64) void turn_pick_kernel(
-    int32_t* __restrict__ seg, int cy, int cx, const int32_t* __restrict__ cand,
-    int n, int* __restrict__ flags, TurnRecord* __restrict__ rec) {
+    size_t plane_words, int row_words, TurnRecord* __restrict__ rec,
+    TurnCtl* __restrict__ ctl, int ahead, TurnPub pub) {
+  {
+    const int j = blockIdx.x;
+    const int z = cand[3 * j], y = cand[3 * j + 1], x = cand[3 * j + 2];
+    const size_t ci = ((size_t)z * cy + y) * cx + x;
+    const int32_t s = seg[ci];
+    int flag = kTurnOk;
+    bool restricted = false;
+    if (rplanes) {
+      const size_t wi = ((size_t)z * cy + y) * row_words + (x >> 6);
+      restricted = ((rplanes[wi] | rplanes[plane_words + wi]) >> (x & 63)) & 1ull;
+    }
+    if (s > 0) {
+      flag = kTurnSegmented;
+    } else if (restricted) {
+      flag = kTurnRestricted;
+    } else {
+      const int z0 = max(z - mz, 0), z1 = min(z + mz + 1, cz);
+      const int y0 = max(y - my, 0), y1 = min(y + my + 1, cy);
+      const int x0 = max(x - mx, 0), x1 = min(x + mx + 1, cx);
+      const int ny = y1 - y0, nx = x1 - x0;
+      const int total = (z1 - z0) * ny * nx;
+      int hit = 0;
+      for (int e = threadIdx.x; e < total; e += 64) {
+        const int ex = e % nx, t = e / nx;
+        hit |= seg[((size_t)(z0 + t / ny) * cy + (y0 + t % ny)) * cx + (x0 + ex)] > 0;
+      }
+      if (__any(hit)) flag = kTurnTooClose;
+    }
+    if (threadIdx.x == 0) {
+      flags[j] = flag;
+      cand_seed[j] = seed[ci];
+      cand_seg[j] = s;
+    }
+  }
+  if (!turn_last_block(&ctl->done[1])) return;
+  auto flag_of = [&](int j) {
+    return __hip_atomic_load(&flags[j], __ATOMIC_RELAXED, __HIP_MEMORY_SCOPE_AGENT);
+  };
   int chosen = -1;
   for (int base = 0; base < n && chosen < 0; base += 64) {
     const int j = base + threadIdx.x;
-    const unsigned long long m = __ballot(j < n && flags[j] == kTurnOk);
+    const unsigned long long m = __ballot(j < n && flag_of(j) == kTurnOk);
     if (m) chosen = base + __ffsll((long long)m) - 1;
   }
   const int upto = chosen < 0 ? n : chosen;
   for (int j = threadIdx.x; j < n; j += 64) {
     if (j < upto) {
-      if (flags[j] == kTurnTooClose)
+      if (flag_of(j) == kTurnTooClose)
         seg[((size_t)cand[3 * j] * cy + cand[3 * j + 1]) * cx + cand[3 * j + 2]] = -1;
     } else if (j > upto) {
       flags[j] = kTurnNotReached;
     }
   }
-  if (threadIdx.x == 0) rec->chosen = chosen;
-}
-
-__global__ void turn_clear_kernel(uint32_t* __restrict__ seed, Box b, long total,
-                                  int linear, size_t nvox,
-                                  const TurnRecord* __restrict__ rec) {
-  if (rec->chosen < 0) return;
-  if (linear) {
-    const size_t n4 = nvox / 4;
-    const uint4 vv = make_uint4(0x7fc00000u, 0x7fc00000u, 0x7fc00000u, 0x7fc00000u);
-    for (size_t e = blockIdx.x * (size_t)blockDim.x + threadIdx.x; e < n4;
-         e += (size_t)gridDim.x * blockDim.x)
-      reinterpret_cast<uint4*>(seed)[e] = vv;
-    if (blockIdx.x == 0 && threadIdx.x < (nvox & 3))
-      seed[n4 * 4 + threadIdx.x] = 0x7fc00000u;
-    return;
-  }
-  for (long e = blockIdx.x * (long)blockDim.x + threadIdx.x; e < total;
-       e += (long)gridDim.x * blockDim.x)
-    seed[box_index(b, e)] = 0x7fc00000u;
-}
-
-__global__ void turn_seed_kernel(float* __restrict__ seed, int cy, int cx,
-                                 const int32_t* __restrict__ cand, float value,
-                                 const TurnRecord* __restrict__ rec) {
-  const int j = rec->chosen;
-  if (j < 0) return;
-  seed[((size_t)cand[3 * j] * cy + cand[3 * j + 1]) * cx + cand[3 * j + 2]] = value;
-}
-
-}
+  if (threadIdx.x == 0) {
+    rec->chosen = chosen;
+    if (ahead) {
+      ctl->ahead[0] = chosen;
+      for (int a = 0; a < 3; ++a) ctl->ahead[1 + a] = chosen < 0 ? 0 : cand[3 * chosen + a];
+    }
+  }
+  if (pub.on) {
+    __threadfence();
+    __syncthreads();
+    turn_publish(pub, rec->committed, chosen);
+  }
+}
+
+__global__ void turn_clear_seed_kernel(uint32_t* __restrict__ seed, Box b, long total,
+                                       int linear, size_t nvox, int cy, int cx,
+                                       const int32_t* __restrict__ cand, float value,
+                                       TurnRecord* __restrict__ rec, TurnPub pub) {
+  const int chosen = rec->chosen;
+  const int committed = rec->committed;
+  if (chosen >= 0) {
+    const size_t seed_ci =
+        ((size_t)cand[3 * chosen] * cy + cand[3 * chosen + 1]) * cx + cand[3 * chosen + 2];
+    const uint32_t nan = 0x7fc00000u;
+    if (linear) {
+      const size_t n4 = nvox / 4;
+      for (size_t e = blockIdx.x * (size_t)blockDim.x + threadIdx.x; e < n4;
+           e += (size_t)gridDim.x * blockDim.x) {
+        uint32_t v[4] = {nan, nan, nan, nan};
+        if (e == seed_ci / 4) v[seed_ci & 3] = __float_as_uint(value);
+        reinterpret_cast<uint4*>(seed)[e] = make_uint4(v[0], v[1], v[2], v[3]);
+      }
+      if (blockIdx.x == 0 && threadIdx.x < (nvox & 3) && n4 * 4 + threadIdx.x != seed_ci)
+        seed[n4 * 4 + threadIdx.x] = nan;
+      if (blockIdx.x == 0 && threadIdx.x == 0 && seed_ci >= n4 * 4)
+        seed[seed_ci] = __float_as_uint(value);
+    } else {
+      for (long e = blockIdx.x * (long)blockDim.x + threadIdx.x; e < total;
+           e += (long)gridDim.x * blockDim.x) {
+        const size_t ci = box_index(b, e);
+        if (ci != seed_ci) seed[ci] = nan;
+      }
+      if (blockIdx.x == 0 && threadIdx.x == 0) seed[seed_ci] = __float_as_uint(value);
+    }
+  }
+  if (pub.on && turn_last_block(&pub.ctl->done[2])) turn_publish(pub, committed, chosen);
+}
+
+}
diff --git a/ffn_amd/csrc/ffn_hip.hip b/ffn_amd/csrc/ffn_hip.hip
--- a/ffn_amd/csrc/ffn_hip.hip
+++ b/ffn_amd/csrc/ffn_hip.hip
@@ -151,8 +151,10 @@
     int pos[kSpecMax][3] = {};
     float pad_value = 0.f, move_thr = 0.f;
     int variant = 0;
+    bool from_turn = false;
   } spec;
   int speculate = 1;
+  int spec_hints = kSpecMax;
   int spec_force_mismatch = 0;
   long stat_spec_mismatch = 0;
   long stat_many_carried = 0;
@@ -163,6 +165,16 @@
   long stat_spec_miss_full = 0, stat_spec_miss_short = 0;
   long long stat_segturn_queue_ns = 0, stat_segturn_wait_ns = 0;
   long stat_segturn_calls = 0;
+  char* d_turn = nullptr;
+  unsigned long long* h_turn_pub = nullptr;
+  int32_t* h_turn_cand = nullptr;
+  size_t turn_hist_cap = 0, turn_cand_cap = 0;
+  unsigned turn_id = 0;
+  int turn_ahead = 1;
+  const ffn_canvas* last1_canvas = nullptr;
+  ffn_step_params last1_params{};
+  long stat_turn_ahead_launched = 0, stat_turn_ahead_used = 0;
+  long stat_turn_ahead_unused = 0, stat_turn_ahead_ended = 0;
   int stack_ahead = 1;
   int paste_blocks = 0;
   int debug_submit_delay_ns = 0;
@@ -270,8 +282,9 @@
 inline unsigned next_tag(unsigned t) { return t + 1 ? t + 1 : 1; }
 inline void drop_spec(ffn_engine* e) {
   if (e->spec.valid && !e->ahead_valid) e->range_tag = next_tag(e->range_tag);
-  if (e->ahead_valid) e->stat_ahead_wasted += 1;
+  if (e->ahead_valid) (e->spec.from_turn ? e->stat_turn_ahead_unused : e->stat_ahead_wasted) += 1;
   e->spec.valid = false;
+  e->spec.from_turn = false;
   e->ahead_valid = false;
 }
 struct EngineLock {
@@ -967,8 +980,10 @@
   const Geom& g = e->g;
   const float* W = e->weights;
   if (!conv0a_done) drop_spec(e);
-  if (e->ahead_valid) e->stat_ahead_wasted += 1;
+  if (e->ahead_valid)
+    (e->spec.from_turn ? e->stat_turn_ahead_unused : e->stat_ahead_wasted) += 1;
   e->spec.valid = false;
+  e->spec.from_turn = false;
   e->ahead_valid = false;
   e->last_stack_resident = false;
   e->range_tag = next_tag(e->range_tag);
@@ -1301,6 +1316,7 @@
     E_TRY(hipStreamCreateWithPriority(&e->ustream, hipStreamNonBlocking, hi));
   }
   E_TRY(hipEventCreateWithFlags(&e->main_ev, hipEventDisableTiming));
+  E_TRY(hipDeviceGetAttribute(&e->cus, hipDeviceAttributeMultiprocessorCount, device_id));
   const size_t act_bytes = (size_t)3 * max_batch * g.act_stride * sizeof(float);
   E_TRY(hipMalloc(&e->act_base, act_bytes));
   E_TRY(hipMemset(e->act_base, 0, act_bytes));
@@ -1457,7 +1473,6 @@
       const int span_h = chunk_span(q, 0, kHChunk, e->n_half);
       int cus = 0, per_cu = 0;
       E_TRY(hipDeviceGetAttribute(&cus, hipDeviceAttributeMultiprocessorCount, device_id));
-      e->cus = cus;
       E_TRY(hipFuncSetAttribute(reinterpret_cast<const void*>(conv32hs_kernel),
                                 hipFuncAttributeMaxDynamicSharedMemorySize, kHLdsBytes));
       E_TRY(hipOccupancyMaxActiveBlocksPerMultiprocessor(&per_cu, conv32hs_kernel, kDThreads,
@@ -1595,6 +1610,9 @@
   (void)hipFree(e->weights);
   (void)hipFree(e->d_items);
   (void)hipFree(e->d_scratch);
+  (void)hipFree(e->d_turn);
+  if (e->h_turn_pub) (void)hipHostFree(e->h_turn_pub);
+  if (e->h_turn_cand) (void)hipHostFree(e->h_turn_cand);
   if (e->h_io) (void)hipHostFree(e->h_io);
   if (e->h_items) (void)hipHostFree(e->h_items);
   if (e->h_pub) (void)hipHostFree(e->h_pub);
@@ -1990,6 +2008,17 @@
     e->stack_ahead = value != 0;
     return FFN_OK;
   }
+  if (std::strcmp(name, "turn_ahead") == 0) {
+    drop_spec(e);
+    e->turn_ahead = value != 0;
+    return FFN_OK;
+  }
+  if (std::strcmp(name, "spec_hints") == 0) {
+    if (value < 1 || value > kSpecMax)
+      return fail(FFN_ERR_ARG, "spec_hints must be 1..%d", kSpecMax);
+    e->spec_hints = value;
+    return FFN_OK;
+  }
   if (std::strcmp(name, "speculate") == 0) {
     drop_spec(e);
     e->speculate = value != 0;
@@ -2001,6 +2030,8 @@
     e->stat_spec_miss_full = e->stat_spec_miss_short = 0;
     e->stat_segturn_queue_ns = e->stat_segturn_wait_ns = 0;
     e->stat_segturn_calls = 0;
+    e->stat_turn_ahead_launched = e->stat_turn_ahead_used = 0;
+    e->stat_turn_ahead_unused = e->stat_turn_ahead_ended = 0;
     e->stat_calls = e->stat_items = 0;
     std::memset(e->stat_hist, 0, sizeof(e->stat_hist));
     e->stat_turn_host_ns = e->stat_launch_host_ns = 0;
@@ -2052,6 +2083,19 @@
   else if (std::strcmp(name, "speculate") == 0) *value = e->speculate;
   else if (std::strcmp(name, "stack_ahead") == 0) *value = e->stack_ahead;
   else if (std::strcmp(name, "paste_blocks") == 0) *value = e->paste_blocks;
+  else if (std::strcmp(name, "turn_ahead") == 0) *value = e->turn_ahead;
+  else if (std::strcmp(name, "spec_hints") == 0) *value = e->spec_hints;
+  else if (std::strcmp(name, "spec_hints_max") == 0) *value = kSpecMax;
+  else if (std::strcmp(name, "cus") == 0) *value = e->cus;
+  else if (std::strcmp(name, "stat_turn_ahead_launched") == 0)
+    *value = (int)e->stat_turn_ahead_launched;
+  else if (std::strcmp(name, "stat_turn_ahead_used") == 0) *value = (int)e->stat_turn_ahead_used;
+  else if (std::strcmp(name, "stat_turn_ahead_unused") == 0)
+    *value = (int)e->stat_turn_ahead_unused;
+  else if (std::strcmp(name, "stat_turn_ahead_ended") == 0)
+    *value = (int)e->stat_turn_ahead_ended;
+  else if (std::strcmp(name, "stat_turn_ahead_pending") == 0)
+    *value = e->ahead_valid && e->spec.from_turn ? 1 : 0;
   else if (std::strcmp(name, "stat_segturn_queue_ns") == 0)
     *value = e->stat_segturn_calls ? (int)(e->stat_segturn_queue_ns / e->stat_segturn_calls) : 0;
   else if (std::strcmp(name, "stat_segturn_wait_ns") == 0)
@@ -2489,9 +2533,10 @@
     for (int j = 0; j < e->spec.n && spec_expected < 0; ++j)
       if (std::memcmp(e->spec.pos[j], requests[0].pos, sizeof(int) * 3) == 0)
         spec_expected = j;
-  if (spec_expected >= 0) e->stat_spec_hits += 1;
-  else if (e->spec.valid && n == 1 && from_loop && e->spec.canvas == canvases[0]) {
-    if (e->spec.n >= kSpecMax) e->stat_spec_miss_full += 1;
+  if (spec_expected >= 0) e->stat_spec_hits += e->spec.from_turn ? 0 : 1;
+  else if (e->spec.valid && !e->spec.from_turn && n == 1 && from_loop &&
+           e->spec.canvas == canvases[0]) {
+    if (e->spec.n >= e->spec_hints) e->stat_spec_miss_full += 1;
     else e->stat_spec_miss_short += 1;
   }
   if (spec_expected >= 0 && e->spec_force_mismatch > 0) {
@@ -2508,7 +2553,8 @@
   if (e->ahead_valid && spec_expected >= 0) {
     e->ahead_valid = false;
     e->spec.valid = false;
-    e->stat_ahead_used += 1;
+    (e->spec.from_turn ? e->stat_turn_ahead_used : e->stat_ahead_used) += 1;
+    e->spec.from_turn = false;
     if (e->ahead_ev_pending) {
       e->ahead_ev_pending = false;
       if (e->events_used + 2 > (int)e->events.size()) {
@@ -2562,6 +2608,7 @@
                                         true, nx);
     const int paste_blocks = e->paste_blocks > 0
         ? e->paste_blocks
+        : e->cus <= 0 ? kPasteBlocks
         : std::max(kPasteBlocksMin, std::min(kPasteBlocks, e->cus - 1 - tiles));
     if (e->debug_fused_twice)
       hipLaunchKernelGGL(faces_paste_conv0a_kernel, dim3(1 + paste_blocks + tiles),
@@ -2610,11 +2657,14 @@
       e->spec.pad_value = params->pad_value;
       e->spec.move_thr = params->move_threshold;
       e->spec.variant = e->conv_variant;
+      e->spec.from_turn = false;
       e->stat_spec_launched += 1;
     }
   }
   e->trace_now = false;
   HIP_TRY(hipGetLastError());
+  e->last1_canvas = n == 1 && from_loop ? canvases[0] : nullptr;
+  e->last1_params = *params;
   e->stat_calls += 1;
   e->stat_items += n;
   e->stat_hist[n < 64 ? n : 64] += 1;
@@ -2768,7 +2818,7 @@
   void hint_next(int n, const int32_t (*pos)[3]) {
     EngineLock lock_(c->engine);
     c->hint_from_loop = true;
-    c->hint_n = n < kSpecMax ? n : kSpecMax;
+    c->hint_n = n < c->engine->spec_hints ? n : c->engine->spec_hints;
     for (int j = 0; j < c->hint_n; ++j)
       for (int a = 0; a < 3; ++a) c->hint_pos[j][a] = pos[j][a];
   }
@@ -3226,6 +3276,40 @@
   return FFN_OK;
 }
 
+}
+
+namespace {
+constexpr size_t kTurnHead = sizeof(TurnRecord) + sizeof(TurnCtl);
+
+int ensure_turn(ffn_engine* e, size_t hist_n, size_t n) {
+  if (e->d_turn && hist_n <= e->turn_hist_cap && n <= e->turn_cand_cap) return FFN_OK;
+  HIP_TRY(hipStreamSynchronize(e->ustream));
+  HIP_TRY(hipStreamSynchronize(e->stream));
+  if (e->d_turn) HIP_TRY(hipFree(e->d_turn));
+  if (e->h_turn_pub) HIP_TRY(hipHostFree(e->h_turn_pub));
+  if (e->h_turn_cand) HIP_TRY(hipHostFree(e->h_turn_cand));
+  e->d_turn = nullptr;
+  e->h_turn_pub = nullptr;
+  e->h_turn_cand = nullptr;
+  e->turn_hist_cap = e->turn_cand_cap = 0;
+  const size_t hist_cap = std::max<size_t>(2 * hist_n, 4096);
+  const size_t cand_cap = std::max<size_t>(2 * n, 256);
+  const size_t d_bytes = kTurnHead + 4 * hist_cap + 12 * cand_cap;
+  const size_t words = kTurnRecWords + hist_cap + 3 * cand_cap;
+  HIP_TRY(hipMalloc(&e->d_turn, d_bytes));
+  HIP_TRY(hipMemset(e->d_turn, 0, d_bytes));
+  HIP_TRY(hipDeviceSynchronize());
+  HIP_TRY(hipHostMalloc(&e->h_turn_pub, 8 * words, hipHostMallocDefault));
+  std::memset(e->h_turn_pub, 0, 8 * words);
+  HIP_TRY(hipHostMalloc(&e->h_turn_cand, 12 * cand_cap, hipHostMallocDefault));
+  e->turn_hist_cap = hist_cap;
+  e->turn_cand_cap = cand_cap;
+  return FFN_OK;
+}
+}
+
+extern "C" {
+
 int ffn_canvas_segment_turn(ffn_canvas* c, const ffn_turn_request* rq,
                             const int32_t* cand, ffn_turn_result* out,
                             int32_t max_overlaps, int32_t* overlap_ids,
@@ -3252,107 +3336,219 @@
   if (!e) return fail(FFN_ERR_STATE, "canvas outlived its engine");
   HIP_TRY(hipSetDevice(e->device));
   const long long t_turn0 = steady_ns();
-  HIP_TRY(lock_.begin(e, c));
   const int32_t max_id = rq->do_commit ? std::max(rq->max_existing_id, 0) : 0;
   const size_t hist_n = rq->do_commit ? (size_t)max_id + 1 : 0;
-  const size_t o_hist = sizeof(TurnRecord);
-  const size_t o_flag = (o_hist + hist_n * 4 + 15) & ~(size_t)15;
-  const size_t o_cand = o_flag + 12 * (size_t)n;
-  const size_t bytes = o_cand + 12 * (size_t)n;
-  rc = ensure_scratch(e, bytes);
+  rc = ensure_turn(e, hist_n, (size_t)n);
   if (rc) return rc;
-  char* ds = static_cast<char*>(e->d_scratch);
-  char* hs = static_cast<char*>(e->h_scratch);
-  auto* d_rec = reinterpret_cast<TurnRecord*>(ds);
-  auto* d_hist = reinterpret_cast<unsigned*>(ds + o_hist);
-  auto* d_flag = reinterpret_cast<int*>(ds + o_flag);
-  auto* d_cseed = reinterpret_cast<float*>(ds + o_flag + 4 * (size_t)n);
-  auto* d_cseg = reinterpret_cast<int32_t*>(ds + o_flag + 8 * (size_t)n);
-  auto* d_cand = reinterpret_cast<int32_t*>(ds + o_cand);
-  HIP_TRY(hipMemsetAsync(ds, 0, o_flag, e->ustream));
-  HIP_TRY(hipMemsetAsync(&d_rec->chosen, 0xff, 4, e->ustream));
-  if (n > 0) {
-    std::memcpy(hs + o_cand, cand, 12 * (size_t)n);
-    HIP_TRY(hipMemcpyAsync(d_cand, hs + o_cand, 12 * (size_t)n, hipMemcpyHostToDevice,
-                           e->ustream));
-  }
+  const bool busy = e->slot_n[0] != 0 || e->slot_n[1] != 0;
+  hipStream_t st = busy ? e->ustream : e->stream;
+  if (busy) {
+    HIP_TRY(lock_.begin(e, c));
+  } else {
+    drop_spec(e);
+    if (c->util_pending) {
+      HIP_TRY(hipStreamWaitEvent(e->stream, c->ev_util, 0));
+      c->util_pending = false;
+    }
+  }
+  auto* d_rec = reinterpret_cast<TurnRecord*>(e->d_turn);
+  auto* d_ctl = reinterpret_cast<TurnCtl*>(e->d_turn + sizeof(TurnRecord));
+  auto* d_hist = reinterpret_cast<unsigned*>(e->d_turn + kTurnHead);
+  auto* d_flag = reinterpret_cast<int*>(e->d_turn + kTurnHead + 4 * e->turn_hist_cap);
+  auto* d_cseed = reinterpret_cast<float*>(d_flag + n);
+  auto* d_cseg = reinterpret_cast<int32_t*>(d_flag + 2 * (size_t)n);
+  if (n > 0) std::memcpy(e->h_turn_cand, cand, 12 * (size_t)n);
+  const int words = kTurnRecWords + (int)hist_n + 3 * n;
+  const bool any_commit = rq->do_commit || rq->mark_mode;
+  const bool any_launch = any_commit || n > 0;
+  const int last_phase = (n > 0 && rq->do_init) ? 3 : n > 0 ? 2 : 1;
+  e->turn_id = next_tag(e->turn_id);
+  const unsigned turn_id = e->turn_id;
+  TurnPub pub;
+  pub.on = 0;
+  pub.turn_id = turn_id;
+  pub.dst = e->h_turn_pub;
+  pub.rec = d_rec;
+  pub.ctl = d_ctl;
+  pub.hist = d_hist;
+  pub.hist_n = (int)hist_n;
+  pub.cand_out = d_flag;
+  pub.n = n;
+  const bool do_ahead = !busy && n > 0 && rq->do_init && e->turn_ahead && e->speculate &&
+                        e->fuse_paste && e->fuse_conv0a && e->stack_ahead && e->flow == 2 &&
+                        e->flow_skip == 0 && e->conv_variant == 9 && e->weights_set &&
+                        e->last_stack_resident && e->last1_canvas == c;
   long total = 0;
   Box b{};
   if (rq->do_commit) {
     b = make_box(c, rq->lo, rq->hi, &total);
     if (total > 0)
-      hipLaunchKernelGGL(commit_count_kernel, dim3(grid_for(total)), dim3(256), 0,
-                         e->ustream, c->seed, c->seg, b, total, rq->segment_threshold,
-                         max_id, d_rec->counts, d_hist);
-  }
-  if (rq->do_commit || rq->mark_mode) {
+      hipLaunchKernelGGL(commit_count_kernel, dim3(grid_for(total)), dim3(256), 0, st,
+                         c->seed, c->seg, b, total, rq->segment_threshold, max_id,
+                         d_rec->counts, d_hist);
+  }
+  if (any_commit) {
     const long mark_ci =
         rq->mark_mode ? ((long)rq->mark_pos[0] * c->cy + rq->mark_pos[1]) * c->cx +
                             rq->mark_pos[2]
                       : 0;
+    pub.on = last_phase == 1;
     hipLaunchKernelGGL(turn_commit_kernel, dim3(total > 0 ? grid_for(total) : 1),
-                       dim3(256), 0, e->ustream, c->seed, c->seg, b, total,
+                       dim3(256), 0, st, c->seed, c->seg, b, total,
                        rq->segment_threshold, rq->segment_id,
-                       (long long)rq->min_segment_size, d_rec, mark_ci, rq->mark_mode);
-  }
-  long dirty_total = 0;
+                       (long long)rq->min_segment_size, d_rec, mark_ci, rq->mark_mode, pub);
+  }
   if (n > 0) {
-    hipLaunchKernelGGL(turn_eval_kernel, dim3(n), dim3(64), 0, e->ustream, c->seed,
-                       c->seg, c->cz, c->cy, c->cx, d_cand, rq->min_boundary_dist[0],
-                       rq->min_boundary_dist[1], rq->min_boundary_dist[2], d_flag,
-                       d_cseed, d_cseg, c->restrict_planes, c->restrict_plane_words,
-                       c->restrict_row_words);
-    hipLaunchKernelGGL(turn_pick_kernel, dim3(1), dim3(64), 0, e->ustream, c->seg,
-                       c->cy, c->cx, d_cand, n, d_flag, d_rec);
+    pub.on = last_phase == 2;
+    hipLaunchKernelGGL(turn_eval_pick_kernel, dim3(n), dim3(64), 0, st, c->seed, c->seg,
+                       c->cz, c->cy, c->cx, e->h_turn_cand, n, rq->min_boundary_dist[0],
+                       rq->min_boundary_dist[1], rq->min_boundary_dist[2], d_flag, d_cseed,
+                       d_cseg, c->restrict_planes, c->restrict_plane_words,
+                       c->restrict_row_words, d_rec, d_ctl, do_ahead ? 1 : 0, pub);
     if (rq->do_init) {
+      long dirty_total = 0;
+      Box db{};
+      int linear = 0;
       if (c->dirty_lo[0] < c->dirty_hi[0]) {
-        Box db = make_box(c, c->dirty_lo, c->dirty_hi, &dirty_total);
-        const int linear = (size_t)dirty_total * 2 >= c->nvox;
-        if (dirty_total > 0)
-          hipLaunchKernelGGL(turn_clear_kernel,
-                             dim3(linear ? 2048 : grid_for(dirty_total)), dim3(256), 0,
-                             e->ustream, reinterpret_cast<uint32_t*>(c->seed), db,
-                             dirty_total, linear, c->nvox, d_rec);
+        db = make_box(c, c->dirty_lo, c->dirty_hi, &dirty_total);
+        linear = (size_t)dirty_total * 2 >= c->nvox;
       }
-      hipLaunchKernelGGL(turn_seed_kernel, dim3(1), dim3(1), 0, e->ustream, c->seed,
-                         c->cy, c->cx, d_cand, rq->init_value, d_rec);
+      pub.on = 1;
+      hipLaunchKernelGGL(turn_clear_seed_kernel,
+                         dim3(linear ? 2048 : dirty_total > 0 ? grid_for(dirty_total) : 1),
+                         dim3(256), 0, st, reinterpret_cast<uint32_t*>(c->seed), db,
+                         dirty_total, linear, c->nvox, c->cy, c->cx, e->h_turn_cand,
+                         rq->init_value, d_rec, pub);
     }
   }
   HIP_TRY(hipGetLastError());
-  HIP_TRY(hipMemcpyAsync(hs, ds, o_cand, hipMemcpyDeviceToHost, e->ustream));
+  long ahead_mark = -1;
+  if (do_ahead) {
+    const Geom& g = e->g;
+    StepItems si;
+    std::memset(&si, 0, sizeof(si));
+    si.items = e->d_items;
+    si.use_inline = 1;
+    si.inline_item.image = c->image;
+    si.inline_item.image_u8 = c->image_u8;
+    si.inline_item.image_lut = c->image_lut;
+    si.inline_item.seed = c->seed;
+    si.inline_item.seg = c->seg;
+    si.inline_item.cz = c->cz;
+    si.inline_item.cy = c->cy;
+    si.inline_item.cx = c->cx;
+    SpecArgs sp;
+    std::memset(&sp, 0, sizeof(sp));
+    sp.n = 1;
+    sp.move_thr = e->last1_params.move_threshold;
+    Conv0Next nx;
+    const int tiles = conv0a_split_args(e, e->last1_params.pad_value, next_tag(e->range_tag),
+                                        sp, true, nx);
+    hipLaunchKernelGGL(conv0a_turn_kernel, dim3(tiles), dim3(kC0Threads), 0, e->stream, si, nx,
+                       d_ctl->ahead, g.fz / 2, g.fy / 2, g.fx / 2);
+    rc = run_stack(e, 1, si, e->last1_params.pad_value, e->last1_params.move_threshold, true,
+                   true);
+    if (rc) return rc;
+    e->stat_turn_ahead_launched += 1;
+    ahead_mark = e->stack_calls;
+  }
   const long long t_turn1 = steady_ns();
-  HIP_TRY(lock_.wait(e, c));
+  auto arrived = [&]() {
+    if (words > 0 &&
+        (unsigned)(__atomic_load_n(&e->h_turn_pub[words - 1], __ATOMIC_ACQUIRE) >> 32) != turn_id)
+      return false;
+    for (int k = 0; k < words; ++k)
+      if ((unsigned)(__atomic_load_n(&e->h_turn_pub[k], __ATOMIC_ACQUIRE) >> 32) != turn_id)
+        return false;
+    return true;
+  };
+  if (any_launch) {
+    lock_.lk.unlock();
+    bool done = false;
+    long long t_first = 0, t_query = 0;
+    for (long spin = 0; !done; ++spin) {
+      done = arrived();
+      if (!done && (spin & 0xfff) == 0xfff) {
+        const long long now = steady_ns();
+        if (t_first == 0) t_first = t_query = now;
+        if (now - t_first > 10000000000LL) break;
+        if (now - t_query > 2000000) {
+          t_query = now;
+          if (hipStreamQuery(st) == hipSuccess) done = true;
+        }
+      }
+    }
+    hipError_t err = hipSuccess;
+    if (!done || !arrived()) err = hipStreamSynchronize(st);
+    lock_.lk.lock();
+    HIP_TRY(err);
+    if (!arrived()) return fail(FFN_ERR_HIP, "segment turn %u did not complete", turn_id);
+    c->util_pending = false;
+    if (!busy) c->paste_after_flag = false;
+  }
   e->stat_segturn_queue_ns += t_turn1 - t_turn0;
   e->stat_segturn_wait_ns += steady_ns() - t_turn1;
   e->stat_segturn_calls += 1;
-  const auto* hr = reinterpret_cast<const TurnRecord*>(hs);
+  auto word = [&](int k) {
+    return any_launch ? (uint32_t)__atomic_load_n(&e->h_turn_pub[k], __ATOMIC_RELAXED) : 0u;
+  };
   std::memset(out, 0, sizeof(*out));
-  out->counts.raw_segmented_voxels = (int64_t)hr->counts[0];
-  out->counts.actual_segmented_voxels = (int64_t)hr->counts[1];
-  out->committed = hr->committed;
-  out->chosen = n > 0 ? hr->chosen : -1;
-  const auto* hh = reinterpret_cast<const unsigned*>(hs + o_hist);
+  out->counts.raw_segmented_voxels = (int64_t)(word(0) | ((uint64_t)word(1) << 32));
+  out->counts.actual_segmented_voxels = (int64_t)(word(2) | ((uint64_t)word(3) << 32));
+  out->committed = any_launch ? (int32_t)word(4) : 0;
+  out->chosen = n > 0 ? (int32_t)word(5) : -1;
   int nover = 0;
   for (size_t id = 1; id < hist_n; ++id) {
-    if (hh[id]) {
+    const uint32_t h = word(kTurnRecWords + (int)id);
+    if (h) {
       if (nover < max_overlaps && overlap_ids && overlap_counts) {
         overlap_ids[nover] = (int32_t)id;
-        overlap_counts[nover] = (int64_t)hh[id];
+        overlap_counts[nover] = (int64_t)h;
       }
       ++nover;
     }
   }
   out->counts.num_overlapped_ids = nover;
   if (n > 0) {
-    std::memcpy(cand_flags, hs + o_flag, 4 * (size_t)n);
-    std::memcpy(cand_seed, hs + o_flag + 4 * (size_t)n, 4 * (size_t)n);
-    std::memcpy(cand_seg, hs + o_flag + 8 * (size_t)n, 4 * (size_t)n);
+    const int o = kTurnRecWords + (int)hist_n;
+    for (int k = 0; k < n; ++k) {
+      cand_flags[k] = (int32_t)word(o + k);
+      const uint32_t sv = word(o + n + k);
+      std::memcpy(&cand_seed[k], &sv, 4);
+      cand_seg[k] = (int32_t)word(o + 2 * n + k);
+    }
     if (rq->do_init && out->chosen >= 0) {
       const int32_t* p = cand + 3 * out->chosen;
       const int lo[3] = {p[0], p[1], p[2]};
       const int hi[3] = {p[0] + 1, p[1] + 1, p[2] + 1};
       c->dirty_lo[0] = c->dirty_hi[0] = 0;
       c->mark_dirty(lo, hi);
+    }
+  }
+  if (do_ahead) {
+    const Geom& g = e->g;
+    const int half[3] = {g.fz / 2, g.fy / 2, g.fx / 2};
+    const int dims[3] = {c->cz, c->cy, c->cx};
+    bool ran = out->chosen >= 0;
+    for (int a = 0; a < 3 && ran; ++a) {
+      const int v = cand[3 * out->chosen + a];
+      if (v - half[a] < 0 || v + half[a] >= dims[a]) ran = false;
+    }
+    if (!ran) {
+      e->stat_turn_ahead_ended += 1;
+    } else if (e->stack_calls != ahead_mark || e->spec.valid) {
+      e->stat_turn_ahead_unused += 1;
+    } else {
+      e->spec.valid = true;
+      e->spec.from_turn = true;
+      e->spec.canvas = c;
+      e->spec.n = 1;
+      for (int j = 0; j < kSpecMax; ++j)
+        for (int a = 0; a < 3; ++a) e->spec.pos[j][a] = cand[3 * out->chosen + a];
+      e->spec.pad_value = e->last1_params.pad_value;
+      e->spec.move_thr = e->last1_params.move_threshold;
+      e->spec.variant = e->conv_variant;
+      e->ahead_valid = true;
     }
   }
   return FFN_OK;
diff --git a/ffn_amd/csrc/ffn_host_loop.h b/ffn_amd/csrc/ffn_host_loop.h
--- a/ffn_amd/csrc/ffn_host_loop.h
+++ b/ffn_amd/csrc/ffn_host_loop.h
@@ -70,7 +70,7 @@
   }
 };
 
-constexpr int kHintMax = 3;
+constexpr int kHintMax = 8;
 
 struct StepPending {
   Coord pos;
diff --git a/ffn_amd/csrc/ffn_step_kernels.h b/ffn_amd/csrc/ffn_step_kernels.h
--- a/ffn_amd/csrc/ffn_step_kernels.h
+++ b/ffn_amd/csrc/ffn_step_kernels.h
@@ -55,7 +55,7 @@
 typedef _Float16 f16x8_c0 __attribute__((ext_vector_type(8)));
 typedef _Float16 f16x4_c0 __attribute__((ext_vector_type(4)));
 
-constexpr int kSpecMax = 3;
+constexpr int kSpecMax = 8;
 struct SpecArgs {
   int n;
   int pos[kSpecMax][3];
@@ -368,6 +368,7 @@
   conv0a_body<SPLIT>(blockIdx.x, blockIdx.y, si, pad_value, w, bias, out, seed_raw, g,
                      tiles_y, tiles_x, so, sp, ov);
 }
+
 
 
 __global__ __launch_bounds__(256) void head_kernel(
@@ -761,6 +762,46 @@
   SpecArgs sp;
 };
 
+__global__ __launch_bounds__(kC0Threads) void conv0a_turn_kernel(
+    StepItems si, Conv0Next nx, const int* __restrict__ ahead, int hz, int hy, int hx) {
+  const int ch = ahead[0];
+  const int z = ahead[1], y = ahead[2], x = ahead[3];
+  const StepItem& it = si.inline_item;
+  if (ch < 0 || z - hz < 0 || z + hz >= it.cz || y - hy < 0 || y + hy >= it.cy ||
+      x - hx < 0 || x + hx >= it.cx) {
+    if (blockIdx.x == 0 && threadIdx.x == 0) *nx.sp.choice = -1;
+    return;
+  }
+  SpecArgs sp = nx.sp;
+  sp.n = 1;
+#pragma unroll
+  for (int k = 0; k < kSpecMax; ++k) sp.pos[k][0] = z, sp.pos[k][1] = y, sp.pos[k][2] = x;
+  SeedOverlay ov;
+  ov.on = 0;
+  conv0a_body<true>(blockIdx.x, 0, si, nx.pad_value, nx.w, nx.bias, nx.out, nx.seed_raw, nx.q,
+                    nx.tiles_y, nx.tiles_x, nx.so, sp, ov);
+}
+
+struct FusedStepKernargs {
+  StepItems si;
+  Geom g;
+  const float* logits;
+  const float* in_seed;
+  const unsigned* block_count;
+  int head_blocks;
+  float move_thr, disco_thr, deleted_thr;
+  const unsigned* range_flag;
+  unsigned range_tag;
+  unsigned long long* pub;
+  unsigned step_id;
+  const int* spec_choice;
+  int spec_expected;
+  Conv0Next nx;
+  long long* stamps;
+  int trace, paste_blocks;
+};
+static_assert(sizeof(FusedStepKernargs) <= 1024, "warm_kernargs covers 1 KiB");
+
 __global__ __launch_bounds__(512) void faces_paste_conv0a_kernel(
     StepItems si, Geom g, const float* __restrict__ logits,
     const float* __restrict__ in_seed,
@@ -771,7 +812,7 @@
     long long* __restrict__ stamps, int trace, int paste_blocks) {
   static_assert(kC0Threads == 512, "one block size for the three roles");
   const long long t_in = wall_clock64();
-  warm_kernargs<832>();
+  warm_kernargs<sizeof(FusedStepKernargs)>();
   const long long t_warm = wall_clock64();
   const bool tr_on = stamps && trace != 0;
   struct RoleStamp {
```
